# xxxupeng/stereo_toolbox

Hardware: AMD Instinct MI355X
Metric: stereo pairs/sec @ 540x960 D=192 (GwcNet_GC fwd+bwd) (higher is better)
Workload: dtype f32; 1 GPU; GwcNet_GC(maxdisp=192) train step: fwd+bwd+allreduce+Adam, 576x960 pairs (reference pad_to_2x shape), batch 1/GPU, fp32, synthetic randn inputs, deterministic filler weights; global_batch=1, parallelism=dp1, grad_sync=none (single rank: flat fp32 buffer packed, no collective), launch=eager, optimizer=torch.optim.Adam(fused=True)

## Files before the change

### include/stx_hip.h

```cpp
#ifndef STX_HIP_H
#define STX_HIP_H
#ifdef __cplusplus
extern "C" {
#endif

const char* stx_last_error(void);
const char* stx_build_info(void);
int stx_get_tuning(const char* name);
int stx_set_tuning(const char* name, int value);

int stx_cost_volume_fwd(const float* Lg, const float* Rg, int Cg, int G, const float* Lc, const float* Rc, int Cc,
                        const float* scale, float* vol, int B, int H, int W, int D, int mask_left, void* stream);
int stx_group_normalize_fwd(const float* x, float* y, int B, int C, int G, int HW, float out_scale, void* stream);
int stx_group_normalize_bwd(const float* x, const float* gy, float* gx, int B, int C, int G, int HW, float out_scale, void* stream);
int stx_cost_volume_bwd(const float* gvol, const float* Lg, const float* Rg, int Cg, int G, int Cc, float* gLg,
                        float* gRg, float* gLc, float* gRc, int B, int H, int W, int D, int mask_left, void* stream);

int stx_head_fwd(const float* cost, float* disp, float* stats, int B, int Dc, int Hc, int Wc, int D, int H, int W,
                 void* stream);
long long stx_head_bwd_workspace_floats(int B, int Dc, int H, int W);
int stx_head_bwd(const float* gdisp, const float* cost, const float* disp, const float* stats, float* gcost,
                 float* workspace, int B, int Dc, int Hc, int Wc, int D, int H, int W, void* stream);
int stx_head_fwd2(const float* cost, float* disp, float* stats, int B, int Dc, int Hc, int Wc, int D, int H, int W,
                  int align_corners, void* stream);
int stx_head_bwd2(const float* gdisp, const float* cost, const float* disp, const float* stats, float* gcost,
                  float* workspace, int B, int Dc, int Hc, int Wc, int D, int H, int W, int align_corners, void* stream);
int stx_softargmax_fwd(const float* x, float* out, int B, int D, int HW, void* stream);
int stx_argmax_fwd(const float* x, long long* out, int B, int D, int HW, void* stream);
int stx_unimodal_fwd(const float* x, float* out, int B, int D, int HW, void* stream);
int stx_dominant_modal_fwd(const float* x, float* out, int B, int D, int HW, void* stream);
int stx_modal_fwd(const float* x, float* out, float* aux, int B, int D, int HW, int kind, void* stream);
int stx_modal_bwd(const float* g, const float* out, const float* aux, float* gx, int B, int D, int HW, void* stream);
int stx_split_mode(const float* x, float* mode, unsigned char* mask, int B, int D, int HW, void* stream);
int stx_softmax_d_fwd(const float* x, float* y, int B, int D, int HW, void* stream);

long long stx_conv3d_packed_floats(int K, int N, int T);
int stx_conv3d_pack_weight(const float* w, float* wp, int A, int B, int T, int mode, void* stream);
int stx_conv3d_fwd_blocks(int Do, int Ho, int Wo);
long long stx_conv3d_fwd_stat_rows(int B, int Di, int Hi, int Wi, int Cin, int Cout, int ks, int stride);
int stx_conv3d_fwd(const float* x, const float* wp, float* out, const float* scale, const float* bias,
                   const float* residual, float* stats, int B, int Di, int Hi, int Wi, int Cin, int Cout, int ks,
                   int stride, int relu, void* stream);
int stx_deconv3d_fwd_blocks(int Di, int Hi, int Wi);
int stx_deconv3d_fwd(const float* x, const float* wp, float* out, const float* scale, const float* bias,
                     const float* residual, float* stats, int B, int Di, int Hi, int Wi, int Cin, int Cout, int Do,
                     int Ho, int Wo, int relu, void* stream);
long long stx_conv3d_wgrad_workspace_floats(int B, int Dc, int Hc, int Wc, int CF, int CC, int ks, int stride);
int stx_conv3d_wgrad(const float* fine, const float* coarse, float* dw, float* workspace, int B, int Df, int Hf, int Wf,
                     int CF, int Dc, int Hc, int Wc, int CC, int ks, int stride, void* stream);

int stx_conv3d_wgrad_bn_supported(int B, int D, int H, int W, int CF, int CC);
int stx_conv3d_wgrad_bn(const float* x, const float* gy, const float* z, const float* scale, const float* shift, const float* mean,
                        const float* invstd, const float* gamma, const float* sums, float inv_n, int act, float* dz, float* dw,
                        float* workspace, int B, int D, int H, int W, int CF, int CC, void* stream);

int stx_conv3d_axial_supported(int Cin, int Cout, int kd, int kh, int kw);
long long stx_conv3d_axial_packed_floats(int K, int N, int kd, int kh, int kw);
int stx_conv3d_axial_pack_weight(const float* w, float* wp, int A, int B, int kd, int kh, int kw, int mode, void* stream);
long long stx_conv3d_axial_fwd_stat_rows(int B, int D, int H, int W, int Cin, int Cout, int kd, int kh, int kw);
int stx_conv3d_axial_fwd(const float* x, const float* wp, float* out, const float* scale, const float* bias,
                         const float* residual, float* stats, int B, int D, int H, int W, int Cin, int Cout, int kd, int kh,
                         int kw, int act, void* stream);
long long stx_conv3d_axial_wgrad_workspace_floats(int B, int D, int H, int W, int CF, int CC, int kd, int kh, int kw);
int stx_conv3d_axial_wgrad(const float* x, const float* gz, float* dw, float* workspace, int B, int D, int H, int W, int CF,
                           int CC, int kd, int kh, int kw, void* stream);

int stx_convgru_supported(int hidden, int nx, int cx0, int cx1, int cx2, int ksize);
long long stx_convgru_packed_floats(int K, int N);
int stx_convgru_pack_weight(const float* w0, const float* w1, float* wp, int A, int Bd, int mode, void* stream);
int stx_convgru_gemm(const float* s0, int c0, int p0, const float* s1, int c1, int p1, const float* s2, int c2, int p2,
                     const float* s3, int c3, int p3, const float* wp, int N, int epi, int split, const float* bias0,
                     const float* bias1, const float* add0, int add0_pitch, const float* add1, int add1_pitch, const float* h,
                     int h_pitch, const float* z, float* out0, float* out1, float* out2, int out_pitch, int B, int H, int W,
                     void* stream);
int stx_convgru_gate_rows(long long P, int hidden);
int stx_convgru_gate_bwd(const float* g, int g_pitch, const float* z, const float* q, const float* h, int h_pitch, float* gq,
                         float* gz, float* rows, long long P, int hidden, void* stream);
int stx_convgru_reset_bwd(float* buf, int buf_pitch, const float* g, int g_pitch, const float* z, const float* r, const float* h,
                          int h_pitch, float* gr, float* rows, long long P, int hidden, void* stream);
int stx_convgru_row_sum(const float* rows, float* out, int nrows, int n, void* stream);
long long stx_convgru_wgrad_workspace_floats(int B, int H, int W, int K, int CC);
int stx_convgru_wgrad(const float* s0, int c0, int p0, const float* s1, int c1, int p1, const float* s2, int c2, int p2,
                      const float* s3, int c3, int p3, const float* g0, const float* g1, int CG, float* dw, float* workspace,
                      int B, int H, int W, void* stream);

int stx_selgru_supported(int hidden, int nx, int cx0, int cx1, int cx2);
long long stx_selgru_packed_floats(int K, int N);
int stx_selgru_pack_weight(const float* w0, const float* w1, float* wp, int A, int Bd, int mode, void* stream);
int stx_selgru_gemm(const float* s0, int c0, int p0, const float* s1, int c1, int p1, const float* s2, int c2, int p2,
                    const float* s3, int c3, int p3, const float* wp, int N, int epi, int split, const float* bias0,
                    const float* bias1, const float* add0, int add0_pitch, const float* add1, int add1_pitch, const float* h,
                    int h_pitch, const float* z, const float* att, const float* other, int blend, float* out0, float* out1,
                    float* out2, int out_pitch, long long P, void* stream);
int stx_selgru_blend_bwd(const float* g, int g_pitch, const float* att, const float* zs, const float* qs, const float* zl,
                         const float* ql, const float* h, int h_pitch, float* gs, float* gl, float* gatt, long long P, int hidden,
                         void* stream);
long long stx_selgru_col_sum_workspace_floats(long long P, int n);
int stx_selgru_col_sum(const float* m0, const float* m1, const float* m2, float* out, double* workspace, long long P, int n,
                       void* stream);
long long stx_selgru_wgrad_workspace_floats(long long P, int K, int CC);
int stx_selgru_wgrad(const float* s0, int c0, int p0, const float* s1, int c1, int p1, const float* s2, int c2, int p2,
                     const float* s3, int c3, int p3, const float* g0, const float* g1, int CG, float* dw, float* workspace,
                     long long P, void* stream);

int stx_csa_supported(int C, int ksize);
int stx_csa_blocks(long long HW, int C);
int stx_csa_pool(const float* x, int pitch, double* psum, float* pmax, int* pidx, int B, long long HW, int C, void* stream);
int stx_csa_gate(const double* psum, const float* pmax, const int* pidx, int nblk, const float* w1, const float* w2, float* gate,
                 double* pooled, int* argp, int B, long long HW, int C, void* stream);
int stx_csa_apply(const float* x, int pitch, const double* psum, const float* pmax, const int* pidx, int nblk, const float* w1,
                  const float* w2, float* xp, float* map, int* argc, float* gate, double* pooled, int* argp, int B, long long HW,
                  int C, void* stream);
int stx_csa_sam(const float* map, const float* w, float* att, int B, int H, int W, int ksize, void* stream);
long long stx_csa_sam_bwd_workspace_floats(int B, int H, int W, int ksize);
int stx_csa_sam_bwd(const float* g, const float* att, const float* map, const float* w, float* gpre, float* gmap, float* dw,
                    double* workspace, int B, int H, int W, int ksize, void* stream);
int stx_csa_apply_bwd(const float* x, int pitch, const float* gate, const float* gxp, int gxp_pitch, const float* gmap,
                      const int* argc, float* gx, double* pgate, int B, long long HW, int C, void* stream);
int stx_csa_gate_bwd(const double* pgate, int nblk, const float* gg, const double* pooled, const float* w1, const float* w2,
                     float* dw1, float* dw2, float* gavg, float* gmx, int B, long long HW, int C, void* stream);
int stx_csa_pool_bwd(float* gx, const float* gavg, const float* gmx, const int* argp, int accumulate, int B, long long HW, int C,
                     void* stream);

int stx_conv2d_supported(int Cin, int Cout);
long long stx_conv2d_stat_rows(int groups);
int stx_conv2d_fwd(const float* x, const float* w, float* out, float* stats, int B, int H, int W, int Cin, int Cout, int dgrad,
                   int groups, void* stream);

int stx_conv3d_c1_fwd(const float* x, const float* w, const float* residual, float* out, int B, int D, int H, int W,
                      int Cin, void* stream);
long long stx_conv3d_c1_wgrad_workspace_floats(int Cin);
int stx_conv3d_c1_wgrad(const float* x, const float* gy, float* dw, float* workspace, int B, int D, int H, int W,
                        int Cin, void* stream);
int stx_conv3d_c1_dgrad(const float* gy, const float* w, float* gx, int B, int D, int H, int W, int Cin, void* stream);

int stx_mish_fwd(const float* x, float* y, long long n, void* stream);
int stx_mish_bwd(const float* gy, const float* x, float* gx, long long n, void* stream);
int stx_depth_to_space(const float* y, float* out, int B, int D, int H, int W, int C, int inverse, void* stream);
int stx_gate_fwd(const float* cv, const float* att, float* out, int B, int D, long long HW, int C, void* stream);
int stx_gate_bwd(const float* g, const float* cv, const float* att, float* gcv, float* gatt, int B, int D, long long HW,
                 int C, void* stream);

int stx_concat_channels(const float* in0, const float* in1, const float* in2, const float* in3, int C0, int C1, int C2, int C3,
                        float* out, long long nvox, void* stream);
int stx_split_channels(const float* in, float* out0, float* out1, float* out2, float* out3, int C0, int C1, int C2, int C3,
                       long long nvox, void* stream);
int stx_transpose(const float* in, float* out, int N, int rows, int cols, void* stream);

int stx_dwconv_hw_fwd(const float* x, const float* w, const int* dil, float* out, int B, int D, int H, int W, int C,
                      int flip, void* stream);
long long stx_dwconv_hw_wgrad_workspace_floats(int C);
int stx_dwconv_hw_wgrad(const float* x, const float* gy, const int* dil, float* dw, float* workspace, int B, int D,
                        int H, int W, int C, void* stream);
int stx_cost_volume_scale_bwd(const float* gvol, const float* Lc, const float* Rc, float* gscale, int B, int Cc, int H,
                              int W, int D, int mask_left, void* stream);
int stx_scale_channels(const float* x, const float* s, float* out, long long nvox, int C, void* stream);
int stx_ac_volume_bwd(const float* gvol, const float* Lc, const float* Rc, const float* prob, float* gL, float* gR,
                      float* gprob, int B, int Cc, int H, int W, int D, int mask_left, void* stream);

int stx_bn_reduce_blocks(void);
int stx_bn_stats_rows(long long nvox, int C);
int stx_bn_stats(const float* z, float* partials, long long nvox, int C, int groups, void* stream);
int stx_bn_finalize(const float* partials, int nrows, int C, double count, const float* gamma, const float* beta,
                    float* running_mean, float* running_var, float momentum, float eps, float* scale, float* shift,
                    float* mean, float* invstd, void* stream);
int stx_bn_finalize_groups(const float* partials, int nrows, int C, double count, const float* gamma, const float* beta,
                           float* running_mean, float* running_var, float momentum, float eps, float* out, int groups,
                           void* stream);
int stx_bn_apply(const float* z1, const float* scale1, const float* shift1, const float* z2, const float* scale2,
                 const float* shift2, float* out, long long nvox, int C, int relu, int groups, void* stream);
int stx_bn_bwd_reduce(const float* gy, const float* y, const float* z1, const float* mean1, const float* invstd1,
                      const float* z2, const float* mean2, const float* invstd2, float* partials, float* sums,
                      long long nvox, int C, int relu, void* stream);
int stx_bn_bwd_apply(const float* gy, const float* y, const float* z1, const float* mean1, const float* invstd1,
                     const float* gamma1, const float* z2, const float* mean2, const float* invstd2,
                     const float* gamma2, const float* sums, float* dz1, float* dz2, float* gout, long long nvox, int C,
                     int relu, void* stream);
int stx_bn_bwd_reduce2(const float* gy, const float* y, const float* z1, const float* mean1, const float* invstd1,
                       const float* z2, const float* mean2, const float* invstd2, const float* scale1,
                       const float* shift1, const float* scale2, const float* shift2, float* partials, float* sums,
                       long long nvox, int C, int relu, int groups, void* stream);
int stx_bn_bwd_apply2(const float* gy, const float* y, const float* z1, const float* mean1, const float* invstd1,
                      const float* gamma1, const float* z2, const float* mean2, const float* invstd2,
                      const float* gamma2, const float* scale1, const float* shift1, const float* scale2,
                      const float* shift2, const float* sums, float* dz1, float* dz2, float* gout, long long nvox,
                      int C, int relu, int groups, void* stream);

int stx_pad_normalize_u8(const unsigned char* img, float* out, int B, int H, int W, int Hp, int Wp, int top,
                         const float* mean3, const float* std3, void* stream);

int stx_sampled_volume_fwd(const float* Lg, const float* Rg, int Cg, int G, const float* Lc, const float* Rc, int Cc,
                           const float* samples, float* vol, int B, int H, int W, int S, int CTp, void* stream);
int stx_sampled_volume_bwd(const float* gvol, const float* Lg, const float* Rg, int Cg, int G, int Cc,
                           const float* samples, float* gLg, float* gRg, float* gLc, float* gRc, int B, int H, int W,
                           int S, int CTp, void* stream);

int stx_warp_fwd(const float* x, const float* disp, float* out, int B, int C, int H, int W, void* stream);
int stx_warp_bwd(const float* gout, const float* x, const float* disp, float* gx, float* gdisp, int B, int C, int H, int W,
                 void* stream);
int stx_corr_volume_fwd(const float* ref, const float* tgt, float* vol, int B, int C, int H, int W, int maxdisp, int groups,
                        void* stream);
int stx_corr_volume_bwd(const float* gvol, const float* ref, const float* tgt, float* gref, float* gtgt, int B, int C, int H,
                        int W, int maxdisp, int groups, void* stream);
int stx_disparity_variance_fwd(const float* x, const float* disp, const float* samples, float* out, int B, int D, int HW,
                               void* stream);
int stx_disparity_variance_bwd(const float* g, const float* x, const float* disp, const float* samples, float* gx, float* gdisp,
                               float* gsamples, int B, int D, int HW, void* stream);

long long stx_geo_pyramid_floats(long long rows, int len, int C, int levels);
int stx_geo_corr_fwd(const float* fmap1, const float* fmap2, float* cpyr, int B, int C, int H, int W1, int W2, int levels,
                     void* stream);
int stx_geo_corr_bwd(const float* gcpyr, const float* fmap1, const float* fmap2, float* gfmap1, float* gfmap2, int B, int C, int H,
                     int W1, int W2, int levels, void* stream);
int stx_geo_pyramid_fwd(const float* vol, float* gpyr, int B, int D, int H, int W, int C, int levels, void* stream);
int stx_geo_pyramid_bwd(const float* ggpyr, float* gvol, int B, int D, int H, int W, int C, int levels, void* stream);
int stx_geo_lookup_fwd(const float* gpyr, const float* cpyr, const float* disp, const float* coords, float* out, int B, int H,
                       int W, int D, int C, int W2, int levels, int radius, void* stream);
int stx_geo_lookup_bwd(const float* gout, const float* disp, const float* coords, float* ggpyr, float* gcpyr, int B, int H, int W,
                       int D, int C, int W2, int levels, int radius, void* stream);
int stx_context_upsample_fwd(const float* disp_low, const float* up_weights, float* out, int B, int h, int w, void* stream);
int stx_context_upsample_bwd(const float* g, const float* disp_low, const float* up_weights, float* gdisp, float* gweights, int B,
                             int h, int w, void* stream);

long long stx_corr1d_pyramid_floats(long long rows, int W2, int levels);
int stx_corr1d_pyramid_fwd(const float* fmap1, const float* fmap2, float* cpyr, int B, int C, int H, int W1, int W2, int levels,
                           float scale, void* stream);
int stx_corr1d_pyramid_bwd(const float* gcpyr, const float* fmap1, const float* fmap2, float* gfmap1, float* gfmap2, int B, int C,
                           int H, int W1, int W2, int levels, float scale, void* stream);
int stx_corr1d_lookup_fwd(const float* cpyr, const float* base, const float* disp, const float* jobs, int njobs, float* out, int B,
                          int H, int W1, int W2, int levels, void* stream);
int stx_corr1d_lookup_bwd(const float* gout, const float* base, const float* disp, const float* jobs, int njobs, float* gcpyr,
                          int B, int H, int W1, int W2, int levels, void* stream);

int stx_allpairs_estimates_fwd(const float* vol, int which, float* disp_l, float* conf_l, float* disp_r, float* conf_r, float* stats,
                               int B, int H, int W1, int W2, void* stream);
int stx_allpairs_estimates_bwd(const float* g_disp_l, const float* g_conf_l, const float* g_disp_r, const float* g_conf_r,
                               const float* vol, const float* stats, float* gvol, int B, int H, int W1, int W2, void* stream);
int stx_corr1d_volume_pyramid_fwd(const float* vol, const float* tdisp, const float* tconf, float atten, float* cpyr, int B, int H,
                                  int W1, int W2, int levels, void* stream);
int stx_corr1d_volume_pyramid_bwd(const float* gcpyr, const float* tdisp, const float* tconf, float atten, float* gvol, int B, int H,
                                  int W1, int W2, int levels, void* stream);
int stx_truncate_mask_fwd(const float* disp, const float* conf, int has_th, float conf_th, float atten, float* mask, int B, int H,
                          int W, void* stream);

int stx_generate_masks_fwd(const float* mde, void* masks, int B, int N, int H, int W, void* stream);
int stx_masked_volume_fwd(const float* vol, const float* mde_l, const float* mde_r, float* out, int B, int N, int H, int W2, int W3,
                          void* stream);
int stx_masked_volume_bwd(const float* g, const float* mde_l, const float* mde_r, float* gvol, int B, int N, int H, int W2, int W3,
                          void* stream);
int stx_softlrc_fwd(const float* disp2, const float* disp3, float lrc_th, float* out2, float* out3, int B, int H, int W,
                    void* stream);
long long stx_softlrc_bwd_workspace_floats(int B, int H, int W);
int stx_softlrc_bwd(const float* g2, const float* g3, const float* disp2, const float* disp3, float lrc_th, void* workspace,
                    float* gdisp2, float* gdisp3, int B, int H, int W, void* stream);
int stx_weighted_lsq_fwd(const float* mde, const float* disp, const float* conf, float min_quantile, float max_quantile, float* scale,
                         float* shift, void* stats, int B, long long n, void* stream);
int stx_weighted_lsq_bwd(const float* g_scale, const float* g_shift, const float* mde, const float* disp, const float* conf,
                         const void* stats, float* g_mde, float* g_disp, float* g_conf, int B, long long n, void* stream);
int stx_mirror_detector_fwd(const float* stereo_disp, const float* mono_disp, const float* stereo_conf, const float* mono_conf,
                            float conf_th, float step_gain, float* out, long long n, void* stream);
int stx_mirror_detector_bwd(const float* g_out, const float* stereo_disp, const float* mono_disp, const float* stereo_conf,
                            const float* mono_conf, float conf_th, float step_gain, float* g_stereo_disp, float* g_mono_disp,
                            float* g_stereo_conf, float* g_mono_conf, long long n, void* stream);

int stx_photo_warp_fwd(const float* right, const float* disp, float* warped, float* valid, int B, int C, int H, int W, void* stream);
int stx_photo_warp_bwd(const float* gwarped, const float* right, const float* disp, float* gdisp, int B, int C, int H, int W,
                       void* stream);
int stx_ssim_fwd(const float* x, const float* y, float* out, int B, int C, int H, int W, int window, void* stream);
long long stx_ssim_bwd_workspace_floats(int B, int C, int H, int W);
int stx_ssim_bwd(const float* g_out, const float* x, const float* y, float* gx, float* gy, float* workspace, int B, int C, int H, int W,
                 int window, void* stream);
int stx_photometric_fwd(const float* left, const float* right, const float* disp, double ssim_weight, int enable_mask, float* loss,
                        int B, int C, int H, int W, void* stream);
long long stx_photometric_bwd_workspace_floats(int B, int C, int H, int W);
int stx_photometric_bwd(const float* gloss, const float* left, const float* right, const float* disp, double ssim_weight,
                        int enable_mask, float* gdisp, float* workspace, int B, int C, int H, int W, void* stream);
int stx_auto_mask_fwd(const float* left, const float* right, const float* disp, int denorm, unsigned char* mask, int B, int C, int H,
                      int W, void* stream);
long long stx_smoothness_workspace_floats(int B, int H, int W);
int stx_smoothness_fwd(const float* disp, const float* img, float* out, float* stats, float* workspace, int B, int C, int H, int W,
                       void* stream);
int stx_smoothness_bwd(const float* gout, const float* disp, const float* img, const float* stats, float* gdisp, int B, int C, int H,
                       int W, void* stream);

int stx_sttr_head_fwd(const float* attn, const float* phi, int mode, int iters, float log_one, float log_bin, float log_2w,
                      const unsigned char* occ_mask, const float* target, float* disp, float* occ, float* norm, int* arg,
                      float* gt_response, float* bin_left, float* bin_right, double* us, double* vs, int N, int H, int W, void* stream);
int stx_sttr_head_bwd(const float* g_disp, const float* g_occ, const float* g_gt, const float* g_bin_left, const float* g_bin_right,
                      const float* attn, const float* phi, int mode, int iters, float log_one, float log_bin, float log_2w,
                      const float* target, const float* disp, const float* norm, const int* arg, const double* us, const double* vs,
                      float* g_attn, double* phi_partials, float* g_phi, int N, int H, int W, void* stream);
int stx_sttr_transport_fwd(const float* attn, const float* phi, int mode, int iters, float log_one, float log_bin, float log_2w,
                           float* P, double* us, double* vs, int N, int H, int W, void* stream);
int stx_sttr_transport_bwd(const float* G, const float* attn, const float* phi, int mode, int iters, float log_one, float log_bin,
                           float log_2w, const double* us, const double* vs, float* g_attn, double* phi_partials, float* g_phi, int N,
                           int H, int W, void* stream);

int stx_sttr_attn_fwd(const float* q, const float* k, const float* v, const float* Qr, const float* Kr, int causal, float* o,
                      float* raw, float* avg, float* stats, int W, int B, int E, int head_dim, void* stream);
int stx_sttr_attn_bwd(const float* dO, const float* dRaw, const float* q, const float* k, const float* v, const float* Qr,
                      const float* Kr, const float* o, const float* stats, int causal, float* dq, float* dk, float* dv, float* dQr,
                      float* dKr, float* scratch, long long scratch_floats, int nb, int W, int B, int E, int head_dim, void* stream);

int stx_disp_attention_supported(int L, int C, int nhead, int F, int layers);
int stx_disp_attention_fwd(const float* x, const float* pe, const float* const* params, float* y, float* saved, const long long* seed,
                           float p, float eps, int N, int L, int C, int nhead, int F, int layers, int hw, long long sb, long long sp,
                           long long st, void* stream);
long long stx_disp_attention_bwd_workspace_floats(int N, int L, int C, int F);
int stx_disp_attention_bwd(const float* gy, const float* saved, const float* const* params, float* const* gparams, float* gx, float* gbuf,
                           float* workspace, long long workspace_floats, const long long* seed, float p, float eps, int N, int L, int C,
                           int nhead, int F, int layers, int hw, long long sb, long long sp, long long st, void* stream);
int stx_disp_attention_masks(const long long* seed, float p, unsigned char* masks, int N, int L, int C, int F, int layers, void* stream);

int stx_convex_upsample_fwd(const float* flow, const float* mask, float* out, int N, int D, int H, int W, int mask_channels, int f,
                            float scale, void* stream);
long long stx_convex_upsample_bwd_workspace_floats(int N, int D, int H, int W);
int stx_convex_upsample_bwd(const float* g, const float* flow, const float* mask, float* gflow, float* gmask, float* workspace, int N,
                            int D, int H, int W, int mask_channels, int f, float scale, void* stream);
int stx_softmax_context_upsample_fwd(const float* disp_low, const float* logits, float* out, int B, int h, int w, float scale,
                                     void* stream);
int stx_softmax_context_upsample_bwd(const float* g, const float* disp_low, const float* logits, float* gdisp, float* glogits,
                                     float* workspace, int B, int h, int w, float scale, void* stream);
int stx_sequence_loss_max_predictions(void);
long long stx_sequence_loss_workspace_floats(long long n);
int stx_sequence_loss_fwd(const float* const* preds, const double* weights, int K, const float* gt, float maxdisp, float* loss,
                          int* count, float* workspace, long long n, void* stream);
int stx_sequence_loss_bwd(const float* gloss, const float* const* preds, const double* weights, int K, const float* gt, float maxdisp,
                          const int* count, float* const* gpreds, long long n, void* stream);

int stx_monster_flaw_fwd(const float* left, const float* right, const float* disp_a, const float* disp_b, int zeros_pad, float* out_a,
                         float* out_b, float* valid, int B, int C, int H, int W, void* stream);
int stx_monster_flaw_bwd(const float* g_a, const float* g_b, const float* right, const float* disp_a, const float* disp_b, int zeros_pad,
                         float* g_left, float* g_right, float* g_disp_a, float* g_disp_b, int B, int C, int H, int W, void* stream);
int stx_monster_scale_shift(const float* mono, const float* gt, const unsigned char* mask, long long k, float* out, void* stats, int B,
                            long long n, void* stream);
int stx_monster_apply_scale_shift(const float* x, const float* scale_shift, int with_shift, float* out, int B, long long n,
                                  void* stream);

#ifdef __cplusplus
}
#endif
#endif
```

### stereo_toolbox_amd/_capi.py

```python
import ctypes
import os
import threading

import torch

_P = ctypes.c_void_p
_I = ctypes.c_int
_F = ctypes.c_float
_L = ctypes.c_longlong

SIGNATURES = {
    "stx_get_tuning": [ctypes.c_char_p],
    "stx_set_tuning": [ctypes.c_char_p, _I],
    "stx_cost_volume_fwd": [_P, _P, _I, _I, _P, _P, _I, _P, _P, _I, _I, _I, _I, _I, _P],
    "stx_cost_volume_bwd": [_P, _P, _P, _I, _I, _I, _P, _P, _P, _P, _I, _I, _I, _I, _I, _P],
    "stx_group_normalize_fwd": [_P, _P, _I, _I, _I, _I, _F, _P],
    "stx_group_normalize_bwd": [_P, _P, _P, _I, _I, _I, _I, _F, _P],
    "stx_head_fwd": [_P, _P, _P, _I, _I, _I, _I, _I, _I, _I, _P],
    "stx_head_bwd_workspace_floats": [_I, _I, _I, _I],
    "stx_head_bwd": [_P, _P, _P, _P, _P, _P, _I, _I, _I, _I, _I, _I, _I, _P],
    "stx_head_fwd2": [_P, _P, _P, _I, _I, _I, _I, _I, _I, _I, _I, _P],
    "stx_head_bwd2": [_P, _P, _P, _P, _P, _P, _I, _I, _I, _I, _I, _I, _I, _I, _P],
    "stx_softargmax_fwd": [_P, _P, _I, _I, _I, _P],
    "stx_argmax_fwd": [_P, _P, _I, _I, _I, _P],
    "stx_softmax_d_fwd": [_P, _P, _I, _I, _I, _P],
    "stx_unimodal_fwd": [_P, _P, _I, _I, _I, _P],
    "stx_dominant_modal_fwd": [_P, _P, _I, _I, _I, _P],
    "stx_modal_fwd": [_P, _P, _P, _I, _I, _I, _I, _P],
    "stx_modal_bwd": [_P, _P, _P, _P, _I, _I, _I, _P],
    "stx_split_mode": [_P, _P, _P, _I, _I, _I, _P],
    "stx_conv3d_packed_floats": [_I, _I, _I],
    "stx_conv3d_pack_weight": [_P, _P, _I, _I, _I, _I, _P],
    "stx_conv3d_fwd_blocks": [_I, _I, _I],
    "stx_conv3d_fwd_stat_rows": [_I, _I, _I, _I, _I, _I, _I, _I],
    "stx_deconv3d_fwd_blocks": [_I, _I, _I],
    "stx_conv3d_fwd": [_P, _P, _P, _P, _P, _P, _P, _I, _I, _I, _I, _I, _I, _I, _I, _I, _P],
    "stx_deconv3d_fwd": [_P, _P, _P, _P, _P, _P, _P, _I, _I, _I, _I, _I, _I, _I, _I, _I, _I, _P],
    "stx_conv3d_wgrad_workspace_floats": [_I, _I, _I, _I, _I, _I, _I, _I],
    "stx_conv3d_wgrad": [_P, _P, _P, _P, _I, _I, _I, _I, _I, _I, _I, _I, _I, _I, _I, _P],
    "stx_conv3d_wgrad_bn_supported": [_I, _I, _I, _I, _I, _I],
    "stx_conv3d_wgrad_bn": [_P] * 9 + [_F, _I, _P, _P, _P, _I, _I, _I, _I, _I, _I, _P],
    "stx_conv3d_axial_supported": [_I, _I, _I, _I, _I],
    "stx_conv3d_axial_packed_floats": [_I, _I, _I, _I, _I],
    "stx_conv3d_axial_pack_weight": [_P, _P, _I, _I, _I, _I, _I, _I, _P],
    "stx_conv3d_axial_fwd_stat_rows": [_I] * 9,
    "stx_conv3d_axial_fwd": [_P] * 7 + [_I] * 10 + [_P],
    "stx_conv3d_axial_wgrad_workspace_floats": [_I] * 9,
    "stx_conv3d_axial_wgrad": [_P, _P, _P, _P] + [_I] * 9 + [_P],
    "stx_convgru_supported": [_I] * 6,
    "stx_convgru_packed_floats": [_I, _I],
    "stx_convgru_pack_weight": [_P, _P, _P, _I, _I, _I, _P],
    "stx_convgru_gemm": [_P, _I, _I] * 4 + [_P, _I, _I, _I, _P, _P, _P, _I, _P, _I, _P, _I, _P, _P, _P, _P, _I, _I, _I, _I, _P],
    "stx_convgru_gate_rows": [_L, _I],
    "stx_convgru_gate_bwd": [_P, _I, _P, _P, _P, _I, _P, _P, _P, _L, _I, _P],
    "stx_convgru_reset_bwd": [_P, _I, _P, _I, _P, _P, _P, _I, _P, _P, _L, _I, _P],
    "stx_convgru_row_sum": [_P, _P, _I, _I, _P],
    "stx_convgru_wgrad_workspace_floats": [_I] * 5,
    "stx_convgru_wgrad": [_P, _I, _I] * 4 + [_P, _P, _I, _P, _P, _I, _I, _I, _P],
    "stx_selgru_supported": [_I] * 5,
    "stx_selgru_packed_floats": [_I, _I],
    "stx_selgru_pack_weight": [_P, _P, _P, _I, _I, _I, _P],
    "stx_selgru_gemm": [_P, _I, _I] * 4 + [_P, _I, _I, _I, _P, _P, _P, _I, _P, _I, _P, _I, _P, _P, _P, _I, _P, _P, _P, _I, _L, _P],
    "stx_selgru_blend_bwd": [_P, _I, _P, _P, _P, _P, _P, _P, _I, _P, _P, _P, _L, _I, _P],
    "stx_selgru_col_sum_workspace_floats": [_L, _I],
    "stx_selgru_col_sum": [_P, _P, _P, _P, _P, _L, _I, _P],
    "stx_selgru_wgrad_workspace_floats": [_L, _I, _I],
    "stx_selgru_wgrad": [_P, _I, _I] * 4 + [_P, _P, _I, _P, _P, _L, _P],
    "stx_csa_supported": [_I, _I],
    "stx_csa_blocks": [_L, _I],
    "stx_csa_pool": [_P, _I, _P, _P, _P, _I, _L, _I, _P],
    "stx_csa_gate": [_P, _P, _P, _I, _P, _P, _P, _P, _P, _I, _L, _I, _P],
    "stx_csa_apply": [_P, _I, _P, _P, _P, _I, _P, _P, _P, _P, _P, _P, _P, _P, _I, _L, _I, _P],
    "stx_csa_sam": [_P, _P, _P, _I, _I, _I, _I, _P],
    "stx_csa_sam_bwd_workspace_floats": [_I] * 4,
    "stx_csa_sam_bwd": [_P] * 8 + [_I] * 4 + [_P],
    "stx_csa_apply_bwd": [_P, _I, _P, _P, _I, _P, _P, _P, _P, _I, _L, _I, _P],
    "stx_csa_gate_bwd": [_P, _I, _P, _P, _P, _P, _P, _P, _P, _P, _I, _L, _I, _P],
    "stx_csa_pool_bwd": [_P, _P, _P, _P, _I, _I, _L, _I, _P],
    "stx_conv2d_supported": [_I, _I],
    "stx_conv2d_stat_rows": [_I],
    "stx_conv2d_fwd": [_P, _P, _P, _P, _I, _I, _I, _I, _I, _I, _I, _P],
    "stx_conv3d_c1_fwd": [_P, _P, _P, _P, _I, _I, _I, _I, _I, _P],
    "stx_conv3d_c1_wgrad_workspace_floats": [_I],
    "stx_conv3d_c1_wgrad": [_P, _P, _P, _P, _I, _I, _I, _I, _I, _P],
    "stx_conv3d_c1_dgrad": [_P, _P, _P, _I, _I, _I, _I, _I, _P],
    "stx_mish_fwd": [_P, _P, _L, _P],
    "stx_mish_bwd": [_P, _P, _P, _L, _P],
    "stx_depth_to_space": [_P, _P, _I, _I, _I, _I, _I, _I, _P],
    "stx_gate_fwd": [_P, _P, _P, _I, _I, _L, _I, _P],
    "stx_gate_bwd": [_P, _P, _P, _P, _P, _I, _I, _L, _I, _P],
    "stx_concat_channels": [_P, _P, _P, _P, _I, _I, _I, _I, _P, _L, _P],
    "stx_split_channels": [_P, _P, _P, _P, _P, _I, _I, _I, _I, _L, _P],
    "stx_transpose": [_P, _P, _I, _I, _I, _P],
    "stx_dwconv_hw_fwd": [_P, _P, _P, _P, _I, _I, _I, _I, _I, _I, _P],
    "stx_dwconv_hw_wgrad_workspace_floats": [_I],
    "stx_dwconv_hw_wgrad": [_P, _P, _P, _P, _P, _I, _I, _I, _I, _I, _P],
    "stx_cost_volume_scale_bwd": [_P, _P, _P, _P, _I, _I, _I, _I, _I, _I, _P],
    "stx_scale_channels": [_P, _P, _P, _L, _I, _P],
    "stx_ac_volume_bwd": [_P, _P, _P, _P, _P, _P, _P, _I, _I, _I, _I, _I, _I, _P],
    "stx_pad_normalize_u8": [_P, _P, _I, _I, _I, _I, _I, _I, _P, _P, _P],
    "stx_warp_fwd": [_P, _P, _P, _I, _I, _I, _I, _P],
    "stx_warp_bwd": [_P, _P, _P, _P, _P, _I, _I, _I, _I, _P],
    "stx_corr_volume_fwd": [_P, _P, _P, _I, _I, _I, _I, _I, _I, _P],
    "stx_corr_volume_bwd": [_P, _P, _P, _P, _P, _I, _I, _I, _I, _I, _I, _P],
    "stx_disparity_variance_fwd": [_P, _P, _P, _P, _I, _I, _I, _P],
    "stx_disparity_variance_bwd": [_P, _P, _P, _P, _P, _P, _P, _I, _I, _I, _P],
    "stx_sampled_volume_fwd": [_P, _P, _I, _I, _P, _P, _I, _P, _P, _I, _I, _I, _I, _I, _P],
    "stx_sampled_volume_bwd": [_P, _P, _P, _I, _I, _I, _P, _P, _P, _P, _P, _I, _I, _I, _I, _I, _P],
    "stx_geo_pyramid_floats": [_L, _I, _I, _I],
    "stx_geo_corr_fwd": [_P, _P, _P, _I, _I, _I, _I, _I, _I, _P],
    "stx_geo_corr_bwd": [_P, _P, _P, _P, _P, _I, _I, _I, _I, _I, _I, _P],
    "stx_geo_pyramid_fwd": [_P, _P, _I, _I, _I, _I, _I, _I, _P],
    "stx_geo_pyramid_bwd": [_P, _P, _I, _I, _I, _I, _I, _I, _P],
    "stx_geo_lookup_fwd": [_P, _P, _P, _P, _P, _I, _I, _I, _I, _I, _I, _I, _I, _P],
    "stx_geo_lookup_bwd": [_P, _P, _P, _P, _P, _I, _I, _I, _I, _I, _I, _I, _I, _P],
    "stx_context_upsample_fwd": [_P, _P, _P, _I, _I, _I, _P],
    "stx_context_upsample_bwd": [_P, _P, _P, _P, _P, _I, _I, _I, _P],
    "stx_corr1d_pyramid_floats": [_L, _I, _I],
    "stx_corr1d_pyramid_fwd": [_P, _P, _P, _I, _I, _I, _I, _I, _I, _F, _P],
    "stx_corr1d_pyramid_bwd": [_P, _P, _P, _P, _P, _I, _I, _I, _I, _I, _I, _F, _P],
    "stx_corr1d_lookup_fwd": [_P, _P, _P, _P, _I, _P, _I, _I, _I, _I, _I, _P],
    "stx_corr1d_lookup_bwd": [_P, _P, _P, _P, _I, _P, _I, _I, _I, _I, _I, _P],
    "stx_allpairs_estimates_fwd": [_P, _I, _P, _P, _P, _P, _P, _I, _I, _I, _I, _P],
    "stx_allpairs_estimates_bwd": [_P, _P, _P, _P, _P, _P, _P, _I, _I, _I, _I, _P],
    "stx_corr1d_volume_pyramid_fwd": [_P, _P, _P, _F, _P, _I, _I, _I, _I, _I, _P],
    "stx_corr1d_volume_pyramid_bwd": [_P, _P, _P, _F, _P, _I, _I, _I, _I, _I, _P],
    "stx_truncate_mask_fwd": [_P, _P, _I, _F, _F, _P, _I, _I, _I, _P],
    "stx_generate_masks_fwd": [_P, _P, _I, _I, _I, _I, _P],
    "stx_masked_volume_fwd": [_P, _P, _P, _P, _I, _I, _I, _I, _I, _P],
    "stx_masked_volume_bwd": [_P, _P, _P, _P, _I, _I, _I, _I, _I, _P],
    "stx_softlrc_fwd": [_P, _P, _F, _P, _P, _I, _I, _I, _P],
    "stx_softlrc_bwd_workspace_floats": [_I, _I, _I],
    "stx_softlrc_bwd": [_P, _P, _P, _P, _F, _P, _P, _P, _I, _I, _I, _P],
    "stx_weighted_lsq_fwd": [_P, _P, _P, _F, _F, _P, _P, _P, _I, _L, _P],
    "stx_weighted_lsq_bwd": [_P, _P, _P, _P, _P, _P, _P, _P, _P, _I, _L, _P],
    "stx_mirror_detector_fwd": [_P, _P, _P, _P, _F, _F, _P, _L, _P],
    "stx_mirror_detector_bwd": [_P, _P, _P, _P, _P, _F, _F, _P, _P, _P, _P, _L, _P],
    "stx_photo_warp_fwd": [_P, _P, _P, _P, _I, _I, _I, _I, _P],
    "stx_photo_warp_bwd": [_P, _P, _P, _P, _I, _I, _I, _I, _P],
    "stx_ssim_fwd": [_P, _P, _P, _I, _I, _I, _I, _I, _P],
    "stx_ssim_bwd_workspace_floats": [_I, _I, _I, _I],
    "stx_ssim_bwd": [_P, _P, _P, _P, _P, _P, _I, _I, _I, _I, _I, _P],
    "stx_photometric_fwd": [_P, _P, _P, ctypes.c_double, _I, _P, _I, _I, _I, _I, _P],
    "stx_photometric_bwd_workspace_floats": [_I, _I, _I, _I],
    "stx_photometric_bwd": [_P, _P, _P, _P, ctypes.c_double, _I, _P, _P, _I, _I, _I, _I, _P],
    "stx_auto_mask_fwd": [_P, _P, _P, _I, _P, _I, _I, _I, _I, _P],
    "stx_smoothness_workspace_floats": [_I, _I, _I],
    "stx_smoothness_fwd": [_P, _P, _P, _P, _P, _I, _I, _I, _I, _P],
    "stx_smoothness_bwd": [_P, _P, _P, _P, _P, _I, _I, _I, _I, _P],
    "stx_sttr_head_fwd": [_P, _P, _I, _I, _F, _F, _F] + [_P] * 11 + [_I, _I, _I, _P],
    "stx_sttr_head_bwd": [_P] * 7 + [_I, _I, _F, _F, _F] + [_P] * 9 + [_I, _I, _I, _P],
    "stx_sttr_transport_fwd": [_P, _P, _I, _I, _F, _F, _F, _P, _P, _P, _I, _I, _I, _P],
    "stx_sttr_transport_bwd": [_P, _P, _P, _I, _I, _F, _F, _F, _P, _P, _P, _P, _P, _I, _I, _I, _P],
    "stx_sttr_attn_fwd": [_P] * 5 + [_I] + [_P] * 4 + [_I, _I, _I, _I, _P],
    "stx_sttr_attn_bwd": [_P] * 9 + [_I] + [_P] * 6 + [_L, _I, _I, _I, _I, _I, _P],
    "stx_disp_attention_supported": [_I] * 5,
    "stx_disp_attention_fwd": [_P] * 6 + [_F, _F] + [_I] * 7 + [_L, _L, _L, _P],
    "stx_disp_attention_bwd_workspace_floats": [_I] * 4,
    "stx_disp_attention_bwd": [_P] * 7 + [_L, _P, _F, _F] + [_I] * 7 + [_L, _L, _L, _P],
    "stx_disp_attention_masks": [_P, _F, _P, _I, _I, _I, _I, _I, _P],
    "stx_convex_upsample_fwd": [_P, _P, _P, _I, _I, _I, _I, _I, _I, _F, _P],
    "stx_convex_upsample_bwd_workspace_floats": [_I, _I, _I, _I],
    "stx_convex_upsample_bwd": [_P, _P, _P, _P, _P, _P, _I, _I, _I, _I, _I, _I, _F, _P],
    "stx_softmax_context_upsample_fwd": [_P, _P, _P, _I, _I, _I, _F, _P],
    "stx_softmax_context_upsample_bwd": [_P, _P, _P, _P, _P, _P, _I, _I, _I, _F, _P],
    "stx_sequence_loss_max_predictions": [],
    "stx_sequence_loss_workspace_floats": [_L],
    "stx_sequence_loss_fwd": [_P, _P, _I, _P, _F, _P, _P, _P, _L, _P],
    "stx_sequence_loss_bwd": [_P, _P, _P, _I, _P, _F, _P, _P, _L, _P],
    "stx_monster_flaw_fwd": [_P, _P, _P, _P, _I, _P, _P, _P, _I, _I, _I, _I, _P],
    "stx_monster_flaw_bwd": [_P, _P, _P, _P, _P, _I, _P, _P, _P, _P, _I, _I, _I, _I, _P],
    "stx_monster_scale_shift": [_P, _P, _P, _L, _P, _P, _I, _L, _P],
    "stx_monster_apply_scale_shift": [_P, _P, _I, _P, _I, _L, _P],
    "stx_bn_reduce_blocks": [],
    "stx_bn_stats_rows": [_L, _I],
    "stx_bn_stats": [_P, _P, _L, _I, _I, _P],
    "stx_bn_finalize": [_P, _I, _I, ctypes.c_double, _P, _P, _P, _P, _F, _F, _P, _P, _P, _P, _P],
    "stx_bn_finalize_groups": [_P, _I, _I, ctypes.c_double, _P, _P, _P, _P, _F, _F, _P, _I, _P],
    "stx_bn_apply": [_P, _P, _P, _P, _P, _P, _P, _L, _I, _I, _I, _P],
    "stx_bn_bwd_reduce": [_P, _P, _P, _P, _P, _P, _P, _P, _P, _P, _L, _I, _I, _P],
    "stx_bn_bwd_apply": [_P, _P, _P, _P, _P, _P, _P, _P, _P, _P, _P, _P, _P, _P, _L, _I, _I, _P],
    "stx_bn_bwd_reduce2": [_P] * 14 + [_L, _I, _I, _I, _P],
    "stx_bn_bwd_apply2": [_P] * 18 + [_L, _I, _I, _I, _P],
}
_RET_CHARP = ("stx_last_error", "stx_build_info")


class StxError(RuntimeError):
    pass


class StxLib:

    def __init__(self, path):
        if not os.path.exists(path):
            raise StxError(
                f"HIP library not found: {path}. Build it with `python -m stereo_toolbox_amd.build` "
                "(hipcc, gfx950). There is no CPU fallback for the cost-volume hot path.")
        self.path = path
        self._dll = ctypes.CDLL(path)
        for name in _RET_CHARP:
            fn = getattr(self._dll, name)
            fn.restype = ctypes.c_char_p
            fn.argtypes = []
        self._fns = {}
        for name, argtypes in SIGNATURES.items():
            fn = getattr(self._dll, name, None)
            if fn is None:
                continue
            fn.restype = ctypes.c_longlong if name.endswith(("_floats", "_stat_rows")) else _I
            fn.argtypes = argtypes
            self._fns[name] = fn

    def has(self, name):
        return name in self._fns

    def build_info(self):
        return self._dll.stx_build_info().decode()

    def get_tuning(self, name):
        return self._fns["stx_get_tuning"](name.encode())

    def set_tuning(self, name, value):
        old = self.get_tuning(name)
        if old < 0 or self._fns["stx_set_tuning"](name.encode(), int(value)) != 0:
            raise StxError(f"unknown tuning switch {name}")
        return old

    def raw(self, name):
        return self._fns[name]

    def call(self, name, *args):
        fn = self._fns.get(name)
        if fn is None:
            raise StxError(f"{self.path} does not export {name}")
        rc = fn(*args)
        if rc != 0:
            raise StxError(f"{name} failed ({rc}): {self._dll.stx_last_error().decode()}")


_LIB = None
_LOCK = threading.Lock()
LIB_PATH = os.environ.get("STX_HIP_LIB") or os.path.join(os.path.dirname(os.path.abspath(__file__)), "lib", "libstx_hip.so")


def get_lib():
    global _LIB
    if _LIB is None:
        with _LOCK:
            if _LIB is None:
                _LIB = StxLib(LIB_PATH)
    return _LIB
```

### stereo_toolbox_amd/csrc/bn.hip

```cpp
#include "stx_common.h"
#include <stdlib.h>

namespace {

constexpr int BN_THREADS = 256;
constexpr int BN_RED_BLOCKS = 1024;

__device__ __forceinline__ double bn_block_sum(double v, double* red, int tid) {
    red[tid] = v;
    __syncthreads();
    for (int s = BN_THREADS / 2; s > 0; s >>= 1) {
        if (tid < s) red[tid] += red[tid + s];
        __syncthreads();
    }
    const double r = red[0];
    __syncthreads();
    return r;
}

__global__ __launch_bounds__(BN_THREADS) void bn_finalize_kernel(
    const float* __restrict__ partials, int nrows, int C, double count, const float* __restrict__ gamma,
    const float* __restrict__ beta, float* __restrict__ running_mean, float* __restrict__ running_var,
    float momentum, float eps, float* __restrict__ scale, float* __restrict__ shift, float* __restrict__ mean_out,
    float* __restrict__ invstd_out, int groups) {
    __shared__ double red[BN_THREADS];
    const int c = blockIdx.x, tid = threadIdx.x;
    for (int g = 0; g < groups; ++g, partials += (size_t)nrows * 2 * C, scale += C, shift += C, mean_out += C, invstd_out += C) {
    double s1 = 0.0, s2 = 0.0;
    for (int r = tid; r < nrows; r += BN_THREADS) {
        s1 += (double)partials[(size_t)r * 2 * C + c];
        s2 += (double)partials[(size_t)r * 2 * C + C + c];
    }
    s1 = bn_block_sum(s1, red, tid);
    s2 = bn_block_sum(s2, red, tid);
    if (tid == 0) {
        const double mean = s1 / count;
        double var = s2 / count - mean * mean;
        if (var < 0.0) var = 0.0;
        const float invstd = (float)(1.0 / sqrt(var + (double)eps));
        const float g = gamma ? gamma[c] : 1.f, bt = beta ? beta[c] : 0.f;
        const float sc = g * invstd;
        scale[c] = sc;
        shift[c] = bt - (float)mean * sc;
        mean_out[c] = (float)mean;
        invstd_out[c] = invstd;
        if (running_mean) running_mean[c] = (1.f - momentum) * running_mean[c] + momentum * (float)mean;
        if (running_var) {
            const double unb = count > 1.0 ? var * count / (count - 1.0) : var;
            running_var[c] = (1.f - momentum) * running_var[c] + momentum * (float)unb;
        }
    }
    }
}

constexpr int BN_FIN_THREADS = 512;

__device__ __forceinline__ double bn_shfl_down_f64(double v, int delta) {
    union { double d; float f[2]; } a, b;
    a.d = v;
    b.f[0] = __shfl_down(a.f[0], delta);
    b.f[1] = __shfl_down(a.f[1], delta);
    return b.d;
}

__global__ __launch_bounds__(BN_FIN_THREADS) void bn_finalize4_kernel(
    const float* __restrict__ partials, int nrows, int C, double count, const float* __restrict__ gamma,
    const float* __restrict__ beta, float* __restrict__ running_mean, float* __restrict__ running_var,
    float momentum, float eps, float* __restrict__ scale, float* __restrict__ shift, float* __restrict__ mean_out,
    float* __restrict__ invstd_out, int groups) {
    __shared__ double red[BN_FIN_THREADS / 64][8];
    const int c0 = blockIdx.x * 4, tid = threadIdx.x, lane = tid & 63, wave = tid >> 6;
    for (int g = 0; g < groups; ++g, partials += (size_t)nrows * 2 * C, scale += C, shift += C, mean_out += C, invstd_out += C) {
    if (g) __syncthreads();
    double acc[8] = {0.0, 0.0, 0.0, 0.0, 0.0, 0.0, 0.0, 0.0};
    const float* p = partials + c0;
#pragma unroll 4
    for (int r = tid; r < nrows; r += BN_FIN_THREADS) {
        const float4 a = stx_ld4(p + (size_t)r * 2 * C), b = stx_ld4(p + (size_t)r * 2 * C + C);
        acc[0] += (double)a.x; acc[1] += (double)a.y; acc[2] += (double)a.z; acc[3] += (double)a.w;
        acc[4] += (double)b.x; acc[5] += (double)b.y; acc[6] += (double)b.z; acc[7] += (double)b.w;
    }
#pragma unroll
    for (int k = 0; k < 8; ++k) {
#pragma unroll
        for (int d = 32; d > 0; d >>= 1) acc[k] += bn_shfl_down_f64(acc[k], d);
        if (lane == 0) red[wave][k] = acc[k];
    }
    __syncthreads();
    if (tid < 4) {
        double s1 = 0.0, s2 = 0.0;
        for (int w = 0; w < BN_FIN_THREADS / 64; ++w) { s1 += red[w][tid]; s2 += red[w][4 + tid]; }
        const int c = c0 + tid;
        const double mean = s1 / count;
        double var = s2 / count - mean * mean;
        if (var < 0.0) var = 0.0;
        const float invstd = (float)(1.0 / sqrt(var + (double)eps));
        const float g = gamma ? gamma[c] : 1.f, bt = beta ? beta[c] : 0.f;
        const float sc = g * invstd;
        scale[c] = sc;
        shift[c] = bt - (float)mean * sc;
        mean_out[c] = (float)mean;
        invstd_out[c] = invstd;
        if (running_mean) running_mean[c] = (1.f - momentum) * running_mean[c] + momentum * (float)mean;
        if (running_var) {
            const double unb = count > 1.0 ? var * count / (count - 1.0) : var;
            running_var[c] = (1.f - momentum) * running_var[c] + momentum * (float)unb;
        }
    }
    }
}

__global__ __launch_bounds__(BN_THREADS) void bn_apply_kernel(
    const float* __restrict__ z1, const float* __restrict__ scale1, const float* __restrict__ shift1,
    const float* __restrict__ z2, const float* __restrict__ scale2, const float* __restrict__ shift2,
    float* __restrict__ out, size_t nquads, int CQ, int relu) {
    {
        const size_t go = (size_t)blockIdx.y * nquads * 4, gc = (size_t)blockIdx.y * CQ * 4;
        z1 += go; out += go; scale1 += gc; shift1 += gc;
        if (z2) z2 += go;
        if (scale2) { scale2 += gc; shift2 += gc; }
    }
    for (size_t i = (size_t)blockIdx.x * BN_THREADS + threadIdx.x; i < nquads; i += (size_t)gridDim.x * BN_THREADS) {
        const int cq = (int)(i % CQ) * 4;
        float4 v = stx_ld4(z1 + i * 4);
        const float4 a = stx_ld4(scale1 + cq), b = stx_ld4(shift1 + cq);
        v.x = fmaf(v.x, a.x, b.x); v.y = fmaf(v.y, a.y, b.y); v.z = fmaf(v.z, a.z, b.z); v.w = fmaf(v.w, a.w, b.w);
        if (z2) {
            float4 u = stx_ld4(z2 + i * 4);
            if (scale2) {
                const float4 a2 = stx_ld4(scale2 + cq), b2 = stx_ld4(shift2 + cq);
                u.x = fmaf(u.x, a2.x, b2.x); u.y = fmaf(u.y, a2.y, b2.y);
                u.z = fmaf(u.z, a2.z, b2.z); u.w = fmaf(u.w, a2.w, b2.w);
            }
            v.x += u.x; v.y += u.y; v.z += u.z; v.w += u.w;
        }
        if (relu) {
            v.x = stx_act(v.x, relu); v.y = stx_act(v.y, relu); v.z = stx_act(v.z, relu); v.w = stx_act(v.w, relu);
        }
        stx_st4(out + i * 4, v);
    }
}

__global__ __launch_bounds__(BN_THREADS) void bn_bwd_reduce_kernel(
    const float* __restrict__ gy, const float* __restrict__ y, const float* __restrict__ z1,
    const float* __restrict__ mean1, const float* __restrict__ invstd1, const float* __restrict__ z2,
    const float* __restrict__ mean2, const float* __restrict__ invstd2, const float* __restrict__ sc1,
    const float* __restrict__ sh1, const float* __restrict__ sc2, const float* __restrict__ sh2, float* __restrict__ partials,
    size_t nvox, int C, int relu) {
    __shared__ float red[BN_THREADS * 12];
    const int tid = threadIdx.x;
    const int CQ = C >> 2;
    const int cq = tid % CQ, vl = tid / CQ, VPB = BN_THREADS / CQ;
    {
        const size_t go = (size_t)blockIdx.y * nvox * C, gc = (size_t)blockIdx.y * C;
        gy += go; z1 += go; mean1 += gc; invstd1 += gc;
        if (y) y += go;
        if (z2) z2 += go;
        if (mean2) { mean2 += gc; invstd2 += gc; }
        if (sc1) { sc1 += gc; sh1 += gc; }
        if (sc2) { sc2 += gc; sh2 += gc; }
        partials += (size_t)blockIdx.y * gridDim.x * 3 * C;
    }
    const float4 m1 = stx_ld4(mean1 + 4 * cq), i1 = stx_ld4(invstd1 + 4 * cq);
    float4 m2 = make_float4(0.f, 0.f, 0.f, 0.f), i2 = m2;
    const bool has2 = z2 && mean2;
    if (has2) { m2 = stx_ld4(mean2 + 4 * cq); i2 = stx_ld4(invstd2 + 4 * cq); }
    const bool remask = relu && !y;
    float4 a1 = m2, b1 = m2, a2 = m2, b2 = m2;
    if (remask) {
        a1 = stx_ld4(sc1 + 4 * cq); b1 = stx_ld4(sh1 + 4 * cq);
        if (has2) { a2 = stx_ld4(sc2 + 4 * cq); b2 = stx_ld4(sh2 + 4 * cq); }
    }
    float s[12];
#pragma unroll
    for (int k = 0; k < 12; ++k) s[k] = 0.f;
    for (size_t v = vl < VPB ? (size_t)blockIdx.x * VPB + vl : nvox; v < nvox; v += (size_t)gridDim.x * VPB) {
        const size_t o = v * C + 4 * cq;
        float4 g = stx_ld4(gy + o);
        const float4 a = stx_ld4(z1 + o);
        float4 c = make_float4(0.f, 0.f, 0.f, 0.f);
        if (has2) c = stx_ld4(z2 + o);
        if (relu) {
            float4 yy;
            if (remask) {
                yy.x = fmaf(a.x, a1.x, b1.x); yy.y = fmaf(a.y, a1.y, b1.y); yy.z = fmaf(a.z, a1.z, b1.z); yy.w = fmaf(a.w, a1.w, b1.w);
                if (has2) {
                    yy.x += fmaf(c.x, a2.x, b2.x); yy.y += fmaf(c.y, a2.y, b2.y);
                    yy.z += fmaf(c.z, a2.z, b2.z); yy.w += fmaf(c.w, a2.w, b2.w);
                }
            } else {
                yy = stx_ld4(y + o);
            }
            g.x = stx_act_bwd(g.x, yy.x, relu); g.y = stx_act_bwd(g.y, yy.y, relu);
            g.z = stx_act_bwd(g.z, yy.z, relu); g.w = stx_act_bwd(g.w, yy.w, relu);
        }
        s[0] += g.x; s[1] += g.y; s[2] += g.z; s[3] += g.w;
        s[4] = fmaf(g.x, (a.x - m1.x) * i1.x, s[4]); s[5] = fmaf(g.y, (a.y - m1.y) * i1.y, s[5]);
        s[6] = fmaf(g.z, (a.z - m1.z) * i1.z, s[6]); s[7] = fmaf(g.w, (a.w - m1.w) * i1.w, s[7]);
        if (has2) {
            s[8] = fmaf(g.x, (c.x - m2.x) * i2.x, s[8]); s[9] = fmaf(g.y, (c.y - m2.y) * i2.y, s[9]);
            s[10] = fmaf(g.z, (c.z - m2.z) * i2.z, s[10]); s[11] = fmaf(g.w, (c.w - m2.w) * i2.w, s[11]);
        }
    }
#pragma unroll
    for (int k = 0; k < 12; ++k) red[k * BN_THREADS + tid] = s[k];
    __syncthreads();
    for (int idx = tid; idx < 12 * CQ; idx += BN_THREADS) {
        const int k = idx / CQ, q = idx % CQ;
        float t = 0.f;
        for (int j = q; j < BN_THREADS; j += CQ) t += red[k * BN_THREADS + j];
        partials[((size_t)blockIdx.x * 3 + (k >> 2)) * C + 4 * q + (k & 3)] = t;
    }
}

__global__ __launch_bounds__(BN_THREADS) void bn_stats_kernel(const float* __restrict__ z, float* __restrict__ partials,
                                                              size_t nvox, int C) {
    __shared__ float red[BN_THREADS * 8];
    const int tid = threadIdx.x;
    const int CQ = C >> 2;
    const int cq = tid % CQ, vl = tid / CQ, VPB = BN_THREADS / CQ;
    z += (size_t)blockIdx.y * nvox * C;
    partials += (size_t)blockIdx.y * gridDim.x * 2 * C;
    float s[8];
#pragma unroll
    for (int k = 0; k < 8; ++k) s[k] = 0.f;
    const size_t step = (size_t)gridDim.x * VPB;
    size_t v = vl < VPB ? (size_t)blockIdx.x * VPB + vl : nvox;
    for (; v + 3 * step < nvox; v += 4 * step) {
        float4 a[4];
#pragma unroll
        for (int u = 0; u < 4; ++u) a[u] = stx_ld4(z + (v + u * step) * C + 4 * cq);
#pragma unroll
        for (int u = 0; u < 4; ++u) {
            s[0] += a[u].x; s[1] += a[u].y; s[2] += a[u].z; s[3] += a[u].w;
            s[4] = fmaf(a[u].x, a[u].x, s[4]); s[5] = fmaf(a[u].y, a[u].y, s[5]);
            s[6] = fmaf(a[u].z, a[u].z, s[6]); s[7] = fmaf(a[u].w, a[u].w, s[7]);
        }
    }
    for (; v < nvox; v += step) {
        const float4 a = stx_ld4(z + v * C + 4 * cq);
        s[0] += a.x; s[1] += a.y; s[2] += a.z; s[3] += a.w;
        s[4] = fmaf(a.x, a.x, s[4]); s[5] = fmaf(a.y, a.y, s[5]); s[6] = fmaf(a.z, a.z, s[6]); s[7] = fmaf(a.w, a.w, s[7]);
    }
#pragma unroll
    for (int k = 0; k < 8; ++k) red[k * BN_THREADS + tid] = s[k];
    __syncthreads();
    for (int idx = tid; idx < 8 * CQ; idx += BN_THREADS) {
        const int k = idx / CQ, q = idx % CQ;
        float t = 0.f;
        for (int j = q; j < BN_THREADS; j += CQ) t += red[k * BN_THREADS + j];
        partials[((size_t)blockIdx.x * 2 + (k >> 2)) * C + 4 * q + (k & 3)] = t;
    }
}

__global__ __launch_bounds__(BN_THREADS) void bn_colsum_kernel(const float* __restrict__ partials, int nrows, int M,
                                                               float* __restrict__ sums, int groups) {
    __shared__ double red[BN_THREADS];
    const int m = blockIdx.x, tid = threadIdx.x;
    float tot = 0.f;
    for (int g = 0; g < groups; ++g) {
        const float* p = partials + (size_t)g * nrows * M;
        double s = 0.0;
        for (int r = tid; r < nrows; r += BN_THREADS) s += (double)p[(size_t)r * M + m];
        s = bn_block_sum(s, red, tid);
        if (tid == 0) {
            sums[(size_t)g * M + m] = (float)s;
            tot += (float)s;
        }
    }
    if (groups > 1 && tid == 0) sums[(size_t)groups * M + m] = tot;
}

__global__ __launch_bounds__(BN_THREADS) void bn_bwd_apply_kernel(
    const float* __restrict__ gy, const float* __restrict__ y, const float* __restrict__ z1,
    const float* __restrict__ mean1, const float* __restrict__ invstd1, const float* __restrict__ gamma1,
    const float* __restrict__ z2, const float* __restrict__ mean2, const float* __restrict__ invstd2,
    const float* __restrict__ gamma2, const float* __restrict__ sc1, const float* __restrict__ sh1,
    const float* __restrict__ sc2, const float* __restrict__ sh2, const float* __restrict__ sums, float* __restrict__ dz1,
    float* __restrict__ dz2, float* __restrict__ gout, size_t nquads, int C, int relu, float inv_n) {
    const int CQ = C >> 2;
    {
        const size_t go = (size_t)blockIdx.y * nquads * 4, gc = (size_t)blockIdx.y * C;
        gy += go; z1 += go; dz1 += go; mean1 += gc; invstd1 += gc; sums += 3 * gc;
        if (y) y += go;
        if (z2) z2 += go;
        if (dz2) dz2 += go;
        if (gout) gout += go;
        if (mean2) { mean2 += gc; invstd2 += gc; }
        if (sc1) { sc1 += gc; sh1 += gc; }
        if (sc2) { sc2 += gc; sh2 += gc; }
    }
    const bool has2 = z2 && mean2 && dz2;
    const bool remask = relu && !y;
    for (size_t i = (size_t)blockIdx.x * BN_THREADS + threadIdx.x; i < nquads; i += (size_t)gridDim.x * BN_THREADS) {
        const int c = (int)(i % CQ) * 4;
        float4 g = stx_ld4(gy + i * 4);
        const float4 a = stx_ld4(z1 + i * 4);
        float4 a2v = make_float4(0.f, 0.f, 0.f, 0.f);
        if (has2) a2v = stx_ld4(z2 + i * 4);
        if (relu) {
            float4 yy;
            if (remask) {
                const float4 p1 = stx_ld4(sc1 + c), q1 = stx_ld4(sh1 + c);
                yy.x = fmaf(a.x, p1.x, q1.x); yy.y = fmaf(a.y, p1.y, q1.y); yy.z = fmaf(a.z, p1.z, q1.z); yy.w = fmaf(a.w, p1.w, q1.w);
                if (has2) {
                    const float4 p2 = stx_ld4(sc2 + c), q2 = stx_ld4(sh2 + c);
                    yy.x += fmaf(a2v.x, p2.x, q2.x); yy.y += fmaf(a2v.y, p2.y, q2.y);
                    yy.z += fmaf(a2v.z, p2.z, q2.z); yy.w += fmaf(a2v.w, p2.w, q2.w);
                }
            } else {
                yy = stx_ld4(y + i * 4);
            }
            g.x = stx_act_bwd(g.x, yy.x, relu); g.y = stx_act_bwd(g.y, yy.y, relu);
            g.z = stx_act_bwd(g.z, yy.z, relu); g.w = stx_act_bwd(g.w, yy.w, relu);
        }
        if (gout) stx_st4(gout + i * 4, g);
        const float4 sg = stx_ld4(sums + c);
        {
            const float4 m = stx_ld4(mean1 + c), is = stx_ld4(invstd1 + c);
            const float4 gm = gamma1 ? stx_ld4(gamma1 + c) : make_float4(1.f, 1.f, 1.f, 1.f);
            const float4 sx = stx_ld4(sums + C + c);
            float4 d;
            d.x = gm.x * is.x * (g.x - sg.x * inv_n - (a.x - m.x) * is.x * sx.x * inv_n);
            d.y = gm.y * is.y * (g.y - sg.y * inv_n - (a.y - m.y) * is.y * sx.y * inv_n);
            d.z = gm.z * is.z * (g.z - sg.z * inv_n - (a.z - m.z) * is.z * sx.z * inv_n);
            d.w = gm.w * is.w * (g.w - sg.w * inv_n - (a.w - m.w) * is.w * sx.w * inv_n);
            stx_st4(dz1 + i * 4, d);
        }
        if (has2) {
            const float4 a = a2v, m = stx_ld4(mean2 + c), is = stx_ld4(invstd2 + c);
            const float4 gm = gamma2 ? stx_ld4(gamma2 + c) : make_float4(1.f, 1.f, 1.f, 1.f);
            const float4 sx = stx_ld4(sums + 2 * C + c);
            float4 d;
            d.x = gm.x * is.x * (g.x - sg.x * inv_n - (a.x - m.x) * is.x * sx.x * inv_n);
            d.y = gm.y * is.y * (g.y - sg.y * inv_n - (a.y - m.y) * is.y * sx.y * inv_n);
            d.z = gm.z * is.z * (g.z - sg.z * inv_n - (a.z - m.z) * is.z * sx.z * inv_n);
            d.w = gm.w * is.w * (g.w - sg.w * inv_n - (a.w - m.w) * is.w * sx.w * inv_n);
            stx_st4(dz2 + i * 4, d);
        }
    }
}

int bn_grid(size_t nquads) {
    size_t g = (nquads + BN_THREADS - 1) / BN_THREADS;
    return (int)(g > 4096 ? 4096 : (g < 1 ? 1 : g));
}

}

extern "C" int stx_bn_reduce_blocks(void) {
    stx_begin(); return BN_RED_BLOCKS; }

static int bn_finalize_launch(const float* partials, int nrows, int C, double count, const float* gamma, const float* beta,
                              float* running_mean, float* running_var, float momentum, float eps, float* scale, float* shift,
                              float* mean, float* invstd, int groups, void* stream) {
    if (C % 4 == 0 && nrows >= 256)
        hipLaunchKernelGGL(bn_finalize4_kernel, dim3(C / 4), dim3(BN_FIN_THREADS), 0, (hipStream_t)stream, partials, nrows, C,
                           count, gamma, beta, running_mean, running_var, momentum, eps, scale, shift, mean, invstd, groups);
    else
        hipLaunchKernelGGL(bn_finalize_kernel, dim3(C), dim3(BN_THREADS), 0, (hipStream_t)stream, partials, nrows, C, count,
                           gamma, beta, running_mean, running_var, momentum, eps, scale, shift, mean, invstd, groups);
    return stx_check_launch("bn_finalize");
}

extern "C" int stx_bn_finalize(const float* partials, int nrows, int C, double count, const float* gamma,
                               const float* beta, float* running_mean, float* running_var, float momentum, float eps,
                               float* scale, float* shift, float* mean, float* invstd, void* stream) {
    stx_begin();
    STX_REQUIRE(partials && nrows > 0 && C > 0 && count > 0 && scale && shift && mean && invstd, "bn_finalize: bad args");
    return bn_finalize_launch(partials, nrows, C, count, gamma, beta, running_mean, running_var, momentum, eps, scale, shift,
                              mean, invstd, 1, stream);
}

extern "C" int stx_bn_finalize_groups(const float* partials, int nrows, int C, double count, const float* gamma,
                                      const float* beta, float* running_mean, float* running_var, float momentum, float eps,
                                      float* out, int groups, void* stream) {
    stx_begin();
    STX_REQUIRE(partials && nrows > 0 && C > 0 && count > 0 && out && groups >= 1, "bn_finalize_groups: bad args");
    const size_t gc = (size_t)groups * C;
    return bn_finalize_launch(partials, nrows, C, count, gamma, beta, running_mean, running_var, momentum, eps, out, out + gc,
                              out + 2 * gc, out + 3 * gc, groups, stream);
}

extern "C" int stx_bn_stats_rows(long long nvox, int C) {
    stx_begin();
    if (C < 4 || C % 4 != 0 || C / 4 > BN_THREADS || nvox < 1) return 0;
    const long long vpb = BN_THREADS / (C / 4);
    const long long g = (nvox + 4 * vpb - 1) / (4 * vpb);
    return (int)(g > 256 ? 256 : (g < 1 ? 1 : g));
}

extern "C" int stx_bn_stats(const float* z, float* partials, long long nvox, int C, int groups, void* stream) {
    stx_begin();
    STX_REQUIRE(z && partials && nvox > 0 && groups >= 1 && groups <= 65535, "bn_stats: bad args");
    STX_REQUIRE(C >= 4 && C % 4 == 0 && C / 4 <= BN_THREADS, "bn_stats: C=%d unsupported (a multiple of 4, at most 1024)", C);
    hipLaunchKernelGGL(bn_stats_kernel, dim3(stx_bn_stats_rows(nvox, C), groups), dim3(BN_THREADS), 0, (hipStream_t)stream, z,
                       partials, (size_t)nvox, C);
    return stx_check_launch("bn_stats");
}

extern "C" int stx_bn_apply(const float* z1, const float* scale1, const float* shift1, const float* z2,
                            const float* scale2, const float* shift2, float* out, long long nvox, int C, int relu,
                            int groups, void* stream) {
    stx_begin();
    STX_REQUIRE(z1 && scale1 && shift1 && out && nvox > 0 && C > 0 && C % 4 == 0, "bn_apply: bad args (C=%d)", C);
    STX_REQUIRE(!scale2 || (z2 && shift2), "bn_apply: second affine needs z2 and shift2");
    STX_REQUIRE(groups >= 1 && groups <= 65535, "bn_apply: groups=%d", groups);
    const size_t nquads = (size_t)nvox * (C / 4);
    hipLaunchKernelGGL(bn_apply_kernel, dim3(bn_grid(nquads), groups), dim3(BN_THREADS), 0, (hipStream_t)stream, z1, scale1,
                       shift1, z2, scale2, shift2, out, nquads, C / 4, relu);
    return stx_check_launch("bn_apply");
}

extern "C" int stx_bn_bwd_reduce2(const float* gy, const float* y, const float* z1, const float* mean1,
                                  const float* invstd1, const float* z2, const float* mean2, const float* invstd2,
                                  const float* scale1, const float* shift1, const float* scale2, const float* shift2,
                                  float* partials, float* sums, long long nvox, int C, int relu, int groups, void* stream) {
    stx_begin();
    STX_REQUIRE(gy && z1 && mean1 && invstd1 && partials && sums && nvox > 0, "bn_bwd_reduce: null operand");
    STX_REQUIRE(groups >= 1 && groups <= 65535, "bn_bwd_reduce: groups=%d", groups);
    STX_REQUIRE(C >= 4 && C % 4 == 0 && C / 4 <= BN_THREADS, "bn_bwd_reduce: C=%d unsupported (a multiple of 4, at most 1024)", C);
    STX_REQUIRE(!relu || y || (scale1 && shift1 && (!(z2 && mean2) || (scale2 && shift2))),
                "bn_bwd_reduce: the relu mask needs y or the forward pass's scale / shift vectors");
    STX_REQUIRE(relu != 2 || !y, "bn_bwd_reduce: Mish (activation code 2) differentiates the pre-activation value: pass y = NULL and the scale / shift vectors");
    hipStream_t st = (hipStream_t)stream;
    const int nblk = ((long long)nvox * C <= (9ll << 19)) ? BN_RED_BLOCKS / 4 : BN_RED_BLOCKS;
    hipLaunchKernelGGL(bn_bwd_reduce_kernel, dim3(nblk, groups), dim3(BN_THREADS), 0, st, gy, y, z1, mean1, invstd1,
                       z2, mean2, invstd2, scale1, shift1, scale2, shift2, partials, (size_t)nvox, C, relu);
    int rc = stx_check_launch("bn_bwd_reduce");
    if (rc) return rc;
    hipLaunchKernelGGL(bn_colsum_kernel, dim3(3 * C), dim3(BN_THREADS), 0, st, partials, nblk, 3 * C, sums, groups);
    return stx_check_launch("bn_colsum");
}

extern "C" int stx_bn_bwd_apply2(const float* gy, const float* y, const float* z1, const float* mean1,
                                 const float* invstd1, const float* gamma1, const float* z2, const float* mean2,
                                 const float* invstd2, const float* gamma2, const float* scale1, const float* shift1,
                                 const float* scale2, const float* shift2, const float* sums, float* dz1, float* dz2,
                                 float* gout, long long nvox, int C, int relu, int groups, void* stream) {
    stx_begin();
    STX_REQUIRE(gy && z1 && mean1 && invstd1 && sums && dz1 && nvox > 0 && C % 4 == 0, "bn_bwd_apply: bad args");
    STX_REQUIRE(groups >= 1 && groups <= 65535, "bn_bwd_apply: groups=%d", groups);
    STX_REQUIRE(!relu || y || (scale1 && shift1 && (!(z2 && mean2 && dz2) || (scale2 && shift2))),
                "bn_bwd_apply: the relu mask needs y or the forward pass's scale / shift vectors");
    STX_REQUIRE(relu != 2 || !y, "bn_bwd_apply: Mish (activation code 2) differentiates the pre-activation value: pass y = NULL and the scale / shift vectors");
    const size_t nquads = (size_t)nvox * (C / 4);
    hipLaunchKernelGGL(bn_bwd_apply_kernel, dim3(bn_grid(nquads), groups), dim3(BN_THREADS), 0, (hipStream_t)stream, gy, y, z1,
                       mean1, invstd1, gamma1, z2, mean2, invstd2, gamma2, scale1, shift1, scale2, shift2, sums, dz1, dz2,
                       gout, nquads, C, relu, (float)(1.0 / (double)nvox));
    return stx_check_launch("bn_bwd_apply");
}

extern "C" int stx_bn_bwd_reduce(const float* gy, const float* y, const float* z1, const float* mean1,
                                 const float* invstd1, const float* z2, const float* mean2, const float* invstd2,
                                 float* partials, float* sums, long long nvox, int C, int relu, void* stream) {
    return stx_bn_bwd_reduce2(gy, y, z1, mean1, invstd1, z2, mean2, invstd2, nullptr, nullptr, nullptr, nullptr, partials,
                              sums, nvox, C, relu, 1, stream);
}

extern "C" int stx_bn_bwd_apply(const float* gy, const float* y, const float* z1, const float* mean1,
                                const float* invstd1, const float* gamma1, const float* z2, const float* mean2,
                                const float* invstd2, const float* gamma2, const float* sums, float* dz1, float* dz2,
                                float* gout, long long nvox, int C, int relu, void* stream) {
    return stx_bn_bwd_apply2(gy, y, z1, mean1, invstd1, gamma1, z2, mean2, invstd2, gamma2, nullptr, nullptr, nullptr,
                             nullptr, sums, dz1, dz2, gout, nvox, C, relu, 1, stream);
}
```

### stereo_toolbox_amd/csrc/conv2d.hip

```cpp
#include "stx_common.h"

namespace {

constexpr int C2_THREADS = 256;
constexpr int C2_TH = 8, C2_TW = 16, C2_EH = C2_TH + 2, C2_EW = C2_TW + 2, C2_NV = C2_EH * C2_EW;

struct Conv2dArgs {
    const float* x;
    const float* w;
    float* out;
    float* stats;
    int B, H, W, Cin, Cout;
    int nHt, nWt, groups;
    int dgrad;
};

__device__ __forceinline__ f32x4 c2_zero4() { f32x4 z = {0.f, 0.f, 0.f, 0.f}; return z; }

template <int KQ, int ABL = 0, int PAD = 8>
__global__ __launch_bounds__(C2_THREADS) void conv2d_march_kernel(Conv2dArgs a) {
    constexpr int CIN = 16 * KQ, VS = CIN + PAD, F4 = CIN / 4;
    constexpr int WFLOATS = 9 * KQ * 256;
    constexpr int NST = (C2_NV * F4 + C2_THREADS - 1) / C2_THREADS;
    constexpr int SLOT = (NST * C2_THREADS / F4) * VS;
    constexpr int NSTEP = 9 * KQ;
    STX_DYN_SMEM(smem);
    float* wl = reinterpret_cast<float*>(smem);
    float* bufs = wl + WFLOATS;
    float* ssum = bufs + 2 * SLOT;

    const int tid = threadIdx.x, lane = tid & 63, wave = __builtin_amdgcn_readfirstlane(tid >> 6);
    const int i = lane & 15, kg = lane >> 4;

    const int wgs_g = gridDim.x / a.groups;
    const int grp = blockIdx.x / wgs_g, wl_id = blockIdx.x - grp * wgs_g;
    const int tiles_img = a.nHt * a.nWt;
    const int tiles_g = (a.B / a.groups) * tiles_img;
    const int nsl = a.Cout / 16;
    const long long units = (long long)tiles_g * nsl;
    const bool idle = grp >= a.groups;
    int u = idle ? 0 : __builtin_amdgcn_readfirstlane((int)(units * wl_id / wgs_g));
    const int u_end = idle ? 0 : __builtin_amdgcn_readfirstlane((int)(units * (wl_id + 1) / wgs_g));

    if (a.stats) {
        for (int e = tid; e < 2 * a.Cout; e += C2_THREADS) ssum[e] = 0.f;
    }

    unsigned rel[NST];
    int crd[NST];
#pragma unroll
    for (int k = 0; k < NST; ++k) {
        const int e = tid + k * C2_THREADS;
        const int v = e / F4, f = e - v * F4;
        const int hy = v / C2_EW, wx = v - hy * C2_EW;
        crd[k] = e < C2_NV * F4 ? (hy << 8 | wx) : -1;
        rel[k] = (unsigned)(((hy * a.W + wx) * CIN + 4 * f) * 4);
    }
    float4 stg[NST];
    auto decode = [&](int uu, int& slice, int& b, int& oh0, int& ow0) {
        slice = uu / tiles_g;
        const int t = uu - slice * tiles_g;
        const int bl = t / tiles_img, r = t - bl * tiles_img;
        const int ht = r / a.nWt, wt = r - ht * a.nWt;
        b = grp * (a.B / a.groups) + bl;
        oh0 = ht * C2_TH; ow0 = wt * C2_TW;
    };
    auto load_tile = [&](int b, int oh0, int ow0) {
        const long long org = (long long)(oh0 - 1) * a.W + (ow0 - 1), img = (long long)a.H * a.W;
        const stx_bufrsrc rs = stx_make_rsrc(a.x + ((long long)b * img + org) * CIN, (unsigned)((img - org) * CIN * 4));
#pragma unroll
        for (int k = 0; k < NST; ++k) {
            const int gh = oh0 - 1 + (crd[k] >> 8), gw = ow0 - 1 + (crd[k] & 255);
            const bool ok = crd[k] >= 0 && gh >= 0 && gh < a.H && gw >= 0 && gw < a.W;
            stg[k] = stx_buf_ld4(rs, ok ? rel[k] : STX_BUF_OOB, 0u);
        }
    };
    auto store_tile = [&](float* buf) {
#pragma unroll
        for (int k = 0; k < NST; ++k) {
            const int e = tid + k * C2_THREADS;
            const int v = e / F4, f = e - v * F4;
            if (e < C2_NV * F4) stx_st4(buf + v * VS + 4 * f, stg[k]);
        }
    };
    auto load_weights = [&](int slice) {
        if (!a.dgrad) {
            for (int e = tid; e < WFLOATS / 4; e += C2_THREADS) {
                const int l = e & 63, ts = e >> 6, tap = ts / KQ, s = ts - tap * KQ;
                stx_st4(wl + 4 * e, stx_ld4(a.w + ((size_t)(16 * slice + (l & 15)) * 9 + tap) * CIN + 16 * s + 4 * (l >> 4)));
            }
        } else {
            for (int e = tid; e < CIN * 9 * 4; e += C2_THREADS) {
                const int q = e & 3, kt = e >> 2, tap = kt % 9, k = kt / 9;
                const float4 v = stx_ld4(a.w + ((size_t)k * 9 + (8 - tap)) * a.Cout + 16 * slice + 4 * q);
                float* dst = wl + ((tap * KQ + (k >> 4)) * 64 + 4 * q + 16 * ((k & 15) >> 2)) * 4 + (k & 3);
                dst[0] = v.x; dst[4] = v.y; dst[8] = v.z; dst[12] = v.w;
            }
        }
    };

    f32x4 pacc0 = c2_zero4(), pacc1 = c2_zero4();
    unsigned pvoff[2] = {STX_BUF_OOB, STX_BUF_OOB}, cvoff[2] = {STX_BUF_OOB, STX_BUF_OOB};
    stx_bufrsrc prs = stx_make_rsrc(a.out, 0u);
    float s1[4] = {0.f, 0.f, 0.f, 0.f}, s2[4] = {0.f, 0.f, 0.f, 0.f};
    auto emit_prev = [&](int r) {
        f32x4 v = r ? pacc1 : pacc0;
        const bool ok = (int)pvoff[r] >= 0;
#pragma unroll
        for (int c = 0; c < 4; ++c) {
            v[c] = ok ? v[c] : 0.f;
            s1[c] += v[c];
            s2[c] = fmaf(v[c], v[c], s2[c]);
        }
        stx_buf_st4(prs, pvoff[r], 0u, make_float4(v[0], v[1], v[2], v[3]));
    };
    auto flush_stats = [&](int slice) {
#pragma unroll
        for (int c = 0; c < 4; ++c) {
#pragma unroll
            for (int d = 1; d < 16; d <<= 1) { s1[c] += __shfl_xor(s1[c], d); s2[c] += __shfl_xor(s2[c], d); }
        }
        for (int w = 0; w < 4; ++w) {
            if (wave == w && i == 0) {
#pragma unroll
                for (int c = 0; c < 4; ++c) {
                    ssum[16 * slice + 4 * kg + c] += s1[c];
                    ssum[a.Cout + 16 * slice + 4 * kg + c] += s2[c];
                }
            }
            __syncthreads();
        }
#pragma unroll
        for (int c = 0; c < 4; ++c) { s1[c] = 0.f; s2[c] = 0.f; }
    };

    const int abase0 = ((2 * wave) * C2_EW + i) * VS + 4 * kg, abase1 = abase0 + C2_EW * VS;
    const float* wlane = wl + lane * 4;

    int slice = 0, b = 0, oh0 = 0, ow0 = 0;
    if (u < u_end) {
        decode(u, slice, b, oh0, ow0);
        load_weights(slice);
        load_tile(b, oh0, ow0);
        store_tile(bufs);
    }
    __syncthreads();
    int cur = 0;
    while (u < u_end) {
        const bool more = u + 1 < u_end;
        int nslice = slice, nb = b, noh0 = oh0, now0 = ow0;
        if (more) decode(u + 1, nslice, nb, noh0, now0);
        const long long norg = (long long)(noh0 - 1) * a.W + (now0 - 1), img = (long long)a.H * a.W;
        const stx_bufrsrc nrs = stx_make_rsrc(a.x + ((long long)nb * img + norg) * CIN, more ? (unsigned)((img - norg) * CIN * 4) : 0u);
        const stx_bufrsrc crs = stx_make_rsrc(a.out + (size_t)b * img * a.Cout, (unsigned)(img * a.Cout * 4));
        const float* pbuf = bufs + cur * SLOT;
        float* nbuf = bufs + (cur ^ 1) * SLOT;
        f32x4 acc0, acc1;
        float4 av0[3], av1[3], bv[3];
        auto load_step = [&](int st, int slot) {
            const int tap = st / KQ, s = st - tap * KQ;
            const int kh = tap / 3, kw = tap - 3 * kh;
            const float* sl = pbuf + (kh * C2_EW + kw) * VS + 16 * s;
            av0[slot] = stx_ld4(sl + abase0);
            av1[slot] = stx_ld4(sl + abase1);
            bv[slot] = stx_ld4(wlane + st * 256);
        };
        load_step(0, 0);
        load_step(1, 1);
#pragma unroll
        for (int st = 0; st < NSTEP; ++st) {
            if (st + 2 < NSTEP) load_step(st + 2, (st + 2) % 3);
            const int cb = st % 3;
            acc0 = __builtin_amdgcn_mfma_f32_16x16x4f32(bv[cb].x, av0[cb].x, st == 0 ? c2_zero4() : acc0, 0, 0, 0);
            acc1 = __builtin_amdgcn_mfma_f32_16x16x4f32(bv[cb].x, av1[cb].x, st == 0 ? c2_zero4() : acc1, 0, 0, 0);
            acc0 = __builtin_amdgcn_mfma_f32_16x16x4f32(bv[cb].y, av0[cb].y, acc0, 0, 0, 0);
            acc1 = __builtin_amdgcn_mfma_f32_16x16x4f32(bv[cb].y, av1[cb].y, acc1, 0, 0, 0);
            acc0 = __builtin_amdgcn_mfma_f32_16x16x4f32(bv[cb].z, av0[cb].z, acc0, 0, 0, 0);
            acc1 = __builtin_amdgcn_mfma_f32_16x16x4f32(bv[cb].z, av1[cb].z, acc1, 0, 0, 0);
            acc0 = __builtin_amdgcn_mfma_f32_16x16x4f32(bv[cb].w, av0[cb].w, acc0, 0, 0, 0);
            acc1 = __builtin_amdgcn_mfma_f32_16x16x4f32(bv[cb].w, av1[cb].w, acc1, 0, 0, 0);
            if (st < NST) {
                const unsigned gh = (unsigned)(noh0 - 1 + (crd[st] >> 8)), gw = (unsigned)(now0 - 1 + (crd[st] & 255));
                const bool ok = (crd[st] >= 0) & (gh < (unsigned)a.H) & (gw < (unsigned)a.W);
                if (!(ABL & 1)) stg[st] = stx_buf_ld4(nrs, ok ? rel[st] : STX_BUF_OOB, 0u);
            }
            if ((st == 0 || st == 4) && !(ABL & 4)) emit_prev(st >> 2);
            if (st == 8 || st == 9) {
                const int r = st - 8;
                const int oh = oh0 + 2 * wave + r, ow = ow0 + i;
                cvoff[r] = (unsigned)((((oh * a.W + ow) * a.Cout) + 16 * slice + 4 * kg) * 4) | (((oh < a.H) & (ow < a.W)) ? 0u : STX_BUF_OOB);
            }
            if (st >= NSTEP - NST) {
                const int k = st - (NSTEP - NST);
                const int e = tid + k * C2_THREADS;
                const int v = e / F4, f = e - v * F4;
                if (!(ABL & 2)) stx_st4(nbuf + v * VS + 4 * f, stg[k]);
            }
            STX_SCHED_GROUP(0x008, 1); STX_SCHED_GROUP(0x100, 1);
            STX_SCHED_GROUP(0x008, 1); STX_SCHED_GROUP(0x100, 1);
            STX_SCHED_GROUP(0x008, 1); STX_SCHED_GROUP(0x100, 1);
            STX_SCHED_GROUP(0x008, 1); STX_SCHED_GROUP(0x002, 4);
            STX_SCHED_GROUP(0x008, 1); STX_SCHED_GROUP(0x010, 1); STX_SCHED_GROUP(0x002, 4);
            STX_SCHED_GROUP(0x008, 1); STX_SCHED_GROUP(0x010, 1); STX_SCHED_GROUP(0x002, 4);
            STX_SCHED_GROUP(0x008, 1); STX_SCHED_GROUP(0x200, 1); STX_SCHED_GROUP(0x002, 4);
            STX_SCHED_GROUP(0x008, 1);
            STX_SCHED_BARRIER();
        }
        prs = crs;
        pvoff[0] = cvoff[0]; pvoff[1] = cvoff[1];
        pacc0 = acc0; pacc1 = acc1;
        if (!(ABL & 8)) __syncthreads();
        if (more && nslice != slice) {
            emit_prev(0); emit_prev(1);
            pvoff[0] = pvoff[1] = STX_BUF_OOB;
            if (a.stats) flush_stats(slice);
            load_weights(nslice);
            __syncthreads();
        }
        slice = nslice; b = nb; oh0 = noh0; ow0 = now0;
        cur ^= 1;
        ++u;
    }
    emit_prev(0); emit_prev(1);
    if (a.stats) {
        __syncthreads();
        if (u_end > 0 && !idle) flush_stats(slice);
        __syncthreads();
        for (int e = tid; e < 2 * a.Cout; e += C2_THREADS) a.stats[(size_t)blockIdx.x * 2 * a.Cout + e] = ssum[e];
    }
}

int conv2d_grid(int groups) {
    int g = 256;
    g -= g % groups;
    return g < groups ? groups : g;
}

}

extern "C" int stx_conv2d_supported(int Cin, int Cout) {
    stx_begin();
    return (Cin == 32 || Cin == 64) && Cout >= 16 && Cout % 16 == 0 && Cout <= 256;
}

extern "C" long long stx_conv2d_stat_rows(int groups) {
    stx_begin();
    return groups >= 1 && groups <= 256 ? conv2d_grid(groups) : 0;
}

extern "C" int stx_conv2d_fwd(const float* x, const float* w, float* out, float* stats, int B, int H, int W, int Cin, int Cout,
                              int dgrad, int groups, void* stream) {
    stx_begin();
    STX_REQUIRE(x && w && out && B > 0 && H > 0 && W > 0 && (dgrad == 0 || dgrad == 1), "conv2d_fwd: bad args");
    STX_REQUIRE(stx_conv2d_supported(Cin, Cout), "conv2d_fwd: %d -> %d channels unsupported (Cin 32 or 64, Cout a multiple of 16)", Cin, Cout);
    STX_REQUIRE(groups >= 1 && groups <= 256 && B % groups == 0, "conv2d_fwd: batch %d does not split into %d groups", B, groups);
    STX_REQUIRE((long long)(H + 2) * W * (Cin > Cout ? Cin : Cout) * 4 < (1ll << 31), "conv2d_fwd: image too large for one descriptor");
    STX_REQUIRE(H < 32768 && W < 32768, "conv2d_fwd: image too large");
    Conv2dArgs a;
    a.x = x; a.w = w; a.out = out; a.stats = stats; a.dgrad = dgrad;
    a.B = B; a.H = H; a.W = W; a.Cin = Cin; a.Cout = Cout;
    a.nHt = stx_cdiv(H, C2_TH); a.nWt = stx_cdiv(W, C2_TW); a.groups = groups;
    const int grid = conv2d_grid(groups);
    int pad = stx_tune(STX_TUNE_C2_PAD);
    if (pad != 4 && pad != 12) pad = 8;
    const size_t lds = ((size_t)9 * Cin * 16 + (size_t)2 * 192 * (Cin + pad) + (size_t)2 * Cout) * 4;
    void (*k)(Conv2dArgs) = Cin == 64 ? conv2d_march_kernel<4> : conv2d_march_kernel<2>;
    if (pad == 4) k = Cin == 64 ? conv2d_march_kernel<4, 0, 4> : conv2d_march_kernel<2, 0, 4>;
    if (pad == 12) k = Cin == 64 ? conv2d_march_kernel<4, 0, 12> : conv2d_march_kernel<2, 0, 12>;
    const int abl = stx_tune(STX_TUNE_C2_ABLATE);
    if (abl && Cin == 64 && pad == 8)
        k = abl == 1 ? conv2d_march_kernel<4, 1> : abl == 2 ? conv2d_march_kernel<4, 2> : abl == 3 ? conv2d_march_kernel<4, 3>
          : abl == 4 ? conv2d_march_kernel<4, 4> : abl == 7 ? conv2d_march_kernel<4, 7> : abl == 8 ? conv2d_march_kernel<4, 8>
          : conv2d_march_kernel<4, 15>;
    if (int rc = stx_lds_require((const void*)k, lds, "conv2d_fwd")) return rc;
    hipLaunchKernelGGL(k, dim3(grid), dim3(C2_THREADS), lds, (hipStream_t)stream, a);
    return stx_check_launch("conv2d_fwd");
}
```

### stereo_toolbox_amd/csrc/stx_runtime.hip

```cpp
#include "stx_common.h"
#include <stdarg.h>
#include <stdio.h>

static thread_local char g_err[512] = "";

int stx_set_error(int code, const char* fmt, ...) {
    va_list ap;
    va_start(ap, fmt);
    vsnprintf(g_err, sizeof(g_err), fmt, ap);
    va_end(ap);
    return code;
}

int stx_check_launch(const char* what) {
    hipError_t e = hipGetLastError();
    if (e != hipSuccess) return stx_set_error(STX_ERR_LAUNCH, "%s: launch failed: %s", what, hipGetErrorString(e));
    return STX_OK;
}

bool stx_lds_try(const void* kern, size_t bytes) {
    if (bytes <= STX_LDS_DEFAULT) return true;
    if (bytes > STX_LDS_MAX) return false;
    if (hipFuncSetAttribute(kern, hipFuncAttributeMaxDynamicSharedMemorySize, (int)bytes) == hipSuccess) return true;
    (void)hipGetLastError();
    return false;
}

int stx_lds_require(const void* kern, size_t bytes, const char* what) {
    if (bytes > STX_LDS_MAX) return stx_set_error(STX_ERR_ARG, "%s: %zu B of LDS exceed the %zu B of a CU", what, bytes, STX_LDS_MAX);
    if (!stx_lds_try(kern, bytes)) return stx_set_error(STX_ERR_LAUNCH, "%s: %zu B of LDS refused by this device", what, bytes);
    return STX_OK;
}

extern "C" const char* stx_last_error(void) { return g_err; }

extern "C" const char* stx_build_info(void) {
#ifdef STX_HIPEMU
    return "stx-hipemu (host SIMT emulator build: tests only)";
#else
    return "stx-gfx950 (hipcc --offload-arch=gfx950)";
#endif
}

#include <stdlib.h>
#include <string.h>
namespace {
struct TuneEntry { const char* name; int value; };
constexpr int TUNE_N = STX_TUNE_COUNT + 1;
TuneEntry g_tune[TUNE_N] = {
    {"STX_MARCH_BS", 1}, {"STX_MARCH_EPI", 1}, {"STX_MARCH_ABLATE", 0}, {"STX_WGRAD_ABLATE", 0}, {"STX_WGRAD_MARCH", 3}, {"STX_WGRAD_GRID", 0}, {"STX_CONV_L1_MARCH", 0}, {"STX_CONV_S2_DENSE", 1}, {"STX_CONV_WN", 2},
    {"STX_CV_OLD", 0}, {"STX_CV_GRID", 0}, {"STX_CV_PF", 0}, {"STX_CV_UNITS", 1}, {"STX_CV_WIN", 0}, {"STX_CVB_OLD", 0}, {"STX_CVB_TEAM", 0}, {"STX_CVB_GRID", 0}, {"STX_CVB_NSET", 3},
    {"STX_SV_BWD_V1", 0}, {"STX_DWCONV_ROLL", 1}, {"STX_C2_PAD", 8}, {"STX_C2_ABLATE", 0}, {"STX_DA_GRID", 0},
};
struct TuneInit {
    TuneInit() {
        for (int i = 0; i < TUNE_N; ++i)
            if (const char* e = getenv(g_tune[i].name)) g_tune[i].value = atoi(e);
    }
} g_tune_init;
}

int stx_tune(StxTune id) { return g_tune[id].value; }

extern "C" int stx_get_tuning(const char* name) {
    for (int i = 0; i < TUNE_N; ++i)
        if (name && !strcmp(name, g_tune[i].name)) return g_tune[i].value;
    return -1;
}

extern "C" int stx_set_tuning(const char* name, int value) {
    for (int i = 0; i < TUNE_N; ++i)
        if (name && !strcmp(name, g_tune[i].name)) { g_tune[i].value = value; return STX_OK; }
    return stx_set_error(STX_ERR_ARG, "stx_set_tuning: unknown switch %s", name ? name : "(null)");
}
```

### stereo_toolbox_amd/models/features2d.py

```python
import math
import os
import threading

import torch
import torch.nn as nn
import torch.nn.functional as F

from .. import ops
from ..aggregation import _bn_state, _fold


def channels_last_weights_(module):
    for m in module.modules():
        if isinstance(m, nn.Conv2d) and m.weight.dim() == 4:
            m.weight.data = m.weight.data.contiguous(memory_format=torch.channels_last)
    return module


def fused_glue(x, *bns):
    if os.environ.get("STX_FEAT2D_FUSED", "1") == "0":
        return False
    if x.dtype != torch.float32 or not ops.on_device(x):
        return False
    if ops.autocast_active():
        return False
    if not all(isinstance(b, nn.modules.batchnorm._BatchNorm) for b in bns):
        return False
    if all(b.training for b in bns):
        return True
    return (not torch.is_grad_enabled() and not any(b.training for b in bns)
            and all(b.track_running_stats and b.running_mean is not None for b in bns))


class view_groups:
    _tls = threading.local()

    def __init__(self, n):
        self.new = int(n)

    @staticmethod
    def current():
        return getattr(view_groups._tls, "n", 1)

    def __enter__(self):
        self.old, view_groups._tls.n = view_groups.current(), self.new
        return self

    def __exit__(self, *exc):
        view_groups._tls.n = self.old
        return False


def _nhwc(t):
    v = t.permute(0, 2, 3, 1)
    return v if v.is_contiguous() else v.contiguous()


def cat_features(parts):
    parts = list(parts)
    if (os.environ.get("STX_FEAT2D_FUSED", "1") != "0" and os.environ.get("STX_FEAT2D_FUSED_CAT", "1") != "0" and 2 <= len(parts) <= 4
            and all(p.dtype == torch.float32 and ops.on_device(p) and p.shape[1] % 4 == 0
                    and p.is_contiguous(memory_format=torch.channels_last) for p in parts)):
        return ops.cat_channels([_nhwc(p) for p in parts]).permute(0, 3, 1, 2)
    return torch.cat(parts, dim=1)


def own_conv2d(x, conv):
    return (os.environ.get("STX_FEAT2D_CONV", "1") != "0" and x.dtype == torch.float32 and ops.on_device(x)
            and ops.conv2d_supported(conv) and x.shape[0] % view_groups.current() == 0)


def conv_bn_act(x, conv, bn, relu=False, residual=None, second=None):
    G = view_groups.current()
    part = None
    if bn.training and own_conv2d(x, conv):
        zl, part = ops.Conv2dFn.apply(x, conv.weight, G)
        z = zl.permute(0, 3, 1, 2)
    else:
        z = F.conv2d(x, conv.weight, conv.bias, conv.stride, conv.padding, conv.dilation, conv.groups)
        zl = _nhwc(z)
    if not bn.training:
        if torch.is_grad_enabled() and (z.requires_grad or bn.weight.requires_grad):
            raise ops.StxError("conv_bn_act: eval-mode BatchNorm under autograd has no fused backward -- gate the call "
                               "with fused_glue() over every BatchNorm of the block")
        sc, sh = _fold(bn)
        if second is not None:
            sc2, sh2 = _fold(second[1])
            y = ops.bn_apply(zl, sc, sh, _nhwc(second[0]), sc2, sh2, relu)
        else:
            y = ops.bn_apply(zl, sc, sh, None if residual is None else _nhwc(residual), None, None, relu)
        return y.permute(0, 3, 1, 2)
    st = _bn_state(bn, part if part is not None else ops.bn_stats(zl.detach(), G), zl.numel() // zl.shape[-1] // G, steps=G)
    if second is not None:
        z2l = _nhwc(second[0])
        bn2 = second[1]
        st2 = _bn_state(bn2, ops.bn_stats(z2l.detach(), G), z2l.numel() // z2l.shape[-1] // G, steps=G)
        y = ops.BnActFn.apply(zl, bn.weight, bn.bias, z2l, bn2.weight, bn2.bias, None, relu, st, st2, G)
    else:
        y = ops.BnActFn.apply(zl, bn.weight, bn.bias, None, None, None, None if residual is None else _nhwc(residual),
                              relu, st, None, G)
    return y.permute(0, 3, 1, 2)


def convbn_relu_chain(seq, x):
    i, n = 0, len(seq)
    while i < n:
        m = seq[i]
        if isinstance(m, nn.Sequential) and len(m) == 2 and isinstance(m[0], nn.Conv2d):
            relu = i + 1 < n and isinstance(seq[i + 1], nn.ReLU)
            x = conv_bn_act(x, m[0], m[1], relu=relu)
            i += 2 if relu else 1
        else:
            x = m(x)
            i += 1
    return x


def _chain_bns(seq):
    return [m[1] for m in seq if isinstance(m, nn.Sequential) and len(m) == 2 and isinstance(m[0], nn.Conv2d)]


def run_head2d(seq, x):
    if fused_glue(x, *_chain_bns(seq)):
        return convbn_relu_chain(seq, x)
    return seq(x)


def convbn(cin, cout, k, stride, pad, dilation):
    return nn.Sequential(
        nn.Conv2d(cin, cout, k, stride, dilation if dilation > 1 else pad, dilation, bias=False),
        nn.BatchNorm2d(cout))


class BasicBlock(nn.Module):
    expansion = 1

    def __init__(self, inplanes, planes, stride, downsample, pad, dilation):
        super().__init__()
        self.conv1 = nn.Sequential(convbn(inplanes, planes, 3, stride, pad, dilation), nn.ReLU(inplace=True))
        self.conv2 = convbn(planes, planes, 3, 1, pad, dilation)
        self.downsample = downsample
        self.stride = stride

    def forward(self, x):
        bns = [self.conv1[0][1], self.conv2[1]] + ([self.downsample[1]] if self.downsample is not None else [])
        if fused_glue(x, *bns):
            y = conv_bn_act(x, self.conv1[0][0], self.conv1[0][1], relu=True)
            if self.downsample is None:
                return conv_bn_act(y, self.conv2[0], self.conv2[1], residual=x)
            d = self.downsample[0]
            zd = F.conv2d(x, d.weight, d.bias, d.stride, d.padding, d.dilation, d.groups)
            return conv_bn_act(y, self.conv2[0], self.conv2[1], second=(zd, self.downsample[1]))
        y = self.conv2(self.conv1(x))
        if self.downsample is not None:
            x = self.downsample(x)
        return y + x


class ResTrunk(nn.Module):

    def __init__(self):
        super().__init__()
        self.inplanes = 32
        self.firstconv = nn.Sequential(convbn(3, 32, 3, 2, 1, 1), nn.ReLU(inplace=True),
                                       convbn(32, 32, 3, 1, 1, 1), nn.ReLU(inplace=True),
                                       convbn(32, 32, 3, 1, 1, 1), nn.ReLU(inplace=True))
        self.layer1 = self._make_layer(32, 3, 1, 1, 1)
        self.layer2 = self._make_layer(64, 16, 2, 1, 1)
        self.layer3 = self._make_layer(128, 3, 1, 1, 1)
        self.layer4 = self._make_layer(128, 3, 1, 1, 2)

    def _make_layer(self, planes, blocks, stride, pad, dilation):
        down = None
        if stride != 1 or self.inplanes != planes:
            down = nn.Sequential(nn.Conv2d(self.inplanes, planes, 1, stride, bias=False), nn.BatchNorm2d(planes))
        layers = [BasicBlock(self.inplanes, planes, stride, down, pad, dilation)]
        self.inplanes = planes
        layers += [BasicBlock(planes, planes, 1, None, pad, dilation) for _ in range(1, blocks)]
        return nn.Sequential(*layers)

    def trunk(self, x):
        if fused_glue(x, *_chain_bns(self.firstconv)):
            x = convbn_relu_chain(self.firstconv, x.contiguous(memory_format=torch.channels_last))
        else:
            x = self.firstconv(x)
        x = self.layer1(x)
        l2 = self.layer2(x)
        l3 = self.layer3(l2)
        l4 = self.layer4(l3)
        return l2, l3, l4


def init_reference_style(model):
    for m in model.modules():
        if isinstance(m, (nn.Conv2d, nn.Conv3d)):
            n = m.out_channels
            for k in m.kernel_size:
                n *= k
            m.weight.data.normal_(0, math.sqrt(2.0 / n))
        elif isinstance(m, (nn.BatchNorm2d, nn.BatchNorm3d)):
            m.weight.data.fill_(1)
            m.bias.data.zero_()
        elif isinstance(m, nn.Linear):
            m.bias.data.zero_()


class _SplitViewsFn(torch.autograd.Function):

    @staticmethod
    def forward(ctx, both, B):
        ctx.B, ctx.n, ctx.fmt = B, both.shape[0], (torch.channels_last if both.dim() == 4 and
                                                   both.is_contiguous(memory_format=torch.channels_last) else torch.contiguous_format)
        return both[:B], both[B:]

    @staticmethod
    def backward(ctx, gl, gr):
        if gl is None and gr is None:
            return None, None
        ref = gl if gl is not None else gr
        if gl is None:
            gl = ref.new_zeros((ctx.B,) + tuple(ref.shape[1:]))
        if gr is None:
            gr = ref.new_zeros((ctx.n - ctx.B,) + tuple(ref.shape[1:]))
        return torch.cat((gl.contiguous(memory_format=ctx.fmt), gr.contiguous(memory_format=ctx.fmt)), 0), None


def _split_views(both, B):
    if isinstance(both, dict):
        halves = {k: _SplitViewsFn.apply(v, B) for k, v in both.items()}
        return {k: h[0] for k, h in halves.items()}, {k: h[1] for k, h in halves.items()}
    return _SplitViewsFn.apply(both, B)


def run_pair(extractor, left, right, training):
    if training:
        bns = [m for m in extractor.modules() if isinstance(m, nn.modules.batchnorm._BatchNorm)]
        if (os.environ.get("STX_FEAT2D_PAIRED", "1") != "0" and left.shape == right.shape and bns and fused_glue(left, *bns)
                and all(b.momentum is not None and not isinstance(b, nn.SyncBatchNorm) for b in bns)
                and getattr(extractor, "fused_everywhere", False)):
            with view_groups(2):
                both = extractor(torch.cat((left, right), 0))
            return _split_views(both, left.shape[0])
        return extractor(left), extractor(right)
    both = extractor(torch.cat((left, right), 0))
    B = left.shape[0]
    if isinstance(both, dict):
        return {k: v[:B] for k, v in both.items()}, {k: v[B:] for k, v in both.items()}
    return both[:B], both[B:]
```

### stereo_toolbox_amd/ops.py

```python
import ctypes

import torch

from ._capi import StxError, get_lib

_P = ctypes.c_void_p


class _DevPtr(ctypes.c_void_p):
    """A device pointer that remembers the device of the tensor it came from: _call() reads the launch device off its
    own arguments, so nothing survives between launches (an exception between building the arguments and the launch
    cannot leak state into the next one)."""


def _stream(dev=None):
    return _P(torch.cuda.current_stream(dev).cuda_stream)


def _p(t):
    if t is None:
        return None
    p = _DevPtr(t.data_ptr())
    p.dev = t.device
    return p


def on_device(t):
    return t.is_cuda


def _chk(t, name, dims=None):
    if t is None:
        return
    if not t.is_cuda:
        raise StxError(f"{name}: expected a ROCm device tensor, got {t.device} -- the cost-volume hot path has "
                       "no CPU fallback (the CPU oracle lives in oracle/ and is test-only)")
    if t.dtype != torch.float32:
        raise StxError(f"{name}: expected float32, got {t.dtype}")
    if not t.is_contiguous():
        raise StxError(f"{name}: expected a dense contiguous tensor, strides {t.stride()}")
    if dims is not None and t.dim() != dims:
        raise StxError(f"{name}: expected {dims} dims, got shape {tuple(t.shape)}")


def _call(name, *args):
    dev = None
    for a in args:
        if isinstance(a, _DevPtr):
            if dev is None:
                dev = a.dev
            elif a.dev != dev:
                raise StxError(f"{name}: operands live on different devices ({dev} and {a.dev})")
    if dev is not None and dev.type == "cuda" and dev.index != torch.cuda.current_device():
        with torch.cuda.device(dev):
            get_lib().call(name, *args, _stream(dev))
    else:
        get_lib().call(name, *args, _stream(dev))


_LOW = (torch.float16, torch.bfloat16)


def _to_fp32(v):
    if isinstance(v, torch.Tensor):
        return v.float() if v.dtype in _LOW else v
    if isinstance(v, dict):
        return {k: _to_fp32(x) for k, x in v.items()}
    if isinstance(v, (list, tuple)):
        return type(v)(_to_fp32(x) for x in v)
    return v


def autocast_active():
    return torch.is_autocast_enabled("cuda") or torch.is_autocast_enabled("cpu")


def fp32_region(fn):
    import functools

    @functools.wraps(fn)
    def wrapped(*args, **kwargs):
        if not autocast_active():
            return fn(*args, **kwargs)
        with torch.autocast("cuda", enabled=False), torch.autocast("cpu", enabled=False):
            return fn(*_to_fp32(args), **_to_fp32(kwargs))
    return wrapped


def to_ncdhw(x):
    return x.permute(0, 4, 1, 2, 3)


def to_ndhwc(x):
    return x.permute(0, 2, 3, 4, 1).contiguous()


class _Workspace:

    def __init__(self):
        self.bufs = {}

    def get(self, tag, nfloats, device):
        sid = torch.cuda.current_stream(device).cuda_stream if device.type == "cuda" else 0
        key = (device.index, sid, tag)
        b = self.bufs.get(key)
        if b is None or b.numel() < nfloats:
            b = torch.empty(int(nfloats), dtype=torch.float32, device=device)
            self.bufs[key] = b
        return b


_WS = _Workspace()


_CACHE_ENABLED = True


def set_weight_cache(enabled):
    global _CACHE_ENABLED
    _CACHE_ENABLED = bool(enabled)


def invalidate_caches(model):
    for m in model.modules():
        m.__dict__.pop("_stx_fold", None)
    for p in model.parameters():
        p.__dict__.pop("_stx_packed", None)


def pack_weight(w, mode, owner=None):
    _chk(w, "weight", 5)
    if owner is not None and _CACHE_ENABLED:
        cache = owner.__dict__.setdefault("_stx_packed", {})
        hit = cache.get(mode)
        if hit is not None and hit[0] == (owner._version, owner.data_ptr()):
            return hit[1]
    A, Bd = w.shape[0], w.shape[1]
    T = w.shape[2] * w.shape[3] * w.shape[4]
    K, N = (Bd, A) if mode == 0 else (A, Bd)
    n = get_lib().raw("stx_conv3d_packed_floats")(K, N, T)
    wp = torch.empty(n, dtype=torch.float32, device=w.device)
    _call("stx_conv3d_pack_weight", _p(w), _p(wp), A, Bd, T, mode)
    if owner is not None and _CACHE_ENABLED:
        cache[mode] = ((owner._version, owner.data_ptr()), wp)
    return wp


def _pad_channels(t, C):
    if t.shape[-1] == C:
        return t
    out = t.new_zeros(*t.shape[:-1], C)
    out[..., : t.shape[-1]] = t
    return out


def pad_input_channels(x, w):
    Cin = x.shape[-1]
    Cp = (Cin + 7) // 8 * 8
    if Cp == Cin:
        return x, w
    wp = w.new_zeros(w.shape[0], Cp, *w.shape[2:])
    wp[:, :Cin] = w
    return _pad_channels(x, Cp), wp


def pad_weight_channels(w, Cp):
    if w.shape[1] == Cp:
        return w
    wp = w.new_zeros(w.shape[0], Cp, *w.shape[2:])
    wp[:, : w.shape[1]] = w
    return wp


def conv_out_dims(D, H, W, ks, stride):
    pad = ks // 2
    return tuple((d + 2 * pad - ks) // stride + 1 for d in (D, H, W))


def conv3d_forward(x, wp, Cout, ks, stride, scale=None, bias=None, residual=None, relu=False, want_stats=False):
    _chk(x, "x", 5)
    B, D, H, W, Cin = x.shape
    Do, Ho, Wo = conv_out_dims(D, H, W, ks, stride)
    out = torch.empty(B, Do, Ho, Wo, Cout, dtype=torch.float32, device=x.device)
    stats = None
    if want_stats:
        rows = get_lib().raw("stx_conv3d_fwd_stat_rows")(B, D, H, W, Cin, Cout, ks, stride)
        stats = torch.empty(rows, 2, Cout, dtype=torch.float32, device=x.device)
    _call("stx_conv3d_fwd", _p(x), _p(wp), _p(out), _p(scale), _p(bias), _p(residual), _p(stats), B, D, H, W, Cin,
          Cout, ks, stride, int(relu))
    return out, stats


def deconv3d_forward(x, wp, Cout, out_dims=None, scale=None, bias=None, residual=None, relu=False, want_stats=False):
    _chk(x, "x", 5)
    B, D, H, W, Cin = x.shape
    Do, Ho, Wo = out_dims if out_dims is not None else (2 * D, 2 * H, 2 * W)
    if Cout > 64:
        if Cout % 64 != 0:
            raise StxError(f"deconv3d_forward: Cout={Cout} > 64 must be a multiple of 64")
        nt = Cout // 32
        wv = wp.view(-1, Cin // 8, nt, 256)
        outs, sts = [], []
        for h in range(Cout // 64):
            sl = slice(64 * h, 64 * h + 64)
            o, st_ = deconv3d_forward(x, wv[:, :, 2 * h:2 * h + 2].contiguous(), 64, (Do, Ho, Wo),
                                      None if scale is None else scale[sl].contiguous(),
                                      None if bias is None else bias[sl].contiguous(),
                                      None if residual is None else residual[..., sl].contiguous(), relu, want_stats)
            outs.append(o)
            sts.append(st_)
        return torch.cat(outs, -1), (torch.cat(sts, -1) if want_stats else None)
    out = torch.empty(B, Do, Ho, Wo, Cout, dtype=torch.float32, device=x.device)
    stats = None
    if want_stats:
        nb = get_lib().raw("stx_deconv3d_fwd_blocks")(D, H, W)
        stats = torch.empty(B * nb, 2, Cout, dtype=torch.float32, device=x.device)
    _call("stx_deconv3d_fwd", _p(x), _p(wp), _p(out), _p(scale), _p(bias), _p(residual), _p(stats), B, D, H, W, Cin,
          Cout, Do, Ho, Wo, int(relu))
    return out, stats


def conv3d_wgrad(fine, coarse, ks, stride):
    B, Df, Hf, Wf, CF = fine.shape
    _, Dc, Hc, Wc, CC = coarse.shape
    n = get_lib().raw("stx_conv3d_wgrad_workspace_floats")(B, Dc, Hc, Wc, CF, CC, ks, stride)
    ws = _WS.get("wgrad", n, fine.device)
    dw = torch.empty(CC, CF, ks ** 3, dtype=torch.float32, device=fine.device)
    _call("stx_conv3d_wgrad", _p(fine), _p(coarse), _p(dw), _p(ws), B, Df, Hf, Wf, CF, Dc, Hc, Wc, CC, ks, stride)
    return dw


def conv3d_wgrad_bn(x, gy, pend):
    B, D, H, W, CF = x.shape
    CC = gy.shape[-1]
    n = get_lib().raw("stx_conv3d_wgrad_workspace_floats")(B, D, H, W, CF, CC, 3, 1)
    ws = _WS.get("wgrad", n, x.device)
    dw = torch.empty(CC, CF, 27, dtype=torch.float32, device=x.device)
    dz = torch.empty_like(gy)
    _call("stx_conv3d_wgrad_bn", _p(x), _p(gy), _p(pend.z), _p(pend.scale), _p(pend.shift), _p(pend.mean), _p(pend.invstd),
          _p(pend.gamma), _p(pend.sums), float(pend.inv_n), int(pend.act), _p(dz), _p(dw), _p(ws), B, D, H, W, CF, CC)
    return dw, dz


class _PendingBn:
    __slots__ = ("g", "z", "scale", "shift", "mean", "invstd", "gamma", "sums", "inv_n", "act")

    def materialize(self):
        C = self.z.shape[-1]
        nvox = self.z.numel() // C
        dz = torch.empty_like(self.z)
        _call("stx_bn_bwd_apply2", _p(self.g), None, _p(self.z), _p(self.mean), _p(self.invstd), _p(self.gamma), None, None,
              None, None, _p(self.scale), _p(self.shift), None, None, _p(self.sums), _p(dz), None, None, nvox, C, int(self.act), 1)
        return dz


_BN_DEFER = {"outstanding": 0, "armed": False}


def _bn_defer_check():
    n, _BN_DEFER["outstanding"], _BN_DEFER["armed"] = _BN_DEFER["outstanding"], 0, False
    if n:
        raise StxError(f"{n} deferred BatchNorm-backward record(s) were not consumed by their convolution's backward node: "
                       "the gradients of this backward pass are wrong (set STX_BN_BWD_IN_WGRAD=0 and report)")


def _defer_pending_bn(g, pend):
    g._stx_pending_bn = pend
    _BN_DEFER["outstanding"] += 1
    if not _BN_DEFER["armed"]:
        _BN_DEFER["armed"] = True
        torch.autograd.Variable._execution_engine.queue_callback(_bn_defer_check)


def bn_defer_reset_if_stale():
    if not _BN_DEFER["armed"]:
        return
    task_id = getattr(torch._C, "_current_graph_task_id", None)
    if task_id is None or task_id() == -1:
        _BN_DEFER["outstanding"], _BN_DEFER["armed"] = 0, False


def _take_pending_bn(g):
    pend = getattr(g, "_stx_pending_bn", None) if g is not None else None
    if pend is not None:
        del g._stx_pending_bn
        _BN_DEFER["outstanding"] -= 1
        if pend.g is not g:
            raise StxError("deferred BatchNorm backward: record attached to a different gradient tensor")
    return pend


def _is_c1(w, ks, stride, transposed):
    return (not transposed) and ks == 3 and stride == 1 and w.shape[0] == 1 and w.shape[1] % 16 == 0 and w.shape[1] <= 64


def conv3d_c1_forward(x, w, residual=None):
    _chk(x, "x", 5)
    _chk(w, "weight", 5)
    B, D, H, W, Cin = x.shape
    out = torch.empty(B, D, H, W, 1, dtype=torch.float32, device=x.device)
    _call("stx_conv3d_c1_fwd", _p(x), _p(w), _p(residual), _p(out), B, D, H, W, Cin)
    return out


def conv3d_c1_wgrad(x, gy):
    B, D, H, W, Cin = x.shape
    ws = _WS.get("c1wgrad", get_lib().raw("stx_conv3d_c1_wgrad_workspace_floats")(Cin), x.device)
    dw = torch.empty(1, Cin, 3, 3, 3, dtype=torch.float32, device=x.device)
    _call("stx_conv3d_c1_wgrad", _p(x), _p(gy), _p(dw), _p(ws), B, D, H, W, Cin)
    return dw


def conv3d_c1_dgrad(gy, w, Cin):
    B, D, H, W, _ = gy.shape
    gx = torch.empty(B, D, H, W, Cin, dtype=torch.float32, device=gy.device)
    _call("stx_conv3d_c1_dgrad", _p(gy), _p(w), _p(gx), B, D, H, W, Cin)
    return gx


class ConvRawFn(torch.autograd.Function):

    @staticmethod
    def forward(ctx, x, w, ks, stride, transposed, want_stats):
        _chk(x, "x", 5)
        ctx.cin_true = None
        ctx.x_prepadded = False
        if not transposed and x.shape[-1] != w.shape[1]:
            if x.shape[-1] != (w.shape[1] + 7) // 8 * 8:
                raise StxError(f"conv: input has {x.shape[-1]} channels, weight expects {w.shape[1]}")
            ctx.cin_true, ctx.x_prepadded = w.shape[1], True
            w = pad_weight_channels(w, x.shape[-1])
        elif not transposed and x.shape[-1] % 8 != 0:
            ctx.cin_true = x.shape[-1]
            x, w = pad_input_channels(x, w)
        if _is_c1(w, ks, stride, transposed) and not want_stats:
            z, stats = conv3d_c1_forward(x, w.contiguous()), None
        elif transposed:
            Cout = w.shape[1]
            z, stats = deconv3d_forward(x, pack_weight(w, 2), Cout, want_stats=want_stats)
        else:
            Cout = w.shape[0]
            z, stats = conv3d_forward(x, pack_weight(w, 0), Cout, ks, stride, want_stats=want_stats)
        ctx.save_for_backward(x, w)
        ctx.cfg = (ks, stride, transposed)
        if stats is None:
            stats = x.new_empty(0)
        ctx.mark_non_differentiable(stats)
        return z, stats

    @staticmethod
    def backward(ctx, gz, _gstats):
        x, w = ctx.saved_tensors
        ks, stride, transposed = ctx.cfg
        pend = _take_pending_bn(gz)
        gx = gw = None
        B, D, H, W, Cin = x.shape
        if pend is not None:
            if (ctx.needs_input_grad[1] and not transposed and ks == 3 and stride == 1 and ctx.cin_true is None
                    and get_lib().raw("stx_conv3d_wgrad_bn_supported")(B, D, H, W, Cin, w.shape[0])):
                gw_pre, gz = conv3d_wgrad_bn(x, gz, pend)
                gw_pre = gw_pre.reshape(w.shape)
            else:
                gw_pre, gz = None, pend.materialize()
        else:
            gw_pre = None
        gz = gz.contiguous()
        if transposed:
            Ci, Co = w.shape[0], w.shape[1]
            if ctx.needs_input_grad[0]:
                gx, _ = conv3d_forward(gz, pack_weight(w, 0), Ci, 3, 2)
            if ctx.needs_input_grad[1]:
                gz_w = gz if Co % 32 == 0 else _pad_channels(gz, (Co + 31) // 32 * 32)
                x_w = x if Ci % 32 == 0 else _pad_channels(x, (Ci + 31) // 32 * 32)
                gw = conv3d_wgrad(gz_w, x_w, 3, 2)[:Ci, :Co].reshape(w.shape)
        else:
            Co, Ci = w.shape[0], w.shape[1]
            c1 = _is_c1(w, ks, stride, transposed)
            gz_k, w_k = gz, w
            if Co % 8 != 0 and not c1:
                Cp = (Co + 7) // 8 * 8
                gz_k = _pad_channels(gz, Cp)
                w_k = w.new_zeros(Cp, *w.shape[1:])
                w_k[:Co] = w
            if ctx.needs_input_grad[0]:
                if c1:
                    gx = conv3d_c1_dgrad(gz, w.contiguous(), Ci)
                elif stride == 1 and Ci > 128:
                    parts = []
                    for lo in range(0, Ci, 128):
                        hi = min(Ci, lo + 128)
                        g, _ = conv3d_forward(gz_k, pack_weight(w_k[:, lo:hi].contiguous(), 1), hi - lo, ks, 1)
                        parts.append(g)
                    gx = torch.cat(parts, -1)
                elif stride == 1:
                    gx, _ = conv3d_forward(gz_k, pack_weight(w_k, 1), Ci, ks, 1)
                else:
                    if Co % 32:
                        Cp = (Co + 31) // 32 * 32
                        gz_k = _pad_channels(gz, Cp)
                        w_k = w.new_zeros(Cp, *w.shape[1:])
                        w_k[:Co] = w
                    gx, _ = deconv3d_forward(gz_k, pack_weight(w_k, 2), Ci, out_dims=(D, H, W))
            if gw_pre is not None:
                gw = gw_pre
            elif ctx.needs_input_grad[1]:
                if c1:
                    gw = conv3d_c1_wgrad(x, gz)
                else:
                    gz_w = gz if Co % 32 == 0 else _pad_channels(gz, (Co + 31) // 32 * 32)
                    x_w = x if Ci % 32 == 0 else _pad_channels(x, (Ci + 31) // 32 * 32)
                    gw = conv3d_wgrad(x_w, gz_w, ks, stride)[:Co, :Ci].reshape(w.shape)
        if ctx.cin_true is not None:
            if gx is not None and not ctx.x_prepadded:
                gx = gx[..., :ctx.cin_true].contiguous()
            if gw is not None:
                gw = gw[:, :ctx.cin_true].contiguous()
        return gx, gw, None, None, None, None


AXIAL_MAX_CHANNELS = 192
AXIAL_MAX_TAPS = 17


def _axial_kernel(w, who):
    if w.dim() != 5:
        raise StxError(f"{who}: expected a weight [Cout, Cin, kd, kh, kw], got shape {tuple(w.shape)}")
    kd, kh, kw = (int(k) for k in w.shape[2:])
    planar = (kd, kh, kw) == (1, 3, 3)
    axial = kh == 1 and kw == 1 and kd % 2 == 1 and 3 <= kd <= AXIAL_MAX_TAPS
    if not (planar or axial):
        raise StxError(f"{who}: kernel {(kd, kh, kw)} is not served -- (1,3,3) or (kd,1,1) with kd odd, 3 <= kd <= {AXIAL_MAX_TAPS}")
    if w.shape[0] > AXIAL_MAX_CHANNELS or w.shape[1] > AXIAL_MAX_CHANNELS:
        raise StxError(f"{who}: {w.shape[1]} -> {w.shape[0]} channels, at most {AXIAL_MAX_CHANNELS} are served")
    return kd, kh, kw


def pack_weight_axial(w, mode, owner=None):
    _chk(w, "weight", 5)
    kd, kh, kw = _axial_kernel(w, "pack_weight_axial")
    if owner is not None and _CACHE_ENABLED:
        cache = owner.__dict__.setdefault("_stx_packed", {})
        hit = cache.get(("axial", mode))
        if hit is not None and hit[0] == (owner._version, owner.data_ptr()):
            return hit[1]
    A, Bd = w.shape[0], w.shape[1]
    K, N = (Bd, A) if mode == 0 else (A, Bd)
    n = get_lib().raw("stx_conv3d_axial_packed_floats")(K, N, kd, kh, kw)
    if n <= 0:
        raise StxError(f"pack_weight_axial: GEMM-K {K} (a multiple of 4), N {N}, kernel {(kd, kh, kw)} unsupported")
    wp = torch.empty(n, dtype=torch.float32, device=w.device)
    _call("stx_conv3d_axial_pack_weight", _p(w), _p(wp), A, Bd, kd, kh, kw, mode)
    if owner is not None and _CACHE_ENABLED:
        cache[("axial", mode)] = ((owner._version, owner.data_ptr()), wp)
    return wp


def conv3d_axial_forward(x, wp, Cout, kernel, scale=None, bias=None, residual=None, act=0, want_stats=False):
    _chk(x, "x", 5)
    B, D, H, W, Cin = x.shape
    kd, kh, kw = kernel
    out = torch.empty(B, D, H, W, Cout, dtype=torch.float32, device=x.device)
    stats = None
    if want_stats:
        rows = get_lib().raw("stx_conv3d_axial_fwd_stat_rows")(B, D, H, W, Cin, Cout, kd, kh, kw)
        stats = torch.empty(rows, 2, Cout, dtype=torch.float32, device=x.device)
    _call("stx_conv3d_axial_fwd", _p(x), _p(wp), _p(out), _p(scale), _p(bias), _p(residual), _p(stats), B, D, H, W, Cin, Cout,
          kd, kh, kw, int(act))
    return out, stats


def conv3d_axial_wgrad(x, gz, kernel):
    B, D, H, W, CF = x.shape
    CC = gz.shape[-1]
    kd, kh, kw = kernel
    n = get_lib().raw("stx_conv3d_axial_wgrad_workspace_floats")(B, D, H, W, CF, CC, kd, kh, kw)
    if n <= 0:
        raise StxError(f"conv3d_axial_wgrad: {CF} x {CC} channels, kernel {kernel} unsupported")
    ws = _WS.get("axwgrad", n, x.device)
    dw = torch.empty(CC, CF, kd * kh * kw, dtype=torch.float32, device=x.device)
    _call("stx_conv3d_axial_wgrad", _p(x), _p(gz), _p(dw), _p(ws), B, D, H, W, CF, CC, kd, kh, kw)
    return dw


def _pad4(C):
    return (C + 3) // 4 * 4


def _axial_prepare(x, w, who):
    _chk(x, "x", 5)
    _chk(w, "weight", 5)
    kernel = _axial_kernel(w, who)
    if x.shape[-1] != w.shape[1]:
        raise StxError(f"{who}: input has {x.shape[-1]} channels, weight expects {w.shape[1]}")
    Cp = _pad4(w.shape[1])
    if Cp != w.shape[1]:
        x, w = _pad_channels(x, Cp), pad_weight_channels(w, Cp)
    return x, w, kernel


def _axial_backward(x, w, kernel, gz, cin_true, need_x, need_w):
    gz = gz.contiguous()
    Co, Ci = w.shape[0], w.shape[1]
    gz_k, w_k = gz, w
    if Co % 4:
        Cp = _pad4(Co)
        gz_k = _pad_channels(gz, Cp)
        w_k = w.new_zeros(Cp, *w.shape[1:])
        w_k[:Co] = w
    gx = gw = None
    if need_x:
        gx, _ = conv3d_axial_forward(gz_k, pack_weight_axial(w_k, 1), Ci, kernel)
        if Ci != cin_true:
            gx = gx[..., :cin_true].contiguous()
    if need_w:
        gw = conv3d_axial_wgrad(x, gz_k, kernel)[:Co, :cin_true].reshape(Co, cin_true, *kernel)
        if not gw.is_contiguous():
            gw = gw.contiguous()
    return gx, gw


class AxialConvRawFn(torch.autograd.Function):

    @staticmethod
    def forward(ctx, x, w, want_stats):
        ctx.cin_true = w.shape[1]
        x, w, kernel = _axial_prepare(x, w, "AxialConvRawFn")
        z, stats = conv3d_axial_forward(x, pack_weight_axial(w, 0), w.shape[0], kernel, want_stats=want_stats)
        ctx.save_for_backward(x, w)
        ctx.kernel = kernel
        if stats is None:
            stats = x.new_empty(0)
        ctx.mark_non_differentiable(stats)
        return z, stats

    @staticmethod
    def backward(ctx, gz, _gstats):
        x, w = ctx.saved_tensors
        gx, gw = _axial_backward(x, w, ctx.kernel, gz, ctx.cin_true, ctx.needs_input_grad[0], ctx.needs_input_grad[1])
        return gx, gw, None


class _AxialConvBiasFn(torch.autograd.Function):

    @staticmethod
    def forward(ctx, x, w, bias):
        ctx.cin_true = w.shape[1]
        x, w, kernel = _axial_prepare(x, w, "conv3d_axial")
        z, _ = conv3d_axial_forward(x, pack_weight_axial(w, 0), w.shape[0], kernel, bias=bias.contiguous())
        ctx.save_for_backward(x, w)
        ctx.kernel = kernel
        return z

    @staticmethod
    def backward(ctx, gz):
        x, w = ctx.saved_tensors
        gx, gw = _axial_backward(x, w, ctx.kernel, gz, ctx.cin_true, ctx.needs_input_grad[0], ctx.needs_input_grad[1])
        gb = gz.sum((0, 1, 2, 3)) if ctx.needs_input_grad[2] else None
        return gx, gw, gb


class ZeroGradBiasFn(torch.autograd.Function):

    @staticmethod
    def forward(ctx, z, bias):
        ctx.save_for_backward(bias)
        return z.view_as(z)

    @staticmethod
    def backward(ctx, gz):
        (bias,) = ctx.saved_tensors
        return gz, torch.zeros_like(bias)


@fp32_region
def conv3d_axial(x, weight, bias=None):
    _chk(x, "x", 5)
    _chk(weight, "weight", 5)
    _chk(bias, "bias", 1)
    _axial_kernel(weight, "conv3d_axial")
    if bias is not None and bias.shape[0] != weight.shape[0]:
        raise StxError(f"conv3d_axial: bias of {bias.shape[0]} for {weight.shape[0]} output channels")
    if torch.is_grad_enabled() and any(t is not None and t.requires_grad for t in (x, weight, bias)):
        if bias is None:
            return AxialConvRawFn.apply(x, weight, False)[0]
        return _AxialConvBiasFn.apply(x, weight, bias)
    xk, wk, kernel = _axial_prepare(x, weight.detach(), "conv3d_axial")
    return conv3d_axial_forward(xk, pack_weight_axial(wk, 0), weight.shape[0], kernel, bias=None if bias is None else bias.detach())[0]


CONVGRU_MAX_HIDDEN = 128
CONVGRU_MAX_K = 512
CONVGRU_MAX_X = 3
CONVGRU_PACKS = 0


def _cl_pitch(t):
    B, C, H, W = t.shape
    sb, sc, sh, sw = t.stride()
    if C > 1 and sc != 1:
        return None
    pitch = sw if W > 1 else (sh if H > 1 else (sb if B > 1 else C))
    if pitch < C or pitch % 4 or t.data_ptr() % 16:
        return None
    if (W > 1 and sw != pitch) or (H > 1 and sh != W * pitch) or (B > 1 and sb != H * W * pitch):
        return None
    return pitch


def _cl_source(t):
    pitch = _cl_pitch(t)
    if pitch is None:
        t = t.contiguous(memory_format=torch.channels_last)
        pitch = _cl_pitch(t)
        if pitch is None:
            t = t.permute(0, 2, 3, 1).contiguous().permute(0, 3, 1, 2)
            pitch = t.shape[1]
    return t, pitch


def _convgru_chk(t, name, like=None, channels=None, who="convgru"):
    if t is None:
        return
    if not on_device(t):
        raise StxError(f"{who}: {name}: expected a ROCm device tensor, got {t.device} -- the cell has no CPU fallback")
    if t.dtype != torch.float32:
        raise StxError(f"{who}: {name}: expected float32, got {t.dtype}")
    if like is not None:
        if t.dim() != 4 or t.shape[0] != like.shape[0] or tuple(t.shape[2:]) != tuple(like.shape[2:]):
            raise StxError(f"{who}: {name} has shape {tuple(t.shape)}, h has {tuple(like.shape)} (batch, H and W must agree)")
        if channels is not None and t.shape[1] != channels:
            raise StxError(f"{who}: {name} has {t.shape[1]} channels, expected {channels}")


def _convgru_pack(w0, w1, mode):
    global CONVGRU_PACKS
    key = tuple(v for w in (w0, w1) if w is not None for v in (w._version, w.data_ptr()))
    tag = ("convgru", mode, w1 is not None)
    if _CACHE_ENABLED:
        cache = w0.__dict__.setdefault("_stx_packed", {})
        hit = cache.get(tag)
        if hit is not None and hit[0] == key:
            return hit[1]
    A, Bd = w0.shape[0], w0.shape[1]
    nw = 1 if w1 is None else 2
    K, N = (Bd, nw * A) if mode == 0 else (nw * A, Bd)
    n = get_lib().raw("stx_convgru_packed_floats")(K, N)
    if n <= 0:
        raise StxError(f"convgru: GEMM-K {K} (a multiple of 4, <= {CONVGRU_MAX_K}) x N {N} unsupported")
    wp = torch.empty(n, dtype=torch.float32, device=w0.device)
    w0c, w1c = w0.detach().contiguous(), None if w1 is None else w1.detach().contiguous()
    _call("stx_convgru_pack_weight", _p(w0c), _p(w1c), _p(wp), A, Bd, mode)
    CONVGRU_PACKS += 1
    if _CACHE_ENABLED:
        cache[tag] = (key, wp)
    return wp


def _src_args(srcs):
    out = []
    for t, pitch in srcs:
        out += [_p(t), t.shape[1], pitch]
    for _ in range(4 - len(srcs)):
        out += [None, 0, 0]
    return out


def convgru_gemm(srcs, wp, N, B, H, W, epi=0, split=0, bias0=None, bias1=None, add0=None, add1=None, h=None, z=None, out0=None,
                 out1=None, out2=None, out_pitch=0):
    a0, a0p = add0 if add0 is not None else (None, 0)
    a1, a1p = add1 if add1 is not None else (None, 0)
    ht, hp = h if h is not None else (None, 0)
    _call("stx_convgru_gemm", *_src_args(srcs), _p(wp), N, epi, split, _p(bias0), _p(bias1), _p(a0), a0p, _p(a1), a1p, _p(ht), hp,
          _p(z), _p(out0), _p(out1), _p(out2), out_pitch, B, H, W)


def _nchw(t):
    return t.permute(0, 3, 1, 2)


class ConvGRUFn(torch.autograd.Function):

    @staticmethod
    def forward(ctx, h, cz, cr, cq, wz, bz, wr, br, wq, bq, *xs):
        B, hidden, H, W = h.shape
        dev = h.device
        need = any(ctx.needs_input_grad)
        hs = _cl_source(h.detach())
        xsrc = [_cl_source(x.detach()) for x in xs]
        cs = [None if c is None else _cl_source(c.detach()) for c in (cz, cr, cq)]
        new = lambda: torch.empty(B, H, W, hidden, dtype=torch.float32, device=dev)
        z, rh, hn = new(), new(), new()
        r = new() if need else None
        q = new() if need else None
        bzc, brc, bqc = (None if b is None else b.detach().contiguous() for b in (bz, br, bq))
        convgru_gemm([hs] + xsrc, _convgru_pack(wz, wr, 0), 2 * hidden, B, H, W, epi=1, split=hidden, bias0=bzc, bias1=brc,
                     add0=cs[0], add1=cs[1], h=hs, out0=z, out1=rh, out2=r)
        convgru_gemm([(_nchw(rh), hidden)] + xsrc, _convgru_pack(wq, None, 0), hidden, B, H, W, epi=2, split=hidden, bias0=bqc,
                     add0=cs[2], h=hs, z=z, out0=hn, out1=q)
        if need:
            ctx.save_for_backward(hs[0], z, r, q, rh, wz, wr, wq, *[t for t, _ in xsrc])
            ctx.pitches = (hs[1], [p for _, p in xsrc])
            ctx.has_c = [c is not None for c in (cz, cr, cq)]
            ctx.has_b = [b is not None for b in (bz, br, bq)]
        return _nchw(hn)

# ... 284 lines not shown
        small_last = ks_s == 1
        first, last = ((ks_l, wl), (ks_s, ws)) if small_last else ((ks_s, ws), (ks_l, wl))
        f = _raft_cell_fwd(first[0], hs, xsrc, first[1], need)
        l = _raft_cell_fwd(last[0], hs, xsrc, last[1], need, att=attc, other=f[4], blend=1 if small_last else 2)
        if need:
            ctx.save_for_backward(hs[0], attc, *f[:4], *l[:4], first[1][0], first[1][2], first[1][4], last[1][0], last[1][2],
                                  last[1][4], *[t for t, _ in xsrc])
            ctx.pitches = (hs[1], [p for _, p in xsrc])
            ctx.small_last = small_last
            ctx.ks = (first[0], last[0])
            ctx.has_b = [[w[i] is not None for i in (1, 3, 5)] for w in (first[1], last[1])]
        return _nchw(l[4])

    @staticmethod
    def backward(ctx, g):
        h, att, zf, rf, qf, rhf, zl, rl, ql, rhl, wzf, wrf, wqf, wzl, wrl, wql, *xt = ctx.saved_tensors
        hp, xp = ctx.pitches
        need = ctx.needs_input_grad
        B, hidden, H, W = h.shape
        dev = h.device
        P = B * H * W
        gt, gp = _cl_source(g)
        new = lambda: torch.empty(B, H, W, hidden, dtype=torch.float32, device=dev)
        g_s, g_l = new(), new()
        gatt = torch.empty(B, 1, H, W, dtype=torch.float32, device=dev) if need[0] else None
        (zs, qs), (zb, qb) = ((zl, ql), (zf, qf)) if ctx.small_last else ((zf, qf), (zl, ql))
        _call("stx_selgru_blend_bwd", _p(gt), gp, _p(att), _p(zs), _p(qs), _p(zb), _p(qb), _p(h), hp, _p(g_s), _p(g_l), _p(gatt),
              P, hidden)
        g_first, g_last = (g_l, g_s) if ctx.small_last else (g_s, g_l)
        o_first, o_last = (8, 2) if ctx.small_last else (2, 8)
        xsrc = list(zip(xt, xp))
        need_x = any(need[14:-1])
        outs = [None] * len(need)
        buf = None
        for ks, gc, o, has_b, (z, r, q, rh), w in ((ctx.ks[0], g_first, o_first, ctx.has_b[0], (zf, rf, qf, rhf), (wzf, wrf, wqf)),
                                                   (ctx.ks[1], g_last, o_last, ctx.has_b[1], (zl, rl, ql, rhl), (wzl, wrl, wql))):
            need_b = [need[o + i] and hb for i, hb in zip((1, 3, 5), has_b)]
            buf, dw, db = _raft_cell_bwd(ks, (_nchw(gc), hidden), (h, hp), z, r, q, rh, xsrc, w, need_x,
                                         [need[o], need[o + 2], need[o + 4]], need_b, prev=buf)
            outs[o:o + 6] = [dw[0], db[0], dw[1], db[1], dw[2], db[2]]
        outs[0] = gatt
        if need[1]:
            outs[1] = _nchw(buf[..., :hidden])
        outs[14:-1] = _x_grads(buf, hidden, [t.shape[1] for t in xt], need[14:-1])
        return tuple(outs)


def _raft_chk(who, h, x_list, cells):
    x_list = list(x_list)
    if h is None or h.dim() != 4:
        raise StxError(f"{who}: h must be a tensor [B, hidden, H, W]")
    _convgru_chk(h, "h", who=who)
    hidden = h.shape[1]
    if not 1 <= len(x_list) <= CONVGRU_MAX_X:
        raise StxError(f"{who}: {len(x_list)} x sources; 1..{CONVGRU_MAX_X} are served (4 sources with h)")
    for i, x in enumerate(x_list):
        _convgru_chk(x, f"x[{i}]", like=h, who=who)
    cx = [int(x.shape[1]) for x in x_list]
    K = hidden + sum(cx)
    sizes = []
    for cell in cells:
        if len(cell) != 6 or cell[0] is None or cell[0].dim() != 4:
            raise StxError(f"{who}: a cell is (wz, bz, wr, br, wq, bq) with weights [hidden, K, k, k]")
        ks = int(cell[0].shape[-1])
        if ks not in (1, 3):
            raise StxError(f"{who}: kernel size {ks}; 1x1 and 3x3 cells are served")
        for name, w, b in zip(("wz", "wr", "wq"), cell[0::2], cell[1::2]):
            _convgru_chk(w, name, who=who)
            _convgru_chk(b, "bias of " + name, who=who)
            if w.dim() != 4 or tuple(w.shape) != (hidden, K, ks, ks):
                raise StxError(f"{who}: {name} has shape {tuple(w.shape)}, expected {(hidden, K, ks, ks)}")
            if b is not None and tuple(b.shape) != (hidden,):
                raise StxError(f"{who}: bias of {name} has shape {tuple(b.shape)}, expected {(hidden,)}")
        sizes.append(ks)
    cx3 = cx + [0] * (3 - len(cx))
    lib = get_lib()
    if not (lib.raw("stx_selgru_supported")(hidden, len(cx), *cx3) and lib.raw("stx_convgru_supported")(hidden, len(cx), *cx3, 3)):
        raise StxError(f"{who}: hidden {hidden} (a multiple of 16, <= {CONVGRU_MAX_HIDDEN}) with x channels {cx} (multiples of 4, "
                       f"hidden + sum <= {CONVGRU_MAX_K}) is not served")
    return sizes


@fp32_region
def raft_convgru(h, x_list, wz, bz, wr, br, wq, bq):
    ks, = _raft_chk("raft_convgru", h, x_list, [(wz, bz, wr, br, wq, bq)])
    if ks == 3:
        return ConvGRUFn.apply(h, None, None, None, wz, bz, wr, br, wq, bq, *x_list)
    return RaftConvGRU1x1Fn.apply(h, wz, bz, wr, br, wq, bq, *x_list, torch.is_grad_enabled())


@fp32_region
def selective_convgru(att, h, x_list, small, large):
    who = "selective_convgru"
    small, large = tuple(small), tuple(large)
    ks_s, ks_l = _raft_chk(who, h, x_list, [small, large])
    if ks_s != 1 and ks_l != 1:
        raise StxError(f"{who}: kernel sizes {ks_s} and {ks_l}; one of the two cells must be 1x1")
    if att is None or att.dim() != 4:
        raise StxError(f"{who}: att must be a tensor [B, 1, H, W]")
    _convgru_chk(att, "att", like=h, channels=1, who=who)
    return SelectiveConvGRUFn.apply(att, h, *small, *large, *x_list, torch.is_grad_enabled())


CSA_MAX_C = 256
CSA_MAX_KERNEL = 7


def _csa_chk(who, x, w1=None, w2=None, w_sam=None):
    for name, t in (("x", x), ("w1", w1), ("w2", w2), ("w_sam", w_sam)):
        if t is None:
            continue
        if not on_device(t):
            raise StxError(f"{who}: {name}: expected a ROCm device tensor, got {t.device} -- the attention has no CPU fallback")
        if t.dtype != torch.float32:
            raise StxError(f"{who}: {name}: expected float32, got {t.dtype}")
        if t.dim() != 4:
            raise StxError(f"{who}: {name} has shape {tuple(t.shape)}, expected 4 dims")
    B, C, H, W = x.shape
    k = None if w_sam is None else int(w_sam.shape[-1])
    if min(B, H, W) < 1 or not get_lib().raw("stx_csa_supported")(C, 1 if k is None else k):
        raise StxError(f"{who}: {C} channels (a multiple of 16, <= {CSA_MAX_C}) with a {k} x {k} kernel (odd, <= {CSA_MAX_KERNEL}) on "
                       f"{tuple(x.shape)} is not served")
    if w1 is not None and (tuple(w1.shape) != (C // 16, C, 1, 1) or w2 is None or tuple(w2.shape) != (C, C // 16, 1, 1)):
        raise StxError(f"{who}: the MLP weights have shapes {tuple(w1.shape)} and {None if w2 is None else tuple(w2.shape)}, expected "
                       f"{(C // 16, C, 1, 1)} and {(C, C // 16, 1, 1)}")
    if w_sam is not None and tuple(w_sam.shape) != (1, 2, k, k):
        raise StxError(f"{who}: w_sam has shape {tuple(w_sam.shape)}, expected {(1, 2, k, k)}")
    return B, C, H, W, k


def _csa_pool(xs, pitch, B, C, HW):
    nblk = get_lib().raw("stx_csa_blocks")(HW, C)
    dev = xs.device
    psum = torch.empty(B, nblk, C, dtype=torch.float64, device=dev)
    pmax = torch.empty(B, nblk, C, dtype=torch.float32, device=dev)
    pidx = torch.empty(B, nblk, C, dtype=torch.int32, device=dev)
    _call("stx_csa_pool", _p(xs), pitch, _p(psum), _p(pmax), _p(pidx), B, HW, C)
    return nblk, psum, pmax, pidx


def _csa_gate_state(B, C, dev):
    return (torch.empty(B, C, dtype=torch.float32, device=dev), torch.empty(B, 2, C, dtype=torch.float64, device=dev),
            torch.empty(B, C, dtype=torch.int32, device=dev))


def _csa_sam_bwd(g, att, cmap, w, need_w):
    B, _, H, W = att.shape
    k = w.shape[-1]
    dev = att.device
    gc = g.contiguous()
    gpre = torch.empty(B, H, W, dtype=torch.float32, device=dev)
    gmap = torch.empty(B, H, W, 2, dtype=torch.float32, device=dev)
    dw = torch.empty(1, 2, k, k, dtype=torch.float32, device=dev) if need_w else None
    ws = _WS.get("csa_sam_bwd", get_lib().raw("stx_csa_sam_bwd_workspace_floats")(B, H, W, k), dev) if need_w else None
    _call("stx_csa_sam_bwd", _p(gc), _p(att), _p(cmap), _p(w), _p(gpre), _p(gmap), _p(dw), _p(ws), B, H, W, k)
    return gmap, dw


def _csa_gate_bwd(pgate, nblk, gg, pooled, argp, w1, w2, gx, accumulate, need_w1, need_w2, need_x, HW):
    B, C = argp.shape
    dev = argp.device
    dw1 = torch.empty(C // 16, C, 1, 1, dtype=torch.float32, device=dev) if need_w1 else None
    dw2 = torch.empty(C, C // 16, 1, 1, dtype=torch.float32, device=dev) if need_w2 else None
    gavg = torch.empty(B, C, dtype=torch.float32, device=dev)
    gmx = torch.empty(B, C, dtype=torch.float32, device=dev)
    _call("stx_csa_gate_bwd", _p(pgate), nblk, _p(gg), _p(pooled), _p(w1), _p(w2), _p(dw1), _p(dw2), _p(gavg), _p(gmx), B, HW, C)
    if need_x:
        _call("stx_csa_pool_bwd", _p(gx), _p(gavg), _p(gmx), _p(argp), 1 if accumulate else 0, B, HW, C)
    return dw1, dw2


class CsaFn(torch.autograd.Function):

    @staticmethod
    def forward(ctx, x, w1, w2, w_sam, track):
        B, C, H, W = x.shape
        k = w_sam.shape[-1]
        dev = x.device
        need = track and any(ctx.needs_input_grad)
        xs, pitch = _cl_source(x.detach())
        w1c, w2c, wsc = w1.detach().contiguous(), w2.detach().contiguous(), w_sam.detach().contiguous()
        nblk, psum, pmax, pidx = _csa_pool(xs, pitch, B, C, H * W)
        xp = torch.empty(B, H, W, C, dtype=torch.float32, device=dev)
        cmap = torch.empty(B, H, W, 2, dtype=torch.float32, device=dev)
        argc = torch.empty(B, H, W, dtype=torch.int32, device=dev) if need else None
        gate, pooled, argp = _csa_gate_state(B, C, dev) if need else (None, None, None)
        _call("stx_csa_apply", _p(xs), pitch, _p(psum), _p(pmax), _p(pidx), nblk, _p(w1c), _p(w2c), _p(xp), _p(cmap), _p(argc),
              _p(gate), _p(pooled), _p(argp), B, H * W, C)
        att = torch.empty(B, 1, H, W, dtype=torch.float32, device=dev)
        _call("stx_csa_sam", _p(cmap), _p(wsc), _p(att), B, H, W, k)
        if need:
            ctx.save_for_backward(xs, gate, pooled, argp, argc, cmap, att, w1c, w2c, wsc)
            ctx.pitch, ctx.nblk = pitch, nblk
            ctx.set_materialize_grads(False)
        return _nchw(xp), att

    @staticmethod
    def backward(ctx, gxp, gatt):
        xs, gate, pooled, argp, argc, cmap, att, w1, w2, wsam = ctx.saved_tensors
        need = ctx.needs_input_grad
        B, C, H, W = xs.shape
        dev = xs.device
        gmap = dws = None
        if gatt is not None:
            gmap, dws = _csa_sam_bwd(gatt, att, cmap, wsam, need[3])
        if not any(need[:3]) or (gxp is None and gmap is None):
            return None, None, None, dws, None
        gs, gpitch = _cl_source(gxp) if gxp is not None else (None, 0)
        gx = torch.empty(B, H, W, C, dtype=torch.float32, device=dev)
        pgate = torch.empty(B, ctx.nblk, C, dtype=torch.float64, device=dev)
        _call("stx_csa_apply_bwd", _p(xs), ctx.pitch, _p(gate), _p(gs), gpitch, _p(gmap), _p(argc), _p(gx), _p(pgate), B, H * W, C)
        dw1, dw2 = _csa_gate_bwd(pgate, ctx.nblk, None, pooled, argp, w1, w2, gx, True, need[1], need[2], need[0], H * W)
        return _nchw(gx) if need[0] else None, dw1, dw2, dws, None


class CsaGateFn(torch.autograd.Function):

    @staticmethod
    def forward(ctx, x, w1, w2):
        B, C, H, W = x.shape
        dev = x.device
        xs, pitch = _cl_source(x.detach())
        w1c, w2c = w1.detach().contiguous(), w2.detach().contiguous()
        nblk, psum, pmax, pidx = _csa_pool(xs, pitch, B, C, H * W)
        gate, pooled, argp = _csa_gate_state(B, C, dev)
        _call("stx_csa_gate", _p(psum), _p(pmax), _p(pidx), nblk, _p(w1c), _p(w2c), _p(gate), _p(pooled), _p(argp), B, H * W, C)
        if any(ctx.needs_input_grad):
            ctx.save_for_backward(pooled, argp, w1c, w2c)
            ctx.hw = (H, W)
        return gate.view(B, C, 1, 1)

    @staticmethod
    def backward(ctx, g):
        pooled, argp, w1, w2 = ctx.saved_tensors
        need = ctx.needs_input_grad
        B, C = argp.shape
        H, W = ctx.hw
        gg = g.reshape(B, C).contiguous()
        gx = torch.empty(B, H, W, C, dtype=torch.float32, device=argp.device) if need[0] else None
        dw1, dw2 = _csa_gate_bwd(None, 0, gg, pooled, argp, w1, w2, gx, False, need[1], need[2], need[0], H * W)
        return None if gx is None else _nchw(gx), dw1, dw2


class CsaSpatialFn(torch.autograd.Function):

    @staticmethod
    def forward(ctx, x, w, track):
        B, C, H, W = x.shape
        k = w.shape[-1]
        dev = x.device
        need = track and any(ctx.needs_input_grad)
        xs, pitch = _cl_source(x.detach())
        wc = w.detach().contiguous()
        cmap = torch.empty(B, H, W, 2, dtype=torch.float32, device=dev)
        argc = torch.empty(B, H, W, dtype=torch.int32, device=dev) if need else None
        _call("stx_csa_apply", _p(xs), pitch, None, None, None, 0, None, None, None, _p(cmap), _p(argc), None, None, None, B, H * W, C)
        att = torch.empty(B, 1, H, W, dtype=torch.float32, device=dev)
        _call("stx_csa_sam", _p(cmap), _p(wc), _p(att), B, H, W, k)
        if need:
            ctx.save_for_backward(argc, cmap, att, wc)
            ctx.C = C
        return att

    @staticmethod
    def backward(ctx, g):
        argc, cmap, att, w = ctx.saved_tensors
        need = ctx.needs_input_grad
        B, _, H, W = att.shape
        gmap, dw = _csa_sam_bwd(g, att, cmap, w, need[1])
        gx = None
        if need[0]:
            gx = torch.empty(B, H, W, ctx.C, dtype=torch.float32, device=att.device)
            _call("stx_csa_apply_bwd", None, 0, None, None, 0, _p(gmap), _p(argc), _p(gx), None, B, H * W, ctx.C)
        return None if gx is None else _nchw(gx), dw, None


@fp32_region
def csa_gate(x, w1, w2):
    _csa_chk("csa_gate", x, w1, w2)
    return CsaGateFn.apply(x, w1, w2)


@fp32_region
def csa_spatial(x, w):
    _csa_chk("csa_spatial", x, w_sam=w)
    return CsaSpatialFn.apply(x, w, torch.is_grad_enabled())


@fp32_region
def csa(x, w1, w2, w_sam):
    _csa_chk("csa", x, w1, w2, w_sam)
    return CsaFn.apply(x, w1, w2, w_sam, torch.is_grad_enabled())


class SharedInputConvsFn(torch.autograd.Function):

    @staticmethod
    def forward(ctx, x, cfgs, *ws):
        _chk(x, "x", 5)
        outs = []
        for (ks, stride, want), w in zip(cfgs, ws):
            if x.shape[-1] != w.shape[1] or w.shape[1] % 8 or w.shape[0] % 8 or _is_c1(w, ks, stride, False):
                raise StxError(f"SharedInputConvsFn: weight {tuple(w.shape)} on an input of {x.shape[-1]} channels")
            z, stats = conv3d_forward(x, pack_weight(w, 0), w.shape[0], ks, stride, want_stats=want)
            if stats is None:
                stats = x.new_empty(0)
            ctx.mark_non_differentiable(stats)
            outs += [z, stats]
        ctx.save_for_backward(x, *ws)
        ctx.cfgs = cfgs
        return tuple(outs)

    @staticmethod
    def backward(ctx, *grads):
        x, ws = ctx.saved_tensors[0], ctx.saved_tensors[1:]
        B, D, H, W, Ci = x.shape
        gws = [None] * len(ws)
        gzs = []
        for k, g in enumerate(grads[0::2]):
            pend = _take_pending_bn(g)
            if pend is not None:
                ks, stride, _ = ctx.cfgs[k]
                if (ctx.needs_input_grad[2 + k] and ks == 3 and stride == 1
                        and get_lib().raw("stx_conv3d_wgrad_bn_supported")(B, D, H, W, Ci, ws[k].shape[0])):
                    gw, g = conv3d_wgrad_bn(x, g, pend)
                    gws[k] = gw.reshape(ws[k].shape)
                else:
                    g = pend.materialize()
            gzs.append(None if g is None else g.contiguous())
        gx = None
        if ctx.needs_input_grad[0]:
            rank = lambda k: (0 if ctx.cfgs[k][0] == 3 and ctx.cfgs[k][1] == 1 else (1 if ctx.cfgs[k][1] == 2 else 2))
            for k in sorted((k for k in range(len(ws)) if gzs[k] is not None), key=rank):
                (ks, stride, _), w, gz = ctx.cfgs[k], ws[k], gzs[k]
                if stride == 1:
                    gx, _ = conv3d_forward(gz, pack_weight(w, 1), Ci, ks, 1, residual=gx)
                else:
                    Co = w.shape[0]
                    gz_k, w_k = gz, w
                    if Co % 32:
                        Cp = (Co + 31) // 32 * 32
                        gz_k = _pad_channels(gz, Cp)
                        w_k = w.new_zeros(Cp, *w.shape[1:])
                        w_k[:Co] = w
                    gx, _ = deconv3d_forward(gz_k, pack_weight(w_k, 2), Ci, out_dims=(D, H, W), residual=gx)
        for k, (w, gz) in enumerate(zip(ws, gzs)):
            if gz is None or not ctx.needs_input_grad[2 + k] or gws[k] is not None:
                continue
            ks, stride, _ = ctx.cfgs[k]
            Co = w.shape[0]
            gz_w = gz if Co % 32 == 0 else _pad_channels(gz, (Co + 31) // 32 * 32)
            x_w = x if Ci % 32 == 0 else _pad_channels(x, (Ci + 31) // 32 * 32)
            gws[k] = conv3d_wgrad(x_w, gz_w, ks, stride)[:Co, :Ci].reshape(w.shape)
        return (gx, None, *gws)


_D4_SEL = ((3, 1, 4), (4, 2, 0))


def embed_deconv4_weight(w):
    Ci, Co = w.shape[0], w.shape[1]
    wz = torch.cat((w, w.new_zeros(Ci, Co, 1, 4, 4)), 2)
    wz = torch.cat((wz, wz.new_zeros(Ci, Co, 5, 1, 4)), 3)
    wz = torch.cat((wz, wz.new_zeros(Ci, Co, 5, 5, 1)), 4)
    parts = []
    for pd in (0, 1):
        for ph in (0, 1):
            for pw in (0, 1):
                sel = wz[:, :, list(_D4_SEL[pd])][:, :, :, list(_D4_SEL[ph])][:, :, :, :, list(_D4_SEL[pw])]
                parts.append(sel.transpose(0, 1))
    return torch.cat(parts, 0).contiguous()


class DepthToSpaceFn(torch.autograd.Function):

    @staticmethod
    def forward(ctx, y):
        y = y.contiguous()
        _chk(y, "y", 5)
        B, D, H, W, C8 = y.shape
        C = C8 // 8
        out = torch.empty(B, 2 * D, 2 * H, 2 * W, C, dtype=torch.float32, device=y.device)
        _call("stx_depth_to_space", _p(y), _p(out), B, D, H, W, C, 0)
        return out

    @staticmethod
    def backward(ctx, g):
        g = g.contiguous()
        B, D2, H2, W2, C = g.shape
        gy = torch.empty(B, D2 // 2, H2 // 2, W2 // 2, 8 * C, dtype=torch.float32, device=g.device)
        _call("stx_depth_to_space", _p(g), _p(gy), B, D2 // 2, H2 // 2, W2 // 2, C, 1)
        return gy


def _d4_chunks(Co):
    per = max(1, min(8, 128 // Co))
    return [(c0, min(8, c0 + per)) for c0 in range(0, 8, per)]


def deconv4_raw(x, w, want_stats):
    Co = w.shape[1]
    if Co % 4:
        raise StxError(f"ConvTranspose3d(k4): {Co} output channels (need a multiple of 4)")
    w3 = embed_deconv4_weight(w)
    ys = [ConvRawFn.apply(x, w3[c0 * Co:c1 * Co], 3, 1, False, False)[0] for c0, c1 in _d4_chunks(Co)]
    z = DepthToSpaceFn.apply(ys[0] if len(ys) == 1 else torch.cat(ys, -1))
    return z, (bn_stats(z.detach()) if want_stats else z.new_empty(0))


@fp32_region
def deconv4_forward(x, w, scale=None, bias=None, relu=0, owner=None):
    _chk(x, "x", 5)
    Co = w.shape[1]
    if Co % 4:
        raise StxError(f"ConvTranspose3d(k4): {Co} output channels (need a multiple of 4)")
    cache = owner.__dict__.setdefault("_stx_packed", {}) if (owner is not None and _CACHE_ENABLED) else None
    key = (owner._version, owner.data_ptr()) if owner is not None else None
    hit = cache.get("d4") if cache is not None else None
    if hit is not None and hit[0] == key:
        packed = hit[1]
    else:
        w3 = embed_deconv4_weight(w)
        packed = [pack_weight(w3[c0 * Co:c1 * Co].contiguous(), 0) for c0, c1 in _d4_chunks(Co)]
        if cache is not None:
            cache["d4"] = (key, packed)
    ys = []
    for (c0, c1), wp in zip(_d4_chunks(Co), packed):
        n = c1 - c0
        ys.append(conv3d_forward(x, wp, n * Co, 3, 1, None if scale is None else scale.repeat(n),
                                 None if bias is None else bias.repeat(n), None, relu)[0])
    B, D, H, W, _ = x.shape
    y = ys[0] if len(ys) == 1 else torch.cat(ys, -1)
    out = torch.empty(B, 2 * D, 2 * H, 2 * W, Co, dtype=torch.float32, device=x.device)
    _call("stx_depth_to_space", _p(y), _p(out), B, D, H, W, Co, 0)
    return out


class GateFn(torch.autograd.Function):

    @staticmethod
    def forward(ctx, cv, att):
        out = gate(cv.detach(), att.detach())
        ctx.save_for_backward(cv, att)
        return out

    @staticmethod
    def backward(ctx, g):
        cv, att = ctx.saved_tensors
        g = g.contiguous()
        B, D, H, W, C = cv.shape
        gcv = torch.empty_like(cv) if ctx.needs_input_grad[0] else None
        gatt = torch.empty_like(att) if ctx.needs_input_grad[1] else None
        if gcv is not None or gatt is not None:
            _call("stx_gate_bwd", _p(g), _p(cv), _p(att), _p(gcv), _p(gatt), B, D, H * W, C)
        return gcv, gatt


@fp32_region
def gate(cv, att):
    if torch.is_grad_enabled() and (cv.requires_grad or att.requires_grad):
        return GateFn.apply(cv.contiguous(), att.contiguous())
    cv, att = cv.contiguous(), att.contiguous()
    _chk(cv, "cv", 5)
    _chk(att, "att", 4)
    B, D, H, W, C = cv.shape
    if att.shape != (B, H, W, C) or C % 4:
        raise StxError(f"gate: volume {tuple(cv.shape)} vs gate {tuple(att.shape)} (need [B,H,W,C], C % 4 == 0)")
    out = torch.empty_like(cv)
    _call("stx_gate_fwd", _p(cv), _p(att), _p(out), B, D, H * W, C)
    return out


class ChannelMajorFn(torch.autograd.Function):

    @staticmethod
    def forward(ctx, x):
        B, C, H, W = x.shape
        out = torch.empty((B, C, H, W), dtype=x.dtype, device=x.device)
        _call("stx_transpose", _p(x.permute(0, 2, 3, 1)), _p(out), B, H * W, C)
        return out

    @staticmethod
    def backward(ctx, g):
        g = g.contiguous()
        B, C, H, W = g.shape
        gx = torch.empty((B, H, W, C), dtype=g.dtype, device=g.device)
        _call("stx_transpose", _p(g), _p(gx), B, C, H * W)
        return gx.permute(0, 3, 1, 2)


@fp32_region
def channel_major(x):
    if x.is_contiguous():
        return x
    if (x.dim() == 4 and x.dtype == torch.float32 and on_device(x) and x.is_contiguous(memory_format=torch.channels_last)
            and x.shape[1] % 4 == 0 and (x.shape[2] * x.shape[3]) % 4 == 0):
        return ChannelMajorFn.apply(x)
    return x.contiguous()


class CatChannelsFn(torch.autograd.Function):

    @staticmethod
    def forward(ctx, *parts):
        ctx.cs = [int(p.shape[-1]) for p in parts]
        nvox = parts[0].numel() // ctx.cs[0]
        out = parts[0].new_empty(*parts[0].shape[:-1], sum(ctx.cs))
        ptrs = [_p(p) for p in parts] + [None] * (4 - len(parts))
        cs = ctx.cs + [0] * (4 - len(parts))
        _call("stx_concat_channels", *ptrs, *cs, _p(out), nvox)
        return out

    @staticmethod
    def backward(ctx, g):
        g = g.contiguous()
        nvox = g.numel() // g.shape[-1]
        outs = [g.new_empty(*g.shape[:-1], c) if need else None for c, need in zip(ctx.cs, ctx.needs_input_grad)]
        if any(o is not None for o in outs):
            dst = [o if o is not None else g.new_empty(*g.shape[:-1], c) for o, c in zip(outs, ctx.cs)]
            ptrs = [_p(o) for o in dst] + [None] * (4 - len(dst))
            cs = ctx.cs + [0] * (4 - len(dst))
            _call("stx_split_channels", _p(g), *ptrs, *cs, nvox)
        return tuple(outs)


@fp32_region
def cat_channels(parts):
    parts = [p.contiguous() for p in parts]
    if not 2 <= len(parts) <= 4:
        raise StxError(f"cat_channels: {len(parts)} parts (2 to 4)")
    lead = parts[0].shape[:-1]
    for p in parts:
        if p.shape[:-1] != lead or p.shape[-1] % 4 or p.dtype != torch.float32 or p.device != parts[0].device:
            raise StxError(f"cat_channels: parts {[tuple(q.shape) for q in parts]} (equal leading shape, fp32, widths % 4 == 0)")
    return CatChannelsFn.apply(*parts)


def conv2d_supported(conv):
    return (conv.kernel_size == (3, 3) and conv.stride == (1, 1) and conv.padding == (1, 1) and conv.dilation == (1, 1)
            and conv.groups == 1 and conv.bias is None and conv.in_channels in (32, 64) and conv.out_channels in (32, 64))


def _ohwi(w):
    v = w.permute(0, 2, 3, 1)
    return v if v.is_contiguous() else v.contiguous()


def conv2d_forward(x, w, dgrad=False, groups=1, want_stats=False):
    _chk(x, "x", 4)
    wo = _ohwi(w)
    _chk(wo, "weight", 4)
    B, H, W, Cin = x.shape
    Co, Ci = w.shape[0], w.shape[1]
    Kin, Nout = (Co, Ci) if dgrad else (Ci, Co)
    if Cin != Kin or B % groups:
        raise StxError(f"conv2d: input {tuple(x.shape)} against weight {tuple(w.shape)} (dgrad={dgrad}, groups={groups})")
    out = torch.empty(B, H, W, Nout, dtype=torch.float32, device=x.device)
    part = None
    if want_stats:
        rows = int(get_lib().raw("stx_conv2d_stat_rows")(groups))
        part = torch.empty(rows, 2, Nout, dtype=torch.float32, device=x.device)
    _call("stx_conv2d_fwd", _p(x), _p(wo), _p(out), _p(part), B, H, W, Kin, Nout, int(dgrad), groups)
    if part is not None and groups > 1:
        part = part.view(groups, rows // groups, 2, Nout)
    return out, part


class Conv2dFn(torch.autograd.Function):

    @staticmethod
    def forward(ctx, x, w, groups):
        xl = x.permute(0, 2, 3, 1)
        if not xl.is_contiguous():
            xl = xl.contiguous()
        z, part = conv2d_forward(xl, w, False, groups, True)
        ctx.save_for_backward(x, w)
        ctx.mark_non_differentiable(part)
        return z, part

    @staticmethod
    def backward(ctx, gz, _gpart):
        x, w = ctx.saved_tensors
        gz = gz.contiguous()
        gx = gw = None
        if ctx.needs_input_grad[0]:
            gx = conv2d_forward(gz, w, True)[0].permute(0, 3, 1, 2)
        if ctx.needs_input_grad[1]:
            gw = torch.ops.aten.convolution_backward(gz.permute(0, 3, 1, 2), x, w, None, (1, 1), (1, 1), (1, 1), False, (0, 0), 1,
                                                     (False, True, False))[1]
        return gx, gw, None


def bn_finalize(partials, count, gamma, beta, running_mean, running_var, momentum, eps, groups=1):
    C = partials.shape[-1]
    out = torch.empty(4, groups, C, dtype=torch.float32, device=partials.device)
    _call("stx_bn_finalize_groups", _p(partials), partials.shape[-3], C, float(count), _p(gamma), _p(beta),
          _p(running_mean), _p(running_var), float(momentum), float(eps), _p(out), groups)
    return list(out.unbind(0)) if groups > 1 else list(out[:, 0].unbind(0))


@fp32_region
def bn_stats(z, groups=1):
    _chk(z, "z")
    C = z.shape[-1]
    nvox = z.numel() // C // groups
    if groups < 1 or z.shape[0] % groups:
        raise StxError(f"bn_stats: leading axis {z.shape[0]} does not split into {groups} groups")
    rows = get_lib().raw("stx_bn_stats_rows")(nvox, C)
    if rows <= 0:
        raise StxError(f"bn_stats: C={C} unsupported")
    part = torch.empty(groups, rows, 2, C, dtype=torch.float32, device=z.device)
    _call("stx_bn_stats", _p(z), _p(part), nvox, C, groups)
    return part if groups > 1 else part[0]


def _sync_bn_partials(partials, count, group, world):
    import torch.distributed as dist
    tot = partials.double().sum(0)
    dist.all_reduce(tot, group=group)
    hi = tot.float()
    lo = (tot - hi.double()).float()
    return torch.stack((hi, lo)).contiguous(), count * world


@fp32_region
def bn_apply(z1, scale1, shift1, z2=None, scale2=None, shift2=None, relu=False, groups=1):
    out = torch.empty_like(z1)
    C = z1.shape[-1]
    _call("stx_bn_apply", _p(z1), _p(scale1), _p(shift1), _p(z2), _p(scale2), _p(shift2), _p(out),
          z1.numel() // C // groups, C, int(relu), groups)
    return out


class BnActFn(torch.autograd.Function):

    @staticmethod
    def forward(ctx, z1, gamma1, beta1, z2, gamma2, beta2, residual, relu, bn1, bn2, groups=1, defer=False):
        G = int(groups)
        ctx.defer = bool(defer)

        def affine(gamma, beta, bn):
            if bn["training"]:
                partials, count = bn["partials"], bn["count"]
                if bn.get("sync"):
                    if G > 1:
                        raise StxError("BnActFn: SyncBatchNorm with groups is not wired (SyncBN runs the views separately)")
                    partials, count = _sync_bn_partials(partials, count, *bn["sync"])
                return bn_finalize(partials, count, gamma, beta, bn["running_mean"], bn["running_var"], bn["momentum"],
                                   bn["eps"], G)
            invstd = torch.rsqrt(bn["running_var"] + bn["eps"])
            scale = gamma * invstd
            res = (scale, beta - bn["running_mean"] * scale, bn["running_mean"].clone(), invstd)
            return res if G == 1 else [t.unsqueeze(0).expand(G, -1).contiguous() for t in res]

        relu = int(relu)
        if relu == 2 and residual is not None:
            raise StxError("BnActFn: Mish with a plain residual is not wired (no model of the family uses it)")
        if G < 1 or z1.shape[0] % G:
            raise StxError(f"BnActFn: leading axis {z1.shape[0]} does not split into {G} groups")
        sc1, sh1, m1, i1 = affine(gamma1, beta1, bn1)
        two = z2 is not None
        if two:
            sc2, sh2, m2, i2 = affine(gamma2, beta2, bn2)
            y = bn_apply(z1, sc1, sh1, z2, sc2, sh2, relu, G)
        else:
            sc2 = sh2 = m2 = i2 = None
            y = bn_apply(z1, sc1, sh1, residual, None, None, relu, G)
        ctx.relu, ctx.two, ctx.has_res, ctx.groups = relu, two, residual is not None, G
        ctx.train1 = bn1["training"]
        ctx.train2 = bn2["training"] if two else False
        ctx.sync = bn1.get("sync") or (bn2.get("sync") if two else None)
        ctx.remask = bool(relu) and residual is None
        keep_y = y if (relu and not ctx.remask) else None
        ctx.save_for_backward(z1, gamma1, m1, i1, z2, gamma2, m2, i2, keep_y, sc1 if ctx.remask else None,
                              sh1 if ctx.remask else None, sc2 if (ctx.remask and two) else None,
                              sh2 if (ctx.remask and two) else None)
        return y

    @staticmethod
    def backward(ctx, gy):
        z1, gamma1, m1, i1, z2, gamma2, m2, i2, y, sc1, sh1, sc2, sh2 = ctx.saved_tensors
        gy = gy.contiguous()
        G = ctx.groups
        C = z1.shape[-1]
        nvox = z1.numel() // C // G
        lib = get_lib()
        NB = lib.raw("stx_bn_reduce_blocks")()
        part = _WS.get("bnred", G * NB * 3 * C, z1.device)
        sums_all = torch.empty(G + (1 if G > 1 else 0), 3, C, dtype=torch.float32, device=z1.device)
        sums = sums_all[:G]
        _call("stx_bn_bwd_reduce2", _p(gy), _p(y), _p(z1), _p(m1), _p(i1), _p(z2) if ctx.two else None,
              _p(m2) if ctx.two else None, _p(i2) if ctx.two else None, _p(sc1), _p(sh1), _p(sc2), _p(sh2), _p(part),
              _p(sums_all), nvox, C, int(ctx.relu), G)
        if not ctx.needs_input_grad[0] and not ctx.two and not ctx.has_res:
            tot = sums_all[G] if G > 1 else sums_all[0]
            return (None, tot[1], tot[0], None, None, None, None, None, None, None, None, None)
        if (ctx.defer and not ctx.two and not ctx.has_res and ctx.relu in (0, 1) and ctx.train1 and not ctx.sync and G == 1
                and (not ctx.relu or ctx.remask)):
            alias = gy.view_as(gy)
            pend = _PendingBn()
            pend.g, pend.z, pend.scale, pend.shift, pend.mean, pend.invstd = alias, z1, sc1, sh1, m1, i1
            pend.gamma, pend.sums, pend.inv_n, pend.act = gamma1, sums, 1.0 / nvox, int(ctx.relu)
            if pend.scale is None:
                pend.scale = pend.shift = m1
            _defer_pending_bn(alias, pend)
            tot = sums_all[0]
            return (alias, tot[1], tot[0], None, None, None, None, None, None, None, None, None)
        dz1 = torch.empty_like(z1)
        dz2 = torch.empty_like(z2) if ctx.two else None
        gres = torch.empty_like(z1) if (ctx.has_res and ctx.relu) else None
        use = sums
        if ctx.sync:
            import torch.distributed as dist
            use = sums.clone()
            dist.all_reduce(use, group=ctx.sync[0])
            use /= ctx.sync[1]
        if not ctx.train1 or (ctx.two and not ctx.train2):
            use = torch.zeros_like(sums)
        _call("stx_bn_bwd_apply2", _p(gy), _p(y), _p(z1), _p(m1), _p(i1), _p(gamma1), _p(z2) if ctx.two else None,
              _p(m2) if ctx.two else None, _p(i2) if ctx.two else None, _p(gamma2) if ctx.two else None, _p(sc1), _p(sh1),
              _p(sc2), _p(sh2), _p(use), _p(dz1), _p(dz2), _p(gres), nvox, C, int(ctx.relu), G)
        if ctx.has_res and not ctx.relu:
            gres = gy
        tot = sums_all[G] if G > 1 else sums_all[0]
        return (dz1, tot[1], tot[0], dz2, tot[2] if ctx.two else None, tot[0].clone() if ctx.two else None, gres,
                None, None, None, None, None)


class MishFn(torch.autograd.Function):

    @staticmethod
    def forward(ctx, x):
        x = x.contiguous()
        _chk(x, "x")
        y = torch.empty_like(x)
        _call("stx_mish_fwd", _p(x), _p(y), x.numel())
        ctx.save_for_backward(x)
        return y

    @staticmethod
    def backward(ctx, gy):
        (x,) = ctx.saved_tensors
        gy = gy.contiguous()
        gx = torch.empty_like(x)
        _call("stx_mish_bwd", _p(gy), _p(x), _p(gx), x.numel())
        return gx


@fp32_region
def mish(x):
    if torch.is_grad_enabled() and x.requires_grad:
        return MishFn.apply(x)
    x = x.contiguous()
    _chk(x, "x")
    y = torch.empty_like(x)
    _call("stx_mish_fwd", _p(x), _p(y), x.numel())
    return y


def _cv_shapes(Lg, Lc, num_groups):
    ref = Lg if Lg is not None else Lc
    B, _, H, W = ref.shape
    Cg = Lg.shape[1] if Lg is not None else 0
    Cc = Lc.shape[1] if Lc is not None else 0
    G = num_groups if Lg is not None else 0
    return B, H, W, Cg, G, Cc


@fp32_region
def cost_volume_forward(Lg, Rg, Lc, Rc, maxdisp, num_groups, mask_left=True, scale=None):
    for n, t in (("ref gwc", Lg), ("tgt gwc", Rg), ("ref concat", Lc), ("tgt concat", Rc)):
        _chk(t, n, 4)
    B, H, W, Cg, G, Cc = _cv_shapes(Lg, Lc, num_groups)
    if G:
        assert Cg % G == 0
    vol = torch.empty(B, maxdisp, H, W, G + 2 * Cc, dtype=torch.float32, device=(Lg if Lg is not None else Lc).device)
    _call("stx_cost_volume_fwd", _p(Lg), _p(Rg), Cg, G, _p(Lc), _p(Rc), Cc, _p(scale), _p(vol), B, H, W, maxdisp,
          int(mask_left))
    return vol


class CostVolumeFn(torch.autograd.Function):

    @staticmethod
    def forward(ctx, Lg, Rg, Lc, Rc, maxdisp, num_groups, mask_left):
        ctx.save_for_backward(Lg, Rg)
        ctx.cfg = (maxdisp, num_groups, mask_left, None if Lc is None else Lc.shape)
        return cost_volume_forward(Lg, Rg, Lc, Rc, maxdisp, num_groups, mask_left)

    @staticmethod
    def backward(ctx, gvol):
        Lg, Rg = ctx.saved_tensors
        maxdisp, num_groups, mask_left, cshape = ctx.cfg
        gvol = gvol.contiguous()
        B, D, H, W, CT = gvol.shape
        Cg = Lg.shape[1] if Lg is not None else 0
        G = num_groups if Lg is not None else 0
        Cc = cshape[1] if cshape is not None else 0
        gLg = torch.empty_like(Lg) if G else None
        gRg = torch.empty_like(Rg) if G else None
        gLc = gvol.new_empty(cshape) if Cc else None
        gRc = gvol.new_empty(cshape) if Cc else None
        _call("stx_cost_volume_bwd", _p(gvol), _p(Lg), _p(Rg), Cg, G, Cc, _p(gLg), _p(gRg), _p(gLc), _p(gRc), B, H, W,
              D, int(mask_left))
        return gLg, gRg, gLc, gRc, None, None, None


class GroupNormalizeFn(torch.autograd.Function):

    @staticmethod
    def forward(ctx, x, num_groups, out_scale):
        x = x.contiguous()
        _chk(x, "x", 4)
        B, C, H, W = x.shape
        y = torch.empty_like(x)
        _call("stx_group_normalize_fwd", _p(x), _p(y), B, C, num_groups, H * W, float(out_scale))
        ctx.save_for_backward(x)
        ctx.cfg = (num_groups, float(out_scale))
        return y

    @staticmethod
    def backward(ctx, gy):
        (x,) = ctx.saved_tensors
        gy = gy.contiguous()
        B, C, H, W = x.shape
        gx = torch.empty_like(x)
        _call("stx_group_normalize_bwd", _p(x), _p(gy), _p(gx), B, C, ctx.cfg[0], H * W, ctx.cfg[1])
        return gx, None, None


@fp32_region
def group_normalize(x, num_groups, out_scale=1.0):
    assert x.dim() == 4 and x.shape[1] % num_groups == 0, f"C:{x.shape[1]}, num_groups:{num_groups}"
    return GroupNormalizeFn.apply(channel_major(x), num_groups, out_scale)


@fp32_region
def cost_volume(Lg, Rg, Lc, Rc, maxdisp, num_groups, mask_left=True, normalize=False):
    if normalize and Lg is not None:
        Lg = group_normalize(Lg, num_groups, float(Lg.shape[1] // num_groups))
        Rg = group_normalize(Rg, num_groups, 1.0)
    ts = [channel_major(t) if t is not None else None for t in (Lg, Rg, Lc, Rc)]
    if torch.is_grad_enabled() and any(t is not None and t.requires_grad for t in ts):
        return CostVolumeFn.apply(*ts, maxdisp, num_groups, mask_left)
    return cost_volume_forward(*ts, maxdisp, num_groups, mask_left)


class SampledVolumeFn(torch.autograd.Function):

    @staticmethod
    def forward(ctx, Lg, Rg, Lc, Rc, samples, num_groups):
        B, H, W, Cg, G, Cc = _cv_shapes(Lg, Lc, num_groups)
        S = samples.shape[1]
        CTp = (G + 2 * Cc + 1 + 7) // 8 * 8
        vol = torch.empty(B, S, H, W, CTp, dtype=torch.float32, device=samples.device)
        _call("stx_sampled_volume_fwd", _p(Lg), _p(Rg), Cg, G, _p(Lc), _p(Rc), Cc, _p(samples), _p(vol), B, H, W, S, CTp)
        ctx.save_for_backward(Lg, Rg, samples)
        ctx.cfg = (G, Cg, Cc, None if Lc is None else Lc.shape)
        return vol

    @staticmethod
    def backward(ctx, gvol):
        Lg, Rg, samples = ctx.saved_tensors
        G, Cg, Cc, cshape = ctx.cfg
        gvol = gvol.contiguous()
        B, S, H, W, CTp = gvol.shape
        gLg = torch.empty_like(Lg) if G else None
        gRg = torch.empty_like(Rg) if G else None
        gLc = gvol.new_empty(cshape) if Cc else None
        gRc = gvol.new_empty(cshape) if Cc else None
        _call("stx_sampled_volume_bwd", _p(gvol), _p(Lg), _p(Rg), Cg, G, Cc, _p(samples), _p(gLg), _p(gRg), _p(gLc),
              _p(gRc), B, H, W, S, CTp)
        return gLg, gRg, gLc, gRc, None, None


@fp32_region
def sampled_volume(Lg, Rg, Lc, Rc, samples, num_groups):
    ts = [channel_major(t) if t is not None else None for t in (Lg, Rg, Lc, Rc)]
    for n, t in (("ref gwc", ts[0]), ("tgt gwc", ts[1]), ("ref concat", ts[2]), ("tgt concat", ts[3])):
        _chk(t, n, 4)
    samples = samples.detach().contiguous()
    _chk(samples, "samples", 4)
    if ts[0] is not None:
        assert ts[0].shape[1] % num_groups == 0
    if torch.is_grad_enabled() and any(t is not None and t.requires_grad for t in ts):
        return SampledVolumeFn.apply(*ts, samples, num_groups)
    return SampledVolumeFn.forward(_NoCtx(), *ts, samples, num_groups)


class _NoCtx:

    def save_for_backward(self, *a):
        pass
# ... 1919 lines not shown
```

Baseline: 0.1787 pairs/s.

## Batch conv3d weight packing, fuse skip-gradient add into conv2d dgrad, prefetch BN reduce

Result: no change. 0.1787 pairs/s (+0.0%).

```diff
diff --git a/include/stx_hip.h b/include/stx_hip.h
--- a/include/stx_hip.h
+++ b/include/stx_hip.h
@@ -36,6 +36,13 @@
 
 long long stx_conv3d_packed_floats(int K, int N, int T);
 int stx_conv3d_pack_weight(const float* w, float* wp, int A, int B, int T, int mode, void* stream);
+typedef struct StxPackRecord {
+    const float* src;
+    float* dst;
+    long long start;
+    int A, B, T, mode;
+} StxPackRecord;
+int stx_conv3d_pack_many(const void* table, int n, long long total, void* stream);
 int stx_conv3d_fwd_blocks(int Do, int Ho, int Wo);
 long long stx_conv3d_fwd_stat_rows(int B, int Di, int Hi, int Wi, int Cin, int Cout, int ks, int stride);
 int stx_conv3d_fwd(const float* x, const float* wp, float* out, const float* scale, const float* bias,
@@ -126,6 +133,8 @@
 long long stx_conv2d_stat_rows(int groups);
 int stx_conv2d_fwd(const float* x, const float* w, float* out, float* stats, int B, int H, int W, int Cin, int Cout, int dgrad,
                    int groups, void* stream);
+int stx_conv2d_dgrad_add(const float* gy, const float* w, const float* add, float* out, int B, int H, int W, int Cin, int Cout,
+                         void* stream);
 
 int stx_conv3d_c1_fwd(const float* x, const float* w, const float* residual, float* out, int B, int D, int H, int W,
                       int Cin, void* stream);
diff --git a/stereo_toolbox_amd/_capi.py b/stereo_toolbox_amd/_capi.py
--- a/stereo_toolbox_amd/_capi.py
+++ b/stereo_toolbox_amd/_capi.py
@@ -31,6 +31,7 @@
     "stx_split_mode": [_P, _P, _P, _I, _I, _I, _P],
     "stx_conv3d_packed_floats": [_I, _I, _I],
     "stx_conv3d_pack_weight": [_P, _P, _I, _I, _I, _I, _P],
+    "stx_conv3d_pack_many": [_P, _I, _L, _P],
     "stx_conv3d_fwd_blocks": [_I, _I, _I],
     "stx_conv3d_fwd_stat_rows": [_I, _I, _I, _I, _I, _I, _I, _I],
     "stx_deconv3d_fwd_blocks": [_I, _I, _I],
@@ -80,6 +81,7 @@
     "stx_conv2d_supported": [_I, _I],
     "stx_conv2d_stat_rows": [_I],
     "stx_conv2d_fwd": [_P, _P, _P, _P, _I, _I, _I, _I, _I, _I, _I, _P],
+    "stx_conv2d_dgrad_add": [_P, _P, _P, _P, _I, _I, _I, _I, _I, _P],
     "stx_conv3d_c1_fwd": [_P, _P, _P, _P, _I, _I, _I, _I, _I, _P],
     "stx_conv3d_c1_wgrad_workspace_floats": [_I],
     "stx_conv3d_c1_wgrad": [_P, _P, _P, _P, _I, _I, _I, _I, _I, _P],
diff --git a/stereo_toolbox_amd/csrc/bn.hip b/stereo_toolbox_amd/csrc/bn.hip
--- a/stereo_toolbox_amd/csrc/bn.hip
+++ b/stereo_toolbox_amd/csrc/bn.hip
@@ -1,5 +1,7 @@
 #include "stx_common.h"
 #include <stdlib.h>
+
+extern "C" int stx_get_tuning(const char* name);
 
 namespace {
 
@@ -141,6 +143,7 @@
     }
 }
 
+template <bool PF>
 __global__ __launch_bounds__(BN_THREADS) void bn_bwd_reduce_kernel(
     const float* __restrict__ gy, const float* __restrict__ y, const float* __restrict__ z1,
     const float* __restrict__ mean1, const float* __restrict__ invstd1, const float* __restrict__ z2,
@@ -174,22 +177,14 @@
     float s[12];
 #pragma unroll
     for (int k = 0; k < 12; ++k) s[k] = 0.f;
-    for (size_t v = vl < VPB ? (size_t)blockIdx.x * VPB + vl : nvox; v < nvox; v += (size_t)gridDim.x * VPB) {
-        const size_t o = v * C + 4 * cq;
-        float4 g = stx_ld4(gy + o);
-        const float4 a = stx_ld4(z1 + o);
-        float4 c = make_float4(0.f, 0.f, 0.f, 0.f);
-        if (has2) c = stx_ld4(z2 + o);
+    auto consume = [&](float4 g, const float4 a, const float4 c, float4 yy) {
         if (relu) {
-            float4 yy;
             if (remask) {
                 yy.x = fmaf(a.x, a1.x, b1.x); yy.y = fmaf(a.y, a1.y, b1.y); yy.z = fmaf(a.z, a1.z, b1.z); yy.w = fmaf(a.w, a1.w, b1.w);
                 if (has2) {
                     yy.x += fmaf(c.x, a2.x, b2.x); yy.y += fmaf(c.y, a2.y, b2.y);
                     yy.z += fmaf(c.z, a2.z, b2.z); yy.w += fmaf(c.w, a2.w, b2.w);
                 }
-            } else {
-                yy = stx_ld4(y + o);
             }
             g.x = stx_act_bwd(g.x, yy.x, relu); g.y = stx_act_bwd(g.y, yy.y, relu);
             g.z = stx_act_bwd(g.z, yy.z, relu); g.w = stx_act_bwd(g.w, yy.w, relu);
@@ -201,6 +196,32 @@
             s[8] = fmaf(g.x, (c.x - m2.x) * i2.x, s[8]); s[9] = fmaf(g.y, (c.y - m2.y) * i2.y, s[9]);
             s[10] = fmaf(g.z, (c.z - m2.z) * i2.z, s[10]); s[11] = fmaf(g.w, (c.w - m2.w) * i2.w, s[11]);
         }
+    };
+    const bool ready = relu && !remask;
+    const float4 zero4 = make_float4(0.f, 0.f, 0.f, 0.f);
+    const size_t step = (size_t)gridDim.x * VPB;
+    size_t v = vl < VPB ? (size_t)blockIdx.x * VPB + vl : nvox;
+    if constexpr (PF) {
+        for (; v + 3 * step < nvox; v += 4 * step) {
+            float4 g[4], a[4], c[4], yy[4];
+#pragma unroll
+            for (int u = 0; u < 4; ++u) {
+                const size_t o = (v + u * step) * C + 4 * cq;
+                g[u] = stx_ld4(gy + o);
+                a[u] = stx_ld4(z1 + o);
+                c[u] = has2 ? stx_ld4(z2 + o) : zero4;
+                yy[u] = ready ? stx_ld4(y + o) : zero4;
+            }
+#pragma unroll
+            for (int u = 0; u < 4; ++u) consume(g[u], a[u], c[u], yy[u]);
+        }
+    }
+    for (; v < nvox; v += step) {
+        const size_t o = v * C + 4 * cq;
+        const float4 g = stx_ld4(gy + o);
+        const float4 a = stx_ld4(z1 + o);
+        const float4 c = has2 ? stx_ld4(z2 + o) : zero4;
+        consume(g, a, c, ready ? stx_ld4(y + o) : zero4);
     }
 #pragma unroll
     for (int k = 0; k < 12; ++k) red[k * BN_THREADS + tid] = s[k];
@@ -424,8 +445,10 @@
                 "bn_bwd_reduce: the relu mask needs y or the forward pass's scale / shift vectors");
     STX_REQUIRE(relu != 2 || !y, "bn_bwd_reduce: Mish (activation code 2) differentiates the pre-activation value: pass y = NULL and the scale / shift vectors");
     hipStream_t st = (hipStream_t)stream;
-    const int nblk = ((long long)nvox * C <= (9ll << 19)) ? BN_RED_BLOCKS / 4 : BN_RED_BLOCKS;
-    hipLaunchKernelGGL(bn_bwd_reduce_kernel, dim3(nblk, groups), dim3(BN_THREADS), 0, st, gy, y, z1, mean1, invstd1,
+    const bool small = (long long)nvox * C <= (9ll << 19);
+    const int nblk = small ? BN_RED_BLOCKS / 4 : BN_RED_BLOCKS;
+    auto kern = small && stx_get_tuning("STX_BN_RED_PF") ? bn_bwd_reduce_kernel<true> : bn_bwd_reduce_kernel<false>;
+    hipLaunchKernelGGL(kern, dim3(nblk, groups), dim3(BN_THREADS), 0, st, gy, y, z1, mean1, invstd1,
                        z2, mean2, invstd2, scale1, shift1, scale2, shift2, partials, (size_t)nvox, C, relu);
     int rc = stx_check_launch("bn_bwd_reduce");
     if (rc) return rc;
diff --git a/stereo_toolbox_amd/csrc/conv2d.hip b/stereo_toolbox_amd/csrc/conv2d.hip
--- a/stereo_toolbox_amd/csrc/conv2d.hip
+++ b/stereo_toolbox_amd/csrc/conv2d.hip
@@ -13,17 +13,20 @@
     int B, H, W, Cin, Cout;
     int nHt, nWt, groups;
     int dgrad;
+    const float* add;
 };
 
 __device__ __forceinline__ f32x4 c2_zero4() { f32x4 z = {0.f, 0.f, 0.f, 0.f}; return z; }
 
-template <int KQ, int ABL = 0, int PAD = 8>
+template <int KQ, int ABL = 0, int PAD = 8, bool ADD = false>
 __global__ __launch_bounds__(C2_THREADS) void conv2d_march_kernel(Conv2dArgs a) {
     constexpr int CIN = 16 * KQ, VS = CIN + PAD, F4 = CIN / 4;
     constexpr int WFLOATS = 9 * KQ * 256;
     constexpr int NST = (C2_NV * F4 + C2_THREADS - 1) / C2_THREADS;
     constexpr int SLOT = (NST * C2_THREADS / F4) * VS;
     constexpr int NSTEP = 9 * KQ;
+    constexpr int AST = NST > 10 ? NST : 10;
+    static_assert(!ADD || AST + 1 < NSTEP - NST, "the add loads sit between the staging loads and the LDS writes");
     STX_DYN_SMEM(smem);
     float* wl = reinterpret_cast<float*>(smem);
     float* bufs = wl + WFLOATS;
@@ -103,14 +106,20 @@
     unsigned pvoff[2] = {STX_BUF_OOB, STX_BUF_OOB}, cvoff[2] = {STX_BUF_OOB, STX_BUF_OOB};
     stx_bufrsrc prs = stx_make_rsrc(a.out, 0u);
     float s1[4] = {0.f, 0.f, 0.f, 0.f}, s2[4] = {0.f, 0.f, 0.f, 0.f};
+    float4 padd[2], cadd[2];
+    padd[0] = padd[1] = cadd[0] = cadd[1] = make_float4(0.f, 0.f, 0.f, 0.f);
     auto emit_prev = [&](int r) {
         f32x4 v = r ? pacc1 : pacc0;
         const bool ok = (int)pvoff[r] >= 0;
-#pragma unroll
-        for (int c = 0; c < 4; ++c) {
-            v[c] = ok ? v[c] : 0.f;
-            s1[c] += v[c];
-            s2[c] = fmaf(v[c], v[c], s2[c]);
+        if constexpr (ADD) {
+            v[0] += padd[r].x; v[1] += padd[r].y; v[2] += padd[r].z; v[3] += padd[r].w;
+        } else {
+#pragma unroll
+            for (int c = 0; c < 4; ++c) {
+                v[c] = ok ? v[c] : 0.f;
+                s1[c] += v[c];
+                s2[c] = fmaf(v[c], v[c], s2[c]);
+            }
         }
         stx_buf_st4(prs, pvoff[r], 0u, make_float4(v[0], v[1], v[2], v[3]));
     };
@@ -153,6 +162,7 @@
         const long long norg = (long long)(noh0 - 1) * a.W + (now0 - 1), img = (long long)a.H * a.W;
         const stx_bufrsrc nrs = stx_make_rsrc(a.x + ((long long)nb * img + norg) * CIN, more ? (unsigned)((img - norg) * CIN * 4) : 0u);
         const stx_bufrsrc crs = stx_make_rsrc(a.out + (size_t)b * img * a.Cout, (unsigned)(img * a.Cout * 4));
+        const stx_bufrsrc ars = stx_make_rsrc(ADD ? a.add + (size_t)b * img * a.Cout : a.out, ADD ? (unsigned)(img * a.Cout * 4) : 0u);
         const float* pbuf = bufs + cur * SLOT;
         float* nbuf = bufs + (cur ^ 1) * SLOT;
         f32x4 acc0, acc1;
@@ -190,6 +200,9 @@
                 const int oh = oh0 + 2 * wave + r, ow = ow0 + i;
                 cvoff[r] = (unsigned)((((oh * a.W + ow) * a.Cout) + 16 * slice + 4 * kg) * 4) | (((oh < a.H) & (ow < a.W)) ? 0u : STX_BUF_OOB);
             }
+            if constexpr (ADD) {
+                if (st == AST || st == AST + 1) cadd[st - AST] = stx_buf_ld4(ars, cvoff[st - AST], 0u);
+            }
             if (st >= NSTEP - NST) {
                 const int k = st - (NSTEP - NST);
                 const int e = tid + k * C2_THREADS;
@@ -209,6 +222,7 @@
         prs = crs;
         pvoff[0] = cvoff[0]; pvoff[1] = cvoff[1];
         pacc0 = acc0; pacc1 = acc1;
+        if constexpr (ADD) { padd[0] = cadd[0]; padd[1] = cadd[1]; }
         if (!(ABL & 8)) __syncthreads();
         if (more && nslice != slice) {
             emit_prev(0); emit_prev(1);
@@ -257,7 +271,7 @@
     STX_REQUIRE((long long)(H + 2) * W * (Cin > Cout ? Cin : Cout) * 4 < (1ll << 31), "conv2d_fwd: image too large for one descriptor");
     STX_REQUIRE(H < 32768 && W < 32768, "conv2d_fwd: image too large");
     Conv2dArgs a;
-    a.x = x; a.w = w; a.out = out; a.stats = stats; a.dgrad = dgrad;
+    a.x = x; a.w = w; a.out = out; a.stats = stats; a.dgrad = dgrad; a.add = nullptr;
     a.B = B; a.H = H; a.W = W; a.Cin = Cin; a.Cout = Cout;
     a.nHt = stx_cdiv(H, C2_TH); a.nWt = stx_cdiv(W, C2_TW); a.groups = groups;
     const int grid = conv2d_grid(groups);
@@ -276,3 +290,23 @@
     hipLaunchKernelGGL(k, dim3(grid), dim3(C2_THREADS), lds, (hipStream_t)stream, a);
     return stx_check_launch("conv2d_fwd");
 }
+
+extern "C" int stx_conv2d_dgrad_add(const float* gy, const float* w, const float* add, float* out, int B, int H, int W, int Cin,
+                                    int Cout, void* stream) {
+    if (!add) return stx_conv2d_fwd(gy, w, out, nullptr, B, H, W, Cin, Cout, 1, 1, stream);
+    stx_begin();
+    STX_REQUIRE(gy && w && out && B > 0 && H > 0 && W > 0, "conv2d_dgrad_add: bad args");
+    STX_REQUIRE(add != out, "conv2d_dgrad_add: `add` must not be the output buffer (it is read one unit ahead of the stores)");
+    STX_REQUIRE(stx_conv2d_supported(Cin, Cout), "conv2d_dgrad_add: %d -> %d channels unsupported (Cin 32 or 64, Cout a multiple of 16)", Cin, Cout);
+    STX_REQUIRE((long long)(H + 2) * W * (Cin > Cout ? Cin : Cout) * 4 < (1ll << 31), "conv2d_dgrad_add: image too large for one descriptor");
+    STX_REQUIRE(H < 32768 && W < 32768, "conv2d_dgrad_add: image too large");
+    Conv2dArgs a;
+    a.x = gy; a.w = w; a.out = out; a.stats = nullptr; a.dgrad = 1; a.add = add;
+    a.B = B; a.H = H; a.W = W; a.Cin = Cin; a.Cout = Cout;
+    a.nHt = stx_cdiv(H, C2_TH); a.nWt = stx_cdiv(W, C2_TW); a.groups = 1;
+    const size_t lds = ((size_t)9 * Cin * 16 + (size_t)2 * 192 * (Cin + 8) + (size_t)2 * Cout) * 4;
+    void (*k)(Conv2dArgs) = Cin == 64 ? conv2d_march_kernel<4, 0, 8, true> : conv2d_march_kernel<2, 0, 8, true>;
+    if (int rc = stx_lds_require((const void*)k, lds, "conv2d_dgrad_add")) return rc;
+    hipLaunchKernelGGL(k, dim3(conv2d_grid(1)), dim3(C2_THREADS), lds, (hipStream_t)stream, a);
+    return stx_check_launch("conv2d_dgrad_add");
+}
diff --git a/stereo_toolbox_amd/csrc/conv3d_pack.hip b/stereo_toolbox_amd/csrc/conv3d_pack.hip
--- /dev/null
+++ b/stereo_toolbox_amd/csrc/conv3d_pack.hip
@@ -0,0 +1,54 @@
+#include "stx_common.h"
+
+namespace {
+
+constexpr int PACK_THREADS = 256;
+
+struct PackRecord {
+    const float* src;
+    float* dst;
+    long long start;
+    int A, Bd, T, mode;
+};
+
+__global__ __launch_bounds__(PACK_THREADS) void conv3d_pack_many_kernel(const PackRecord* __restrict__ table, int n, size_t total) {
+    const size_t gidx = (size_t)blockIdx.x * PACK_THREADS + threadIdx.x;
+    if (gidx >= total) return;
+    int lo = 0, hi = n - 1;
+    while (lo < hi) {
+        const int mid = (lo + hi + 1) >> 1;
+        if ((size_t)table[mid].start <= gidx) lo = mid; else hi = mid - 1;
+    }
+    const PackRecord rec = table[lo];
+    const size_t idx = gidx - (size_t)rec.start;
+    const int A = rec.A, Bd = rec.Bd, T = rec.T, mode = rec.mode;
+    const int K = (mode == 0) ? Bd : A, N = (mode == 0) ? A : Bd;
+    const int NT = N <= 32 ? 1 : (N <= 64 ? 2 : 4);
+    const int j = idx & 3, lane = (idx >> 2) & 63;
+    size_t r = idx >> 8;
+    const int nt = r % NT; r /= NT;
+    const int NQ = K / 8;
+    const int q = r % NQ;
+    const size_t tap = r / NQ;
+    if (tap >= (size_t)T) return;
+    const int k = 8 * q + 4 * (lane >> 5) + j, nn = 32 * nt + (lane & 31);
+    float v = 0.f;
+    if (nn < N && k < K) {
+        if (mode == 0) v = rec.src[((size_t)nn * Bd + k) * T + tap];
+        else if (mode == 1) v = rec.src[((size_t)k * Bd + nn) * T + (T - 1 - tap)];
+        else v = rec.src[((size_t)k * Bd + nn) * T + tap];
+    }
+    rec.dst[idx] = v;
+}
+
+}
+
+extern "C" int stx_conv3d_pack_many(const void* table, int n, long long total, void* stream) {
+    stx_begin();
+    STX_REQUIRE(table && n > 0 && total > 0 && total % 256 == 0, "conv3d_pack_many: bad args (n %d, total %lld)", n, total);
+    STX_REQUIRE(total / PACK_THREADS < (1ll << 31), "conv3d_pack_many: %lld packed elements exceed one grid", total);
+    static_assert(sizeof(PackRecord) == 40, "PackRecord is the 40-byte StxPackRecord of include/stx_hip.h");
+    hipLaunchKernelGGL(conv3d_pack_many_kernel, dim3((unsigned)((total + PACK_THREADS - 1) / PACK_THREADS)), dim3(PACK_THREADS), 0,
+                       (hipStream_t)stream, (const PackRecord*)table, n, (size_t)total);
+    return stx_check_launch("conv3d_pack_many");
+}
diff --git a/stereo_toolbox_amd/csrc/stx_runtime.hip b/stereo_toolbox_amd/csrc/stx_runtime.hip
--- a/stereo_toolbox_amd/csrc/stx_runtime.hip
+++ b/stereo_toolbox_amd/csrc/stx_runtime.hip
@@ -46,11 +46,11 @@
 #include <string.h>
 namespace {
 struct TuneEntry { const char* name; int value; };
-constexpr int TUNE_N = STX_TUNE_COUNT + 1;
+constexpr int TUNE_N = STX_TUNE_COUNT + 2;
 TuneEntry g_tune[TUNE_N] = {
     {"STX_MARCH_BS", 1}, {"STX_MARCH_EPI", 1}, {"STX_MARCH_ABLATE", 0}, {"STX_WGRAD_ABLATE", 0}, {"STX_WGRAD_MARCH", 3}, {"STX_WGRAD_GRID", 0}, {"STX_CONV_L1_MARCH", 0}, {"STX_CONV_S2_DENSE", 1}, {"STX_CONV_WN", 2},
     {"STX_CV_OLD", 0}, {"STX_CV_GRID", 0}, {"STX_CV_PF", 0}, {"STX_CV_UNITS", 1}, {"STX_CV_WIN", 0}, {"STX_CVB_OLD", 0}, {"STX_CVB_TEAM", 0}, {"STX_CVB_GRID", 0}, {"STX_CVB_NSET", 3},
-    {"STX_SV_BWD_V1", 0}, {"STX_DWCONV_ROLL", 1}, {"STX_C2_PAD", 8}, {"STX_C2_ABLATE", 0}, {"STX_DA_GRID", 0},
+    {"STX_SV_BWD_V1", 0}, {"STX_DWCONV_ROLL", 1}, {"STX_C2_PAD", 8}, {"STX_C2_ABLATE", 0}, {"STX_DA_GRID", 0}, {"STX_BN_RED_PF", 1},
 };
 struct TuneInit {
     TuneInit() {
diff --git a/stereo_toolbox_amd/models/features2d.py b/stereo_toolbox_amd/models/features2d.py
--- a/stereo_toolbox_amd/models/features2d.py
+++ b/stereo_toolbox_amd/models/features2d.py
@@ -70,11 +70,20 @@
             and ops.conv2d_supported(conv) and x.shape[0] % view_groups.current() == 0)
 
 
-def conv_bn_act(x, conv, bn, relu=False, residual=None, second=None):
+def skip_in_dgrad(x, conv, bn):
+    return (os.environ.get("STX_FEAT2D_DGRAD_ADD", "1") != "0" and bn.training and torch.is_grad_enabled() and x.requires_grad
+            and own_conv2d(x, conv))
+
+
+def conv_bn_act(x, conv, bn, relu=False, residual=None, second=None, want_skip=False):
     G = view_groups.current()
     part = None
+    skip = None
     if bn.training and own_conv2d(x, conv):
-        zl, part = ops.Conv2dFn.apply(x, conv.weight, G)
+        if want_skip:
+            zl, part, skip = ops.Conv2dFn.apply(x, conv.weight, G, True)
+        else:
+            zl, part = ops.Conv2dFn.apply(x, conv.weight, G)
         z = zl.permute(0, 3, 1, 2)
     else:
         z = F.conv2d(x, conv.weight, conv.bias, conv.stride, conv.padding, conv.dilation, conv.groups)
@@ -99,7 +108,7 @@
     else:
         y = ops.BnActFn.apply(zl, bn.weight, bn.bias, None, None, None, None if residual is None else _nhwc(residual),
                               relu, st, None, G)
-    return y.permute(0, 3, 1, 2)
+    return (y.permute(0, 3, 1, 2), skip) if want_skip else y.permute(0, 3, 1, 2)
 
 
 def convbn_relu_chain(seq, x):
@@ -145,6 +154,9 @@
     def forward(self, x):
         bns = [self.conv1[0][1], self.conv2[1]] + ([self.downsample[1]] if self.downsample is not None else [])
         if fused_glue(x, *bns):
+            if self.downsample is None and skip_in_dgrad(x, self.conv1[0][0], self.conv1[0][1]):
+                y, xs = conv_bn_act(x, self.conv1[0][0], self.conv1[0][1], relu=True, want_skip=True)
+                return conv_bn_act(y, self.conv2[0], self.conv2[1], residual=xs)
             y = conv_bn_act(x, self.conv1[0][0], self.conv1[0][1], relu=True)
             if self.downsample is None:
                 return conv_bn_act(y, self.conv2[0], self.conv2[1], residual=x)
diff --git a/stereo_toolbox_amd/ops.py b/stereo_toolbox_amd/ops.py
--- a/stereo_toolbox_amd/ops.py
+++ b/stereo_toolbox_amd/ops.py
@@ -119,6 +119,7 @@
 def set_weight_cache(enabled):
     global _CACHE_ENABLED
     _CACHE_ENABLED = bool(enabled)
+    _PACK_STATE.clear()
 
 
 def invalidate_caches(model):
@@ -126,6 +127,112 @@
         m.__dict__.pop("_stx_fold", None)
     for p in model.parameters():
         p.__dict__.pop("_stx_packed", None)
+        p.__dict__.pop("_stx_pack_train", None)
+    _PACK_STATE.clear()
+
+
+_PACK_STATE = {}
+_PACK_TABLES = {}
+
+
+def _pack_batch_enabled():
+    import os
+    return os.environ.get("STX_PACK_BATCH", "1") != "0"
+
+
+def _packed_floats(shape, mode):
+    A, Bd = shape[0], shape[1]
+    T = shape[2] * shape[3] * shape[4]
+    K, N = (Bd, A) if mode == 0 else (A, Bd)
+    return A, Bd, T, int(get_lib().raw("stx_conv3d_packed_floats")(K, N, T))
+
+
+class _PackTable:
+    RECORD = 5
+
+    def __init__(self, n, device):
+        self.host = torch.empty(n * self.RECORD, dtype=torch.int64).pin_memory() if device.type == "cuda" else \
+            torch.empty(n * self.RECORD, dtype=torch.int64)
+        self.dev = torch.empty(n * self.RECORD, dtype=torch.int64, device=device)
+        self.event = None
+        self.key = None
+
+    def fill(self, items, outs):
+        if self.event is not None:
+            self.event.synchronize()
+        key = [(o.data_ptr(), o.shape, m) for o, m, _ in items]
+        rows = self.host.view(-1, self.RECORD)
+        if key != self.key:
+            start, recs = 0, []
+            for o, m, (A, Bd, T, n) in items:
+                recs.append((o.data_ptr(), 0, start, A | (Bd << 32), T | (m << 32)))
+                start += n
+            rows.copy_(torch.tensor(recs, dtype=torch.int64))
+            self.key = key
+        rows[:, 1] = torch.tensor([t.data_ptr() for t in outs], dtype=torch.int64)
+        self.dev.copy_(self.host, non_blocking=True)
+        if self.dev.is_cuda:
+            self.event = torch.cuda.Event()
+            self.event.record(torch.cuda.current_stream(self.dev.device))
+
+
+def _pack_batch(device):
+    st = _PACK_STATE[device]
+    items = []
+    for key, ref in list(st["reg"].items()):
+        o = ref()
+        if o is None or o.device != device or not o.is_contiguous() or o.dtype != torch.float32 or o.dim() != 5:
+            del st["reg"][key]
+            continue
+        items.append((o, key[1], _packed_floats(o.shape, key[1])))
+    st["dirty"] = False
+    if not items:
+        return
+    total = sum(it[2][3] for it in items)
+    outs = [torch.empty(it[2][3], dtype=torch.float32, device=device) for it in items]
+    sid = torch.cuda.current_stream(device).cuda_stream if device.type == "cuda" else 0
+    ring = _PACK_TABLES.setdefault((device.index, sid), {"tables": [], "next": 0})
+    if not ring["tables"] or ring["tables"][0].dev.numel() != len(items) * _PackTable.RECORD:
+        ring["tables"] = [_PackTable(len(items), device) for _ in range(4)]
+    tab = ring["tables"][ring["next"] % 4]
+    ring["next"] += 1
+    tab.fill(items, outs)
+    _call("stx_conv3d_pack_many", _p(tab.dev), len(items), total)
+    for (o, m, _), wp in zip(items, outs):
+        o.__dict__.setdefault("_stx_pack_train", {})[m] = ((o._version, o.data_ptr()), wp)
+        o.__dict__["_stx_pack_used"] = set()
+
+
+def _pack_weight_train(w, mode, fwd, given=None):
+    if (not isinstance(w, torch.nn.Parameter) or (given is not None and given is not w) or not _CACHE_ENABLED
+            or not _pack_batch_enabled() or (w.is_cuda and torch.cuda.is_current_stream_capturing())):
+        return pack_weight(w, mode)
+    _chk(w, "weight", 5)
+    st = _PACK_STATE.setdefault(w.device, {"dirty": False, "reg": {}})
+    cache = w.__dict__.setdefault("_stx_pack_train", {})
+    key = (id(w), mode)
+    ref = st["reg"].get(key)
+    hit = cache.get(mode)
+    valid = ref is not None and ref() is w and hit is not None and hit[0] == (w._version, w.data_ptr())
+    if fwd:
+        used = w.__dict__.setdefault("_stx_pack_used", set())
+        if ref is not None and ref() is w and (st["dirty"] or not valid or mode in used):
+            _pack_batch(w.device)
+            valid, hit = True, cache[mode]
+        if valid:
+            w.__dict__["_stx_pack_used"].add(mode)
+            return hit[1]
+    else:
+        st["dirty"] = True
+        if valid:
+            return hit[1]
+    import weakref
+    st["reg"][key] = weakref.ref(w)
+    wp = pack_weight(w, mode)
+    cache[mode] = ((w._version, w.data_ptr()), wp)
+    if fwd:
+        w.__dict__.setdefault("_stx_pack_used", set()).add(mode)
+    return wp
 
 
 def pack_weight(w, mode, owner=None):
@@ -337,10 +444,10 @@
             z, stats = conv3d_c1_forward(x, w.contiguous()), None
         elif transposed:
             Cout = w.shape[1]
-            z, stats = deconv3d_forward(x, pack_weight(w, 2), Cout, want_stats=want_stats)
+            z, stats = deconv3d_forward(x, _pack_weight_train(w, 2, True), Cout, want_stats=want_stats)
         else:
             Cout = w.shape[0]
-            z, stats = conv3d_forward(x, pack_weight(w, 0), Cout, ks, stride, want_stats=want_stats)
+            z, stats = conv3d_forward(x, _pack_weight_train(w, 0, True), Cout, ks, stride, want_stats=want_stats)
         ctx.save_for_backward(x, w)
         ctx.cfg = (ks, stride, transposed)
         if stats is None:
@@ -368,7 +475,7 @@
         if transposed:
             Ci, Co = w.shape[0], w.shape[1]
             if ctx.needs_input_grad[0]:
-                gx, _ = conv3d_forward(gz, pack_weight(w, 0), Ci, 3, 2)
+                gx, _ = conv3d_forward(gz, _pack_weight_train(w, 0, False), Ci, 3, 2)
             if ctx.needs_input_grad[1]:
                 gz_w = gz if Co % 32 == 0 else _pad_channels(gz, (Co + 31) // 32 * 32)
                 x_w = x if Ci % 32 == 0 else _pad_channels(x, (Ci + 31) // 32 * 32)
@@ -393,14 +500,14 @@
                         parts.append(g)
                     gx = torch.cat(parts, -1)
                 elif stride == 1:
-                    gx, _ = conv3d_forward(gz_k, pack_weight(w_k, 1), Ci, ks, 1)
+                    gx, _ = conv3d_forward(gz_k, _pack_weight_train(w_k, 1, False, w), Ci, ks, 1)
                 else:
                     if Co % 32:
                         Cp = (Co + 31) // 32 * 32
                         gz_k = _pad_channels(gz, Cp)
                         w_k = w.new_zeros(Cp, *w.shape[1:])
                         w_k[:Co] = w
-                    gx, _ = deconv3d_forward(gz_k, pack_weight(w_k, 2), Ci, out_dims=(D, H, W))
+                    gx, _ = deconv3d_forward(gz_k, _pack_weight_train(w_k, 2, False, w), Ci, out_dims=(D, H, W))
             if gw_pre is not None:
                 gw = gw_pre
             elif ctx.needs_input_grad[1]:
@@ -1291,7 +1398,7 @@
         for (ks, stride, want), w in zip(cfgs, ws):
             if x.shape[-1] != w.shape[1] or w.shape[1] % 8 or w.shape[0] % 8 or _is_c1(w, ks, stride, False):
                 raise StxError(f"SharedInputConvsFn: weight {tuple(w.shape)} on an input of {x.shape[-1]} channels")
-            z, stats = conv3d_forward(x, pack_weight(w, 0), w.shape[0], ks, stride, want_stats=want)
+            z, stats = conv3d_forward(x, _pack_weight_train(w, 0, True), w.shape[0], ks, stride, want_stats=want)
             if stats is None:
                 stats = x.new_empty(0)
             ctx.mark_non_differentiable(stats)
@@ -1323,7 +1430,7 @@
             for k in sorted((k for k in range(len(ws)) if gzs[k] is not None), key=rank):
                 (ks, stride, _), w, gz = ctx.cfgs[k], ws[k], gzs[k]
                 if stride == 1:
-                    gx, _ = conv3d_forward(gz, pack_weight(w, 1), Ci, ks, 1, residual=gx)
+                    gx, _ = conv3d_forward(gz, _pack_weight_train(w, 1, False), Ci, ks, 1, residual=gx)
                 else:
                     Co = w.shape[0]
                     gz_k, w_k = gz, w
@@ -1332,7 +1439,7 @@
                         gz_k = _pad_channels(gz, Cp)
                         w_k = w.new_zeros(Cp, *w.shape[1:])
                         w_k[:Co] = w
-                    gx, _ = deconv3d_forward(gz_k, pack_weight(w_k, 2), Ci, out_dims=(D, H, W), residual=gx)
+                    gx, _ = deconv3d_forward(gz_k, _pack_weight_train(w_k, 2, False, w), Ci, out_dims=(D, H, W), residual=gx)
         for k, (w, gz) in enumerate(zip(ws, gzs)):
             if gz is None or not ctx.needs_input_grad[2 + k] or gws[k] is not None:
                 continue
@@ -1535,7 +1642,7 @@
     return v if v.is_contiguous() else v.contiguous()
 
 
-def conv2d_forward(x, w, dgrad=False, groups=1, want_stats=False):
+def conv2d_forward(x, w, dgrad=False, groups=1, want_stats=False, add=None):
     _chk(x, "x", 4)
     wo = _ohwi(w)
     _chk(wo, "weight", 4)
@@ -1545,6 +1652,12 @@
     if Cin != Kin or B % groups:
         raise StxError(f"conv2d: input {tuple(x.shape)} against weight {tuple(w.shape)} (dgrad={dgrad}, groups={groups})")
     out = torch.empty(B, H, W, Nout, dtype=torch.float32, device=x.device)
+    if add is not None:
+        _chk(add, "add", 4)
+        if not dgrad or want_stats or groups != 1 or add.shape != out.shape:
+            raise StxError(f"conv2d: add {tuple(add.shape)} goes with the plain data gradient {tuple(out.shape)} only")
+        _call("stx_conv2d_dgrad_add", _p(x), _p(wo), _p(add), _p(out), B, H, W, Kin, Nout)
+        return out, None
     part = None
     if want_stats:
         rows = int(get_lib().raw("stx_conv2d_stat_rows")(groups))
@@ -1558,26 +1671,34 @@
 class Conv2dFn(torch.autograd.Function):
 
     @staticmethod
-    def forward(ctx, x, w, groups):
+    def forward(ctx, x, w, groups, skip=False):
         xl = x.permute(0, 2, 3, 1)
         if not xl.is_contiguous():
             xl = xl.contiguous()
         z, part = conv2d_forward(xl, w, False, groups, True)
         ctx.save_for_backward(x, w)
         ctx.mark_non_differentiable(part)
-        return z, part
-
-    @staticmethod
-    def backward(ctx, gz, _gpart):
+        ctx.set_materialize_grads(False)
+        return (z, part, x.view_as(x)) if skip else (z, part)
+
+    @staticmethod
+    def backward(ctx, gz, _gpart, gskip=None):
         x, w = ctx.saved_tensors
+        gx = gw = None
+        if gz is None:
+            gz = x.new_zeros(x.shape[0], x.shape[2], x.shape[3], w.shape[0])
         gz = gz.contiguous()
-        gx = gw = None
         if ctx.needs_input_grad[0]:
-            gx = conv2d_forward(gz, w, True)[0].permute(0, 3, 1, 2)
+            add = None
+            if gskip is not None:
+                add = gskip.permute(0, 2, 3, 1)
+                if not add.is_contiguous():
+                    add = add.contiguous()
+            gx = conv2d_forward(gz, w, True, add=add)[0].permute(0, 3, 1, 2)
         if ctx.needs_input_grad[1]:
             gw = torch.ops.aten.convolution_backward(gz.permute(0, 3, 1, 2), x, w, None, (1, 1), (1, 1), (1, 1), False, (0, 0), 1,
                                                      (False, True, False))[1]
-        return gx, gw, None
+        return gx, gw, None, None
 
 
 def bn_finalize(partials, count, gamma, beta, running_mean, running_var, momentum, eps, groups=1):
```
